# kiva12138/MIMRL

Measured on AMD Instinct MI355X. Metric: two-stage train iters/sec, higher is better.
Workload: dtype bf16

## Files before the change

include/mimrl.h:

```cpp
#ifndef MIMRL_H_
#define MIMRL_H_

#include <stdint.h>

#ifdef __cplusplus
extern "C" {
#endif

#define MIMRL_ABI_VERSION 6
#define MIMRL_MAX_BLOCKS 4
#define MIMRL_MAX_BATCH 2048
#define MIMRL_MAX_BATCH_CONCAT 1024
#define MIMRL_MAX_CLASSES 8

enum { MIMRL_OK = 0, MIMRL_ERR_ARG = -1, MIMRL_ERR_HIP = -2, MIMRL_ERR_STATE = -3, MIMRL_ERR_NODEVICE = -4 };
enum { MIMRL_GROUP_MAIN = 0, MIMRL_GROUP_CRITIC = 1 };
enum { MIMRL_CRITIC_SEPARATE = 0, MIMRL_CRITIC_CONCAT = 1 };
enum { MIMRL_BOUND_INFONCE = 0, MIMRL_BOUND_NWJ, MIMRL_BOUND_TUBA, MIMRL_BOUND_DV, MIMRL_BOUND_JS_FGAN,
       MIMRL_BOUND_JS, MIMRL_BOUND_SMILE, MIMRL_BOUND_MINE, MIMRL_BOUND_INTERPOLATE };
enum { MIMRL_ACT_NONE = 0, MIMRL_ACT_RELU = 1, MIMRL_ACT_GELU = 2, MIMRL_ACT_TANH = 3 };
enum { MIMRL_PREC_FP32 = 0, MIMRL_PREC_BF16_GEMM_FWD = 1, MIMRL_PREC_BF16_GEMM_BWD = 2, MIMRL_PREC_BF16_GRU_FWD = 4,
       MIMRL_PREC_BF16_GRU_BWD = 8, MIMRL_PREC_BF16 = 15 };

enum { MIMRL_BASELINE_CONSTANT = 0, MIMRL_BASELINE_GAUSSAIN = 1, MIMRL_BASELINE_UNNORMALIZED = 2 };
enum { MIMRL_ENCODER_GRU = 0, MIMRL_ENCODER_CONV = 1, MIMRL_ENCODER_LSTM = 2 };
enum { MIMRL_TASK_LOSS_MAE = 0, MIMRL_TASK_LOSS_MSE = 1, MIMRL_TASK_LOSS_RMSE = 2, MIMRL_TASK_LOSS_SIMSE = 3, MIMRL_TASK_LOSS_CCC = 4 };
enum { MIMRL_CLASS_LOSS_CE = 5, MIMRL_CLASS_LOSS_FOCAL = 6, MIMRL_CLASS_LOSS_BCE = 7 };

typedef struct mimrl_cfg {
  int32_t batch;
  int32_t seq_len;
  int32_t time_len;
  int32_t d_t, d_a, d_v;
  int32_t d_common;
  int32_t n_blocks;
  int32_t d_hiddens[MIMRL_MAX_BLOCKS][3];
  int32_t d_outs[MIMRL_MAX_BLOCKS][3];
  int32_t res_project[MIMRL_MAX_BLOCKS];
  int32_t bias, ln_first;
  int32_t activation;
  int32_t compose_t_sum, compose_k_sum;
  int32_t critic_type, bound_type;
  int32_t cmi_hardtanh;
  int32_t k_neighbor;
  int32_t bank_capacity;
  float dropout[4];
  float dropout_mlp[3];
  float coef1[11];
  float coef2[8];
  float weight_decay, grad_clip;
  float beta1, beta2, adam_eps;
  int32_t precision;
  int32_t use_graph;
  int32_t device_anchors;
  int32_t baseline_type;
  int32_t encoder;
  uint64_t seed;
  int32_t num_class;
} mimrl_cfg;

typedef struct mimrl_buffers {
  float *main_p, *main_g, *main_m, *main_v;
  float *crit_p, *crit_g, *crit_m, *crit_v;
  const float *text, *audio, *video, *labels;
  const float *bank_c, *bank_f, *bank_t, *bank_a, *bank_v;
  int32_t* anchors;
  float *lr_main, *lr_critic;
  float *pred;
  float *feats;
  float *scalars;
  const int32_t* knn_override;
  int32_t* counters;
} mimrl_buffers;

enum {
  MIMRL_S1_LOSS = 0,
  MIMRL_S1_MIS = 1,
  MIMRL_S1_LOSSES = 12,
  MIMRL_S2_LOSS = 32,
  MIMRL_S2_TASK = 33,
  MIMRL_S2_MIS = 34,
  MIMRL_S2_LOSSES = 42,
  MIMRL_NSCALARS = 64
};

const char* mimrl_last_error(void);
int mimrl_abi_version(void);
int mimrl_deterministic(void);
int mimrl_device_check(void);

int mimrl_layout_count(const mimrl_cfg* cfg);
int mimrl_layout_entry(const mimrl_cfg* cfg, int idx, char* name, int name_cap, int* group, int64_t* offset, int* ndim,
                       int* dim0, int* dim1);
int mimrl_layout_entry_dim2(const mimrl_cfg* cfg, int idx);
int64_t mimrl_bucket_floats(const mimrl_cfg* cfg, int group);

typedef struct mimrl_handle mimrl_handle;
int mimrl_create(const mimrl_cfg* cfg, void* hip_stream, mimrl_handle** out);
int mimrl_bind(mimrl_handle* h, const mimrl_buffers* bufs);
int mimrl_set_bank_rows(mimrl_handle* h, int rows);
int mimrl_set_inputs(mimrl_handle* h, int set, const float* text, const float* audio, const float* video, const float* labels);
int mimrl_stage1_pipe_prime(mimrl_handle* h);
int mimrl_stage1_pipe(mimrl_handle* h, int next_valid);
int mimrl_stage1_step(mimrl_handle* h);
int mimrl_stage2_step(mimrl_handle* h);
int mimrl_two_stage_step(mimrl_handle* h);
int mimrl_stage_grads(mimrl_handle* h, int stage);
int mimrl_stage_apply(mimrl_handle* h, int stage);
int mimrl_stage_grads_part(mimrl_handle* h, int stage, int part);
int mimrl_forward(mimrl_handle* h, int train_mode, int with_losses);
int mimrl_estimate(mimrl_handle* h, int stage);
int mimrl_set_stage2_prefetch(mimrl_handle* h, int on);
int mimrl_stage2_forward_tail(mimrl_handle* h);
int mimrl_set_grad_scale(mimrl_handle* h, float scale);
int mimrl_params_changed(mimrl_handle* h);
int64_t mimrl_workspace_bytes(const mimrl_handle* h);
enum { MIMRL_PH_GEMM_MISC = 0, MIMRL_PH_GRU_FWD, MIMRL_PH_GRU_BWD, MIMRL_PH_CUBE_FWD, MIMRL_PH_CUBE_BWD, MIMRL_PH_EST_FWD,
       MIMRL_PH_EST_BWD, MIMRL_PH_OPT, MIMRL_PH_MODEL_MISC, MIMRL_NPHASES };
int mimrl_profile_enable(mimrl_handle* h, int on);
int mimrl_set_kernel_stamps(mimrl_handle* h, unsigned long long* ring, int slots);
int mimrl_comm_unique_id(void* out128);
int mimrl_set_comm(mimrl_handle* h, const void* unique_id128, int world, int rank);
int64_t mimrl_main_late_offset(const mimrl_handle* h);
int mimrl_set_comm_critic_bf16(mimrl_handle* h, int on);
int mimrl_set_task_loss(mimrl_handle* h, int kind);
int mimrl_set_class_loss(mimrl_handle* h, int kind);
int mimrl_profile_read(mimrl_handle* h, float* ms_sum , int32_t* launches );
int mimrl_profile_read_gemm(mimrl_handle* h, double out[4]);
void mimrl_destroy(mimrl_handle* h);

int mimrl_op_gemm(void* stream, const float* A, const float* B, float* C, int M, int N, int K, int batch,
                  const int64_t strides[9] , const float* bias_n,
                  const float* bias_m, float alpha, float beta, int act, int precision);
int mimrl_op_gemm_ex(void* stream, const float* A, const float* B, float* C, int M, int N, int K, int batch, const int64_t strides[9],
                     const float* A2, const float* B2, int K2, const int64_t strides2[6], int a_gap_at, int a_gap_rows,
                     const float* bias_n, const float* gradact_u, float* colsum, int act, int precision);
int mimrl_op_gemm16(void* stream, const void* A, const void* B, void* C, int M, int N, int K, int batch, const int64_t strides[9],
                    const void* A2, const void* B2, int K2, const int64_t strides2[6], int batch_in, const int64_t strides_bo[5],
                    const float* bias_n, int flags);
int mimrl_op_gemm_wgrad_group(void* stream, int n, const float* const* A, const float* const* B, float* const* C, const int32_t* dims,
                              const int64_t* strides, int precision);
int64_t mimrl_op_gru_saved_floats(int B, int T);
int mimrl_op_gru_forward(void* stream, const float* gx_f, const float* gx_r, const float* whh_f, const float* whh_r,
                         const float* bhh_f, const float* bhh_r, const int32_t* lens, float* out, float* saved_f,
                         float* saved_r, int B, int T, int precision);
int mimrl_op_gru_backward(void* stream, const float* whh_f, const float* whh_r, const float* saved_f,
                          const float* saved_r, const int32_t* lens, const float* out, const float* dout, float* dg_f,
                          float* dg_r, float* hprev_f, float* hprev_r, int B, int T, int precision);
int mimrl_op_recur_btv(int B, int nmod);
int mimrl_op_lstm_forward(void* stream, const float* gx_f, const float* gx_r, const float* whh_f, const float* whh_r,
                          const float* bhh_f, const float* bhh_r, const int32_t* lens, float* out, float* saved_f,
                          float* saved_r, int B, int T, int kernel);
int mimrl_op_lstm_backward(void* stream, const float* whh_f, const float* whh_r, const float* saved_f,
                           const float* saved_r, const int32_t* lens, const float* out, const float* dout, float* dg_f,
                           float* dg_r, float* hprev_f, float* hprev_r, int B, int T, int kernel);
int mimrl_op_concat_dw(void* stream, const void* dz2, const void* a1, float* dw2, const void* dz1, const void* a0, float* dw1, int E, int64_t rows,
                       int64_t dw_stride, const float* ds, const void* a2h, float* dw3, const uint32_t* m2, const float* w3, const float* P,
                       const float* Q, int B);
int mimrl_op_gru_wgrad(void* stream, const void* const* dg, const void* const* x, const void* const* hp, float* const* dw_ih,
                       float* const* dw_hh, int64_t rows, int kp);
int mimrl_op_mi_bound(void* stream, const float* scores, float* dscores, float* mi, const float* gscale, int E, int B,
                      int bound);
int mimrl_op_mi_bound_ex(void* stream, const float* scores, float* dscores, float* mi, float* mi_loss, const float* gscale,
                         int E, int B, int bound, uint32_t lossform);
#define MIMRL_NCE_WS_FLOATS 2064
int mimrl_op_mi_infonce_rows(void* stream, const float* scores, float* dscores, float* mi, float* mi_loss, const float* gscale,
                             int E, int B, float* ws);
int mimrl_op_mi_bound_baseline(void* stream, float* scores, float* dscores, float* mi, const float* gscale, const float* lb,
                               float* dlb, int E, int B, int bound);
int mimrl_op_mi_sep_infonce(void* stream, const float* tout, float* dtout, float* mi, float* mi_loss, const float* gscale, int E,
                            int B, int tiled);
int mimrl_op_knn(void* stream, const float* Z, int dz, int N, const int32_t* anchors, int m, int k, int32_t* idx_out);
int mimrl_op_sample_anchors(void* stream, int32_t* anchors_out, int ncall, int m, int N, uint64_t seed, const int32_t* step,
                            uint32_t stream_id, int step_add);
int mimrl_knn_r1_host(const float* z, int N, const int32_t* anchors, int m, int k, int32_t* idx_out);
int mimrl_set_knn_override_mask(mimrl_handle* h, int stage, unsigned call_mask);
int mimrl_op_cmi_loss(void* stream, const float* logits, float* dlogits, float* bce, float* cmi, const float* g_bce,
                      const float* g_cmi, int E, int n, int hardtanh);
int mimrl_op_task_loss(void* stream, int kind, const float* pred, const float* y, float* dpred, float* loss, int B);
int mimrl_op_class_loss(void* stream, int kind, const float* logits, const float* y, float* dlogits, float* loss, int B, int C);
int mimrl_op_gather_rows(void* stream, int n_arrays, const void* const* src, void* const* dst, const int64_t* row_bytes, int64_t src_rows,
                         const int32_t* idx, int rows, int max_workgroups);
int mimrl_op_mlp_stack_forward(void* stream, int nb, int rows, int brows, int nl, const int32_t* dims, const float* const* W,
                               const float* const* b, int64_t pstride, const float* in, float* const* act, float* out);
int mimrl_op_mlp_stack_backward(void* stream, int nb, int rows, int brows, int nl, const int32_t* dims, const float* const* W,
                                int64_t pstride, const float* const* act, const float* dout, float* const* dz, float* din,
                                float* const* db);
int mimrl_probe_cube(mimrl_handle* h, const float* x, float* out, const float* dout, float* dx);
int mimrl_probe_encoders(mimrl_handle* h, float* cube_x, const float* dcube, const float* dmean);
int mimrl_probe_mi(mimrl_handle* h, int stage, float* mi, float* scores, float* dtin_out);
int mimrl_probe_cmi(mimrl_handle* h, int stage, const float* cmi_in, float* logits, float* vals, float* dcin_out);
int mimrl_probe_knn(mimrl_handle* h, int stage, int32_t* idx_out);
int mimrl_op_adam(void* stream, float* p, float* g, float* m, float* v, int64_t n, const float* lr, const int32_t* step,
                  float beta1, float beta2, float eps, float weight_decay, float clip);

#ifdef __cplusplus
}
#endif
#endif
```

mimrl_amd/_lib.py:

```python
from __future__ import annotations

import ctypes as C
import os
from typing import List, Tuple

_HERE = os.path.dirname(os.path.abspath(__file__))
DETERMINISTIC = os.environ.get("MIMRL_DETERMINISTIC", "0") not in ("", "0")
LIB_PATH = os.environ.get("MIMRL_LIB_PATH") or os.path.join(_HERE, "libmimrl_hip_det.so" if DETERMINISTIC else "libmimrl_hip.so")
MAX_BLOCKS = 4
MAX_BATCH = 2048
MAX_BATCH_CONCAT = 1024
NCE_WS_FLOATS = 2064
NSCALARS = 64
MAX_CLASSES = 8
PHASES = ["gemm_misc", "gru_fwd", "gru_bwd", "cube_fwd", "cube_bwd", "est_fwd", "est_bwd", "opt", "model_misc"]
S1_LOSS, S1_MIS, S1_LOSSES, S2_LOSS, S2_TASK, S2_MIS, S2_LOSSES = 0, 1, 12, 32, 33, 34, 42

BOUNDS = {"infonce": 0, "nwj": 1, "tuba": 2, "dv": 3, "js_fgan": 4, "js": 5, "smile": 6, "mine": 7, "interpolate": 8}
ACTS = {"none": 0, "relu": 1, "gelu": 2, "tanh": 3}
PREC = {"fp32": 0, "bf16": 15, "bf16_gemm_fwd": 1, "bf16_gemm_bwd": 2, "bf16_gemm": 3, "bf16_gru": 12, "bf16_nogemmbwd": 13}


class MimrlError(RuntimeError):
    pass


class Cfg(C.Structure):
    _fields_ = [
        ("batch", C.c_int32), ("seq_len", C.c_int32), ("time_len", C.c_int32),
        ("d_t", C.c_int32), ("d_a", C.c_int32), ("d_v", C.c_int32), ("d_common", C.c_int32),
        ("n_blocks", C.c_int32),
        ("d_hiddens", (C.c_int32 * 3) * MAX_BLOCKS), ("d_outs", (C.c_int32 * 3) * MAX_BLOCKS),
        ("res_project", C.c_int32 * MAX_BLOCKS),
        ("bias", C.c_int32), ("ln_first", C.c_int32), ("activation", C.c_int32),
        ("compose_t_sum", C.c_int32), ("compose_k_sum", C.c_int32),
        ("critic_type", C.c_int32), ("bound_type", C.c_int32), ("cmi_hardtanh", C.c_int32),
        ("k_neighbor", C.c_int32), ("bank_capacity", C.c_int32),
        ("dropout", C.c_float * 4), ("dropout_mlp", C.c_float * 3),
        ("coef1", C.c_float * 11), ("coef2", C.c_float * 8),
        ("weight_decay", C.c_float), ("grad_clip", C.c_float),
        ("beta1", C.c_float), ("beta2", C.c_float), ("adam_eps", C.c_float),
        ("precision", C.c_int32), ("use_graph", C.c_int32), ("device_anchors", C.c_int32), ("baseline_type", C.c_int32),
        ("encoder", C.c_int32),
        ("seed", C.c_uint64),
        ("num_class", C.c_int32),
    ]


_FP = C.c_void_p


class Buffers(C.Structure):
    _fields_ = [(n, _FP) for n in (
        "main_p", "main_g", "main_m", "main_v", "crit_p", "crit_g", "crit_m", "crit_v",
        "text", "audio", "video", "labels", "bank_c", "bank_f", "bank_t", "bank_a", "bank_v",
        "anchors", "lr_main", "lr_critic", "pred", "feats", "scalars", "knn_override", "counters")]


_lib = None


def load() -> C.CDLL:
    global _lib
    if _lib is not None:
        return _lib
    if not os.path.exists(LIB_PATH):
        raise MimrlError(f"{LIB_PATH} is missing: build it with `python -c 'import __graft_entry__ as g; g.build()'` "
                         f"or `make -C mimrl_amd/csrc` (hipcc --offload-arch=gfx950). There is no CPU fallback.")
    try:
        import torch
    except ImportError:
        pass
    lib = C.CDLL(LIB_PATH)
    if os.environ.get("MIMRL_LIB_PATH"):
        class _Partial:
            def __init__(self, lib):
                object.__setattr__(self, "_lib", lib)

            def __getattr__(self, name):
                try:
                    return getattr(self._lib, name)
                except AttributeError:
                    return type("_Missing", (), {})()
        real, lib = lib, _Partial(lib)
    lib.mimrl_last_error.restype = C.c_char_p
    lib.mimrl_bucket_floats.restype = C.c_int64
    lib.mimrl_workspace_bytes.restype = C.c_int64
    lib.mimrl_op_gru_saved_floats.restype = C.c_int64
    lib.mimrl_destroy.restype = None
    lib.mimrl_op_gemm.argtypes = [_FP, _FP, _FP, _FP, C.c_int, C.c_int, C.c_int, C.c_int, C.POINTER(C.c_int64), _FP, _FP,
                                  C.c_float, C.c_float, C.c_int, C.c_int]
    lib.mimrl_op_gemm_ex.argtypes = [_FP, _FP, _FP, _FP, C.c_int, C.c_int, C.c_int, C.c_int, C.POINTER(C.c_int64), _FP, _FP, C.c_int,
                                     C.POINTER(C.c_int64), C.c_int, C.c_int, _FP, _FP, _FP, C.c_int, C.c_int]
    lib.mimrl_comm_unique_id.argtypes = [_FP]
    lib.mimrl_set_comm.argtypes = [_FP, _FP, C.c_int, C.c_int]
    lib.mimrl_set_comm_critic_bf16.argtypes = [_FP, C.c_int]
    lib.mimrl_set_task_loss.argtypes = [_FP, C.c_int]
    lib.mimrl_op_task_loss.argtypes = [_FP, C.c_int, _FP, _FP, _FP, _FP, C.c_int]
    lib.mimrl_set_class_loss.argtypes = [_FP, C.c_int]
    lib.mimrl_op_class_loss.argtypes = [_FP, C.c_int, _FP, _FP, _FP, _FP, C.c_int, C.c_int]
    lib.mimrl_op_gather_rows.argtypes = [_FP, C.c_int, C.POINTER(C.c_void_p), C.POINTER(C.c_void_p), C.POINTER(C.c_int64), C.c_int64, _FP,
                                         C.c_int, C.c_int]
    lib.mimrl_main_late_offset.argtypes = [_FP]
    lib.mimrl_main_late_offset.restype = C.c_int64
    lib.mimrl_op_gemm16.argtypes = [_FP, _FP, _FP, _FP, C.c_int, C.c_int, C.c_int, C.c_int, C.POINTER(C.c_int64), _FP, _FP, C.c_int,
                                    C.POINTER(C.c_int64), C.c_int, C.POINTER(C.c_int64), _FP, C.c_int]
    lib.mimrl_op_gemm_wgrad_group.argtypes = [_FP, C.c_int, C.POINTER(C.c_void_p), C.POINTER(C.c_void_p), C.POINTER(C.c_void_p),
                                              C.POINTER(C.c_int32), C.POINTER(C.c_int64), C.c_int]
    lib.mimrl_op_adam.argtypes = [_FP, _FP, _FP, _FP, _FP, C.c_int64, _FP, _FP, C.c_float, C.c_float, C.c_float,
                                  C.c_float, C.c_float]
    lib.mimrl_op_gru_forward.argtypes = [_FP] * 11 + [C.c_int, C.c_int, C.c_int]
    lib.mimrl_op_gru_backward.argtypes = [_FP] * 12 + [C.c_int, C.c_int, C.c_int]
    lib.mimrl_op_lstm_forward.argtypes = [_FP] * 11 + [C.c_int, C.c_int, C.c_int]
    lib.mimrl_op_lstm_backward.argtypes = [_FP] * 12 + [C.c_int, C.c_int, C.c_int]
    lib.mimrl_op_recur_btv.argtypes = [C.c_int, C.c_int]
    lib.mimrl_op_concat_dw.argtypes = [C.c_void_p] * 7 + [C.c_int, C.c_int64, C.c_int64] + [C.c_void_p] * 7 + [C.c_int]
    lib.mimrl_op_gru_wgrad.argtypes = [C.c_void_p] + [C.POINTER(C.c_void_p)] * 5 + [C.c_int64, C.c_int]
    lib.mimrl_op_mi_bound.argtypes = [_FP] * 5 + [C.c_int, C.c_int, C.c_int]
    lib.mimrl_op_mi_bound_ex.argtypes = [_FP] * 6 + [C.c_int, C.c_int, C.c_int, C.c_uint32]
    lib.mimrl_op_mi_infonce_rows.argtypes = [_FP] * 6 + [C.c_int, C.c_int, _FP]
    lib.mimrl_op_mi_sep_infonce.argtypes = [_FP] * 6 + [C.c_int, C.c_int, C.c_int]
    lib.mimrl_op_mi_bound_baseline.argtypes = [_FP] * 7 + [C.c_int, C.c_int, C.c_int]
    lib.mimrl_op_knn.argtypes = [_FP, _FP, C.c_int, C.c_int, _FP, C.c_int, C.c_int, _FP]
    lib.mimrl_op_cmi_loss.argtypes = [_FP] * 7 + [C.c_int, C.c_int, C.c_int]
    lib.mimrl_op_sample_anchors.argtypes = [_FP, _FP, C.c_int, C.c_int, C.c_int, C.c_uint64, _FP, C.c_uint32, C.c_int]
    lib.mimrl_create.argtypes = [C.POINTER(Cfg), _FP, C.POINTER(_FP)]
    lib.mimrl_bind.argtypes = [_FP, C.POINTER(Buffers)]
    lib.mimrl_profile_read.argtypes = [_FP, C.POINTER(C.c_float), C.POINTER(C.c_int32)]
    lib.mimrl_profile_read_gemm.argtypes = [_FP, C.POINTER(C.c_double)]
    for fn in ("mimrl_set_bank_rows", "mimrl_stage_grads", "mimrl_stage_grads_part", "mimrl_stage_apply", "mimrl_estimate", "mimrl_profile_enable", "mimrl_set_stage2_prefetch"):
        getattr(lib, fn).argtypes = [_FP, C.c_int]
    lib.mimrl_set_grad_scale.argtypes = [_FP, C.c_float]
    lib.mimrl_stage_grads_part.argtypes = [_FP, C.c_int, C.c_int]
    lib.mimrl_set_inputs.argtypes = [_FP, C.c_int, _FP, _FP, _FP, _FP]
    lib.mimrl_knn_r1_host.argtypes = [_FP, C.c_int, _FP, C.c_int, C.c_int, _FP]
    lib.mimrl_set_knn_override_mask.argtypes = [_FP, C.c_int, C.c_uint]
    for fn in ("mimrl_stage1_step", "mimrl_stage2_step", "mimrl_two_stage_step", "mimrl_destroy", "mimrl_workspace_bytes", "mimrl_params_changed",
               "mimrl_stage2_forward_tail"):
        getattr(lib, fn).argtypes = [_FP]
    lib.mimrl_forward.argtypes = [_FP, C.c_int, C.c_int]
    lib.mimrl_set_kernel_stamps.argtypes = [_FP, _FP, C.c_int]
    lib.mimrl_probe_cube.argtypes = [_FP] * 5
    lib.mimrl_probe_mi.argtypes = [_FP, C.c_int, _FP, _FP, _FP]
    lib.mimrl_probe_cmi.argtypes = [_FP, C.c_int, _FP, _FP, _FP, _FP]
    lib.mimrl_probe_knn.argtypes = [_FP, C.c_int, _FP]
    lib.mimrl_probe_encoders.argtypes = [_FP] * 4
    lib.mimrl_layout_count.argtypes = [C.POINTER(Cfg)]
    lib.mimrl_layout_entry_dim2.argtypes = [C.POINTER(Cfg), C.c_int]
    lib.mimrl_bucket_floats.argtypes = [C.POINTER(Cfg), C.c_int]
    lib.mimrl_layout_entry.argtypes = [C.POINTER(Cfg), C.c_int, C.c_char_p, C.c_int, C.POINTER(C.c_int),
                                       C.POINTER(C.c_int64), C.POINTER(C.c_int), C.POINTER(C.c_int), C.POINTER(C.c_int)]
    if os.environ.get("MIMRL_LIB_PATH"):
        lib = real
    _lib = lib
    return lib


ENCODERS = {"gru": 0, "conv": 1, "lstm": 2}
BASELINES = {"constant": 0, "gaussain": 1, "unnormalized": 2}

EXPORTS = [
    "mimrl_last_error", "mimrl_abi_version", "mimrl_deterministic", "mimrl_device_check", "mimrl_layout_count", "mimrl_layout_entry", "mimrl_layout_entry_dim2",
    "mimrl_bucket_floats", "mimrl_create", "mimrl_bind", "mimrl_set_bank_rows", "mimrl_set_inputs", "mimrl_stage1_step", "mimrl_stage2_step", "mimrl_two_stage_step",
    "mimrl_stage_grads", "mimrl_stage_grads_part", "mimrl_stage_apply", "mimrl_forward", "mimrl_estimate", "mimrl_profile_enable", "mimrl_profile_read", "mimrl_profile_read_gemm",
    "mimrl_workspace_bytes", "mimrl_params_changed", "mimrl_set_stage2_prefetch", "mimrl_stage2_forward_tail", "mimrl_set_grad_scale", "mimrl_destroy", "mimrl_op_gemm", "mimrl_op_gemm_ex", "mimrl_op_gemm16", "mimrl_op_gemm_wgrad_group",
    "mimrl_op_gru_saved_floats", "mimrl_op_gru_forward", "mimrl_op_gru_backward", "mimrl_op_gru_wgrad", "mimrl_op_concat_dw", "mimrl_op_mi_bound", "mimrl_op_mi_bound_ex", "mimrl_op_mi_bound_baseline", "mimrl_op_mi_sep_infonce", "mimrl_op_knn",
    "mimrl_op_cmi_loss", "mimrl_op_sample_anchors", "mimrl_knn_r1_host", "mimrl_set_knn_override_mask", "mimrl_op_mlp_stack_forward", "mimrl_op_mlp_stack_backward", "mimrl_op_adam",
    "mimrl_probe_cube", "mimrl_probe_mi", "mimrl_probe_cmi", "mimrl_probe_knn", "mimrl_probe_encoders", "mimrl_set_kernel_stamps", "mimrl_comm_unique_id", "mimrl_set_comm", "mimrl_main_late_offset", "mimrl_set_comm_critic_bf16",
    "mimrl_stage1_pipe_prime", "mimrl_stage1_pipe", "mimrl_set_task_loss", "mimrl_op_task_loss", "mimrl_set_class_loss", "mimrl_op_class_loss",
    "mimrl_op_mi_infonce_rows", "mimrl_op_lstm_forward", "mimrl_op_lstm_backward", "mimrl_op_recur_btv", "mimrl_op_gather_rows",
]

TASK_LOSSES = {"MAE": 0, "MSE": 1, "RMSE": 2, "SIMSE": 3, "CCC": 4}
BATCH_COUPLED_LOSSES = ("RMSE", "SIMSE", "CCC")
CLASS_LOSSES = {"CE": 5, "Focal": 6, "BCE": 7}


def task_loss_code(opt, world: int = 1) -> int:
    loss = getattr(opt, "loss", "MAE")
    task = getattr(opt, "task", "regression")
    ncls = int(getattr(opt, "num_class", 1))
    if loss in CLASS_LOSSES:
        if task != "classification":
            raise NotImplementedError(f"--loss {loss} is a classification loss: it needs --task classification (and --num_class)")
        if loss == "BCE" and ncls not in (1, 2):
            raise NotImplementedError(f"--loss BCE needs --num_class 1 or 2, got {ncls} (Solver.py:327-337)")
        if loss != "BCE" and not 2 <= ncls <= MAX_CLASSES:
            raise NotImplementedError(f"--loss {loss} needs 2 <= --num_class <= {MAX_CLASSES}, got {ncls}")
        if int(world) > 1 and loss == "Focal":
            raise NotImplementedError(f"--loss {loss} couples the whole batch: with {int(world)} ranks each would see only its shard, not the "
                                      f"reference's global batch; run it on one rank, or use CE / BCE")
        return CLASS_LOSSES[loss]
    if loss not in TASK_LOSSES:
        raise NotImplementedError(f"--loss {loss}: unknown task loss (choose one of {', '.join(list(TASK_LOSSES) + list(CLASS_LOSSES))})")
    if task == "classification" or ncls > 1:
        raise NotImplementedError(f"--loss {loss} is a regression loss: --task classification / --num_class {ncls} need one of "
                                  f"{', '.join(CLASS_LOSSES)}")
    if int(world) > 1 and loss in BATCH_COUPLED_LOSSES:
        raise NotImplementedError(f"--loss {loss} couples the whole batch: with {int(world)} ranks each would see only its shard, not the "
                                  f"reference's global batch; run it on one rank, or use MAE / MSE")
    return TASK_LOSSES[loss]


def check(rc: int) -> int:
    if rc < 0:
        raise MimrlError(f"libmimrl_hip error {rc}: {load().mimrl_last_error().decode()}")
    return rc


def make_cfg(opt, d_t: int, d_a: int, d_v: int, seq_len: int = None, bank_capacity: int = 0, precision: str = "fp32",
             use_graph: bool = False, seed: int = 0, device_anchors: bool = False, batch: int = None) -> Cfg:
    c = Cfg()
    c.batch = int(batch if batch is not None else opt.batch_size)
    c.time_len = int(opt.time_len)
    c.seq_len = int(seq_len if seq_len is not None else opt.time_len)
    c.d_t, c.d_a, c.d_v, c.d_common = int(d_t), int(d_a), int(d_v), int(opt.d_common)
    enc = getattr(opt, "encoders", "gru")
    if enc not in ENCODERS:
        raise MimrlError(f"--encoders {enc}: choose gru, conv or lstm (Model.py:237)")
    c.encoder = ENCODERS[enc]
    nb = len(opt.d_hiddens)
    if nb > MAX_BLOCKS or len(opt.d_outs) != nb or len(opt.res_project) != nb:
        raise MimrlError("d_hiddens / d_outs / res_project must have the same length (<= 4)")
    c.n_blocks = nb
    for i in range(nb):
        for ax in range(3):
            c.d_hiddens[i][ax] = int(opt.d_hiddens[i][ax])
            c.d_outs[i][ax] = int(opt.d_outs[i][ax])
        c.res_project[i] = int(bool(opt.res_project[i]))
    c.bias, c.ln_first = int(bool(opt.bias)), int(bool(opt.ln_first))
    if opt.activate not in ACTS:
        raise MimrlError(f"--activate {opt.activate} not supported on the HIP path (gelu/relu/tanh)")
    c.activation = ACTS[opt.activate]
    for name, attr in (("features_compose_t", "compose_t_sum"), ("features_compose_k", "compose_k_sum")):
        v = getattr(opt, name, "mean")
        if v not in ("mean", "sum"):
            raise MimrlError(f"--{name} {v}: only mean/sum supported")
        setattr(c, attr, int(v == "sum"))
    if opt.critic_type not in ("separate", "concat"):
        raise NotImplementedError(opt.critic_type)
    c.critic_type = 0 if opt.critic_type == "separate" else 1
    bl = getattr(opt, "baseline_type", "constant")
    if bl not in BASELINES:
        raise NotImplementedError(f"--baseline_type {bl}")
    c.baseline_type = BASELINES[bl]
    if opt.bound_type not in BOUNDS:
        raise NotImplementedError(opt.bound_type)
    c.bound_type = BOUNDS[opt.bound_type]
    if opt.cmi_last_acticate not in ("sigmoid", "hardtanh"):
        raise NotImplementedError(opt.cmi_last_acticate)
    c.cmi_hardtanh = int(opt.cmi_last_acticate == "hardtanh")
    c.k_neighbor = int(opt.k_neighbor)
    c.bank_capacity = int(bank_capacity)
    for i in range(4):
        c.dropout[i] = float(opt.dropout[i])
    for i in range(3):
        c.dropout_mlp[i] = float(opt.dropout_mlp[i])
    if len(opt.loss_mi_coefficient1) != 11 or len(opt.loss_mi_coefficient2) != 8:
        raise MimrlError("loss_mi_coefficient1/2 need 11 / 8 entries")
    for i in range(11):
        c.coef1[i] = float(opt.loss_mi_coefficient1[i])
    for i in range(8):
        c.coef2[i] = float(opt.loss_mi_coefficient2[i])
    c.weight_decay, c.grad_clip = float(opt.weight_decay), float(opt.gradient_clip)
    c.beta1, c.beta2, c.adam_eps = 0.9, 0.999, 1e-8
    c.precision = PREC[precision]
    c.use_graph = int(bool(use_graph))
    c.device_anchors = int(bool(device_anchors))
    c.seed = int(seed) & 0xFFFFFFFFFFFFFFFF
    c.num_class = int(getattr(opt, "num_class", 1))
    return c


def layout_entries(cfg: Cfg) -> Tuple[List[Tuple[str, int, int, Tuple[int, ...]]], Tuple[int, int]]:
    lib = load()
    n = check(lib.mimrl_layout_count(C.byref(cfg)))
    out = []
    name = C.create_string_buffer(256)
    g, nd, d0, d1 = C.c_int(), C.c_int(), C.c_int(), C.c_int()
    off = C.c_int64()
    for i in range(n):
        check(lib.mimrl_layout_entry(C.byref(cfg), i, name, 256, C.byref(g), C.byref(off), C.byref(nd), C.byref(d0), C.byref(d1)))
        shape = (d0.value, d1.value) if nd.value == 2 else (d0.value,)
        if nd.value == 3:
            shape = (d0.value, d1.value, check(lib.mimrl_layout_entry_dim2(C.byref(cfg), i)))
        out.append((name.value.decode(), g.value, off.value, shape))
    sizes = (check(lib.mimrl_bucket_floats(C.byref(cfg), 0)), check(lib.mimrl_bucket_floats(C.byref(cfg), 1)))
    return out, sizes


def knn_r1_host(z, anchors, k: int):
    import numpy as np
    z = np.ascontiguousarray(np.asarray(z, dtype=np.float32).reshape(-1))
    a = np.ascontiguousarray(np.asarray(anchors, dtype=np.int32).reshape(-1))
    if int(k) >= (len(z) - len(a)) // 2:
        return None
    out = np.empty((len(a), int(k)), dtype=np.int32)
    check(load().mimrl_knn_r1_host(z.ctypes.data_as(C.c_void_p), len(z), a.ctypes.data_as(C.c_void_p), len(a), int(k),
                                   out.ctypes.data_as(C.c_void_p)))
    return out
```

mimrl_amd/csrc/cube_bwd_fused.h:

```cpp
#pragma once
#include "common.h"
#include "model_ops.h"

namespace mimrl {

struct LAxisBwdArgs {
  const float *dz, *y, *mean, *rstd, *gamma;
  const float* u;
  const float *w2, *w1, *wr;
  float *dy, *du, *dx;
  float *db2, *db1;
  int B, il, hl, ol, C, act;
};
bool laxis_bwd_supported(int il, int hl, int ol, int C);
int laxis_bwd_fused(hipStream_t s, const LAxisBwdArgs& a);

struct DAxisBwdArgs {
  const float *dz, *y, *mean, *rstd, *gamma;
  const float* u;
  const __bf16 *w2t, *w1t, *wrt;
  float *dy, *du, *dx;
  long R;
  int act;
  float *dgamma, *dbeta, *db2, *db1;
};
bool daxis_bwd_supported(int id, int hd, int od);
int daxis_bwd_fused(hipStream_t s, const DAxisBwdArgs& a);

struct WtTransposeArgs { const float* src[12]; __bf16* dst[12]; int n; };
int wt_transpose_bf16(hipStream_t s, const WtTransposeArgs& a);

int daxis_param_grads(hipStream_t s, const float* y, const float* mean, const float* rstd, const float* dz, const float* dy,
                      const float* du, float* dgamma, float* dbeta, float* db2, float* db1, long R);

#ifdef MIMRL_PHASE_PROBE
int cube_bwd_read_phases(long long* out);
#endif

}
```

mimrl_amd/csrc/cube_bwd_fused.hip:

```cpp
#include "cube_bwd_fused.h"
#include "kmix_device.h"

namespace mimrl {

namespace {

#ifdef MIMRL_PHASE_PROBE
__device__ long long g_cbwd_phase[64];
#define BPHASE(base, i) do { if (blockIdx.x == 0 && blockIdx.y == 0 && threadIdx.x == 0) g_cbwd_phase[(base) + (i)] = (long long)wall_clock64(); } while (0)
#else
#define BPHASE(base, i) do { } while (0)
#endif

constexpr int CT = 128;
constexpr int KP = 64 + 8;


template <bool LONG = false>
__global__ __launch_bounds__(256, LONG ? 2 : 1) void laxis_bwd_kernel(LAxisBwdArgs a) {
  __shared__ __attribute__((aligned(16))) __bf16 sdyu[2][CT][KP];
  auto& sdy = sdyu[0];
  auto& sdu = sdyu[1];
  __shared__ __attribute__((aligned(16))) __bf16 wts[3][64][KP];
  float (*red)[2][CT] = reinterpret_cast<float (*)[2][CT]>(&sdu[0][0]);
  __shared__ float acc_l[3][64];
  __shared__ LdsAcc acc_h[64];
  __shared__ float sgam[64];
  const int tid = threadIdx.x, lane = tid & 63, wave = tid >> 6, lr = lane & 31, lh = lane >> 5;
  const int b = blockIdx.y, c0 = blockIdx.x * CT;
  const int il = a.il, hl = a.hl, ol = a.ol, C = a.C;
  const int pb = ol > 32 ? 16 : 0;
  BPHASE(pb, 0);

  float uu[2][16];
  {
    const int ccu = c0 + wave * 32 + lr;
#pragma unroll
    for (int mt = 0; mt < 2; ++mt)
#pragma unroll
      for (int r = 0; r < 16; ++r) {
        const int h = min(mt * 32 + (r & 3) + 8 * (r >> 2) + 4 * lh, hl - 1);
        uu[mt][r] = a.u[((long)b * hl + h) * C + ccu];
      }
  }
  {
    uint4* z = reinterpret_cast<uint4*>(&wts[0][0][0]);
    for (int i = tid; i < 3 * 64 * KP * 2 / 16; i += 256) z[i] = make_uint4(0u, 0u, 0u, 0u);
    if (tid < 64) { acc_l[0][tid] = 0.f; acc_l[1][tid] = 0.f; acc_l[2][tid] = 0.f; acc_h[tid].zero(); sgam[tid] = a.gamma[tid < ol ? tid : ol - 1]; }
  }
  __syncthreads();
  BPHASE(pb, 1);
  {
    const int n2 = ol * hl, n1 = hl * il, nr = ol * il;
    float wv[3][16];
#pragma unroll
    for (int j = 0; j < 16; ++j) {
      const int idx = tid + 256 * j;
      wv[0][j] = a.w2[idx < n2 ? idx : n2 - 1];
      if constexpr (!LONG) {
        wv[1][j] = a.w1[idx < n1 ? idx : n1 - 1];
        wv[2][j] = a.wr[idx < nr ? idx : nr - 1];
      }
    }
#pragma unroll
    for (int j = 0; j < 16; ++j) {
      const int idx = tid + 256 * j;
      if (idx < n2) { const int o = idx / hl, h = idx - o * hl; wts[0][h][o] = to_bf16(wv[0][j]); }
      if constexpr (!LONG) {
        if (idx < n1) { const int h = idx / il, i = idx - h * il; wts[1][i][h] = to_bf16(wv[1][j]); }
        if (idx < nr) { const int o = idx / il, i = idx - o * il; wts[2][i][o] = to_bf16(wv[2][j]); }
      }
    }
  }

  BPHASE(pb, 2);
  const int col = tid & (CT - 1), half = tid >> 7;
  const long cidx = (long)b * C + c0 + col;
  const float mu = a.mean[cidx], rs = a.rstd[cidx];
  const float* __restrict__ dzb = a.dz + (long)b * ol * C + c0 + col;
  const float* __restrict__ yb = a.y + (long)b * ol * C + c0 + col;
  float* __restrict__ dyb = a.dy + (long)b * ol * C + c0 + col;
  float gq[32], xq[32];
#pragma unroll
  for (int j = 0; j < 32; ++j) {
    const int l = min(half + 2 * j, ol - 1);
    gq[j] = dzb[(long)l * C]; xq[j] = yb[(long)l * C];
  }
  float s1 = 0.f, s2 = 0.f;
#pragma unroll
  for (int j = 0; j < 32; ++j) {
    const int l = half + 2 * j;
    xq[j] = (xq[j] - mu) * rs;
    gq[j] = l < ol ? gq[j] * sgam[min(l, 63)] : 0.f;
    s1 += gq[j]; s2 += gq[j] * xq[j];
  }
  BPHASE(pb, 3);
  red[0][half][col] = s1;
  red[1][half][col] = s2;
  __syncthreads();
  s1 = (red[0][0][col] + red[0][1][col]) / ol;
  s2 = (red[1][0][col] + red[1][1][col]) / ol;
#pragma unroll
  for (int j = 0; j < 32; ++j) {
    const int l = half + 2 * j;
    if (l < ol) {
      const float v = rs * (gq[j] - s1 - xq[j] * s2);
      dyb[(long)l * C] = v;
      sdy[col][l] = to_bf16(v);
    }
  }
  for (int l = ol + ((half ^ ol) & 1); l < 64; l += 2) sdy[col][l] = to_bf16(0.f);
  __syncthreads();

  if (a.db2 && tid >= 192 && tid - 192 < ol) {
    float t = 0.f;
    for (int c = 0; c < CT; ++c) t += (float)sdy[(c + tid) & (CT - 1)][tid - 192];
    acc_l[2][tid - 192] = t;
  }
  BPHASE(pb, 4);
  const int nt = wave;
  const int cc = c0 + nt * 32 + lr;
  {
    f32x16 acc0, acc1;
#pragma unroll
    for (int r = 0; r < 16; ++r) { acc0[r] = 0.f; acc1[r] = 0.f; }
#pragma unroll
    for (int ks = 0; ks < 4; ++ks) {
      const bf16x8 bf = *reinterpret_cast<const bf16x8*>(&sdy[nt * 32 + lr][ks * 16 + 8 * lh]);
      const bf16x8 a0 = *reinterpret_cast<const bf16x8*>(&wts[0][lr][ks * 16 + 8 * lh]);
      acc0 = __builtin_amdgcn_mfma_f32_32x32x16_bf16(a0, bf, acc0, 0, 0, 0);
      const bf16x8 a1 = *reinterpret_cast<const bf16x8*>(&wts[0][32 + lr][ks * 16 + 8 * lh]);
      acc1 = __builtin_amdgcn_mfma_f32_32x32x16_bf16(a1, bf, acc1, 0, 0, 0);
    }
    act_dispatch(a.act, [&](auto AT) __attribute__((always_inline)) {
#pragma unroll
    for (int mt = 0; mt < 2; ++mt)
#pragma unroll
      for (int r = 0; r < 16; ++r) {
        const int h = mt * 32 + (r & 3) + 8 * (r >> 2) + 4 * lh;
        float v = 0.f;
        if (h < hl) {
          const long ui = ((long)b * hl + h) * C + cc;
          v = (mt == 0 ? acc0[r] : acc1[r]) * act_grad_c<decltype(AT)::value>(a.act, uu[mt][r]);
          a.du[ui] = v;
        }
        sdu[nt * 32 + lr][h] = to_bf16(v);
        if (a.db1) {
          const float t = half_sum_hi(v);
          if (lr == 16 && h < hl) acc_h[h].add(t);
        }
      }
    });
  }
  __syncthreads();
  BPHASE(pb, 5);
  if constexpr (LONG) {
    float w1v[16], wrv[16];
    auto wreq = [&](int i0) __attribute__((always_inline)) {
      const int i = min(i0 + (tid & 63), il - 1);
#pragma unroll
      for (int j = 0; j < 16; ++j) {
        const int r = 16 * (tid >> 6) + j;
        w1v[j] = a.w1[(long)min(r, hl - 1) * il + i];
        wrv[j] = a.wr[(long)min(r, ol - 1) * il + i];
      }
    };
    wreq(0);
    for (int i0 = 0; i0 < il; i0 += 64) {
      __syncthreads();
      {
        const int ii = tid & 63, r0 = 16 * (tid >> 6);
        const bool iok = i0 + ii < il;
        bf16x8 p1[2], p2[2];
#pragma unroll
        for (int j = 0; j < 16; ++j) {
          p1[j >> 3][j & 7] = to_bf16(iok && r0 + j < hl ? w1v[j] : 0.f);
          p2[j >> 3][j & 7] = to_bf16(iok && r0 + j < ol ? wrv[j] : 0.f);
        }
        *reinterpret_cast<bf16x8*>(&wts[1][ii][r0]) = p1[0]; *reinterpret_cast<bf16x8*>(&wts[1][ii][r0 + 8]) = p1[1];
        *reinterpret_cast<bf16x8*>(&wts[2][ii][r0]) = p2[0]; *reinterpret_cast<bf16x8*>(&wts[2][ii][r0 + 8]) = p2[1];
      }
      __syncthreads();
      wreq(i0 + 64 < il ? i0 + 64 : i0);
      f32x16 acc0, acc1;
#pragma unroll
      for (int r = 0; r < 16; ++r) { acc0[r] = 0.f; acc1[r] = 0.f; }
#pragma unroll
      for (int ks = 0; ks < 8; ++ks) {
        const bool first = ks < 4;
        const int kk = (first ? ks : ks - 4) * 16 + 8 * lh;
        const bf16x8 bf = *reinterpret_cast<const bf16x8*>(first ? &sdu[nt * 32 + lr][kk] : &sdy[nt * 32 + lr][kk]);
        const bf16x8 a0 = *reinterpret_cast<const bf16x8*>(&wts[first ? 1 : 2][lr][kk]);
        acc0 = __builtin_amdgcn_mfma_f32_32x32x16_bf16(a0, bf, acc0, 0, 0, 0);
        const bf16x8 a1 = *reinterpret_cast<const bf16x8*>(&wts[first ? 1 : 2][32 + lr][kk]);
        acc1 = __builtin_amdgcn_mfma_f32_32x32x16_bf16(a1, bf, acc1, 0, 0, 0);
      }
      {
#pragma unroll
        for (int mt = 0; mt < 2; ++mt)
#pragma unroll
          for (int r = 0; r < 16; ++r) {
            const int i = i0 + mt * 32 + (r & 3) + 8 * (r >> 2) + 4 * lh;
            if (i < il) a.dx[((long)b * il + i) * C + cc] = mt == 0 ? acc0[r] : acc1[r];
          }
      }
    }
  } else {
    f32x16 acc0, acc1;
#pragma unroll
    for (int r = 0; r < 16; ++r) { acc0[r] = 0.f; acc1[r] = 0.f; }
#pragma unroll
    for (int ks = 0; ks < 8; ++ks) {
      const bool first = ks < 4;
      const int kk = (first ? ks : ks - 4) * 16 + 8 * lh;
      const bf16x8 bf = *reinterpret_cast<const bf16x8*>(first ? &sdu[nt * 32 + lr][kk] : &sdy[nt * 32 + lr][kk]);
      const bf16x8 a0 = *reinterpret_cast<const bf16x8*>(&wts[first ? 1 : 2][lr][kk]);
      acc0 = __builtin_amdgcn_mfma_f32_32x32x16_bf16(a0, bf, acc0, 0, 0, 0);
      const bf16x8 a1 = *reinterpret_cast<const bf16x8*>(&wts[first ? 1 : 2][32 + lr][kk]);
      acc1 = __builtin_amdgcn_mfma_f32_32x32x16_bf16(a1, bf, acc1, 0, 0, 0);
    }
    {
#pragma unroll
      for (int mt = 0; mt < 2; ++mt)
#pragma unroll
        for (int r = 0; r < 16; ++r) {
          const int i = mt * 32 + (r & 3) + 8 * (r >> 2) + 4 * lh;
          if (i < il) a.dx[((long)b * il + i) * C + cc] = mt == 0 ? acc0[r] : acc1[r];
        }
    }
  }
  __syncthreads();
  BPHASE(pb, 6);
  if (a.db2 && tid < ol) acc_add(&a.db2[tid], acc_l[2][tid]);
  if (a.db1 && tid >= 64 && tid - 64 < hl) acc_add(&a.db1[tid - 64], acc_h[tid - 64].get());
  BPHASE(pb, 7);
}

}

#ifdef MIMRL_PHASE_PROBE
int cube_bwd_read_phases(long long* out) { return hipMemcpyFromSymbol(out, HIP_SYMBOL(g_cbwd_phase), sizeof(long long) * 64) == hipSuccess ? 0 : 1; }
#endif

bool laxis_bwd_supported(int il, int hl, int ol, int C) {
  return il >= 1 && hl >= 1 && ol >= 1 && hl <= 64 && ol <= 64 && C % CT == 0;
}

int laxis_bwd_fused(hipStream_t s, const LAxisBwdArgs& a) {
  if (!laxis_bwd_supported(a.il, a.hl, a.ol, a.C)) return set_error(MIMRL_ERR_ARG, "laxis_bwd_fused: unsupported shape");
  if (!a.wr) return set_error(MIMRL_ERR_ARG, "laxis_bwd_fused: needs the residual projection");
  if (a.il > 64) hipLaunchKernelGGL(laxis_bwd_kernel<true>, dim3(a.C / CT, a.B), dim3(256), 0, s, a);
  else hipLaunchKernelGGL(laxis_bwd_kernel<false>, dim3(a.C / CT, a.B), dim3(256), 0, s, a);
  LAUNCH_CHECK();
  return MIMRL_OK;
}

namespace {

constexpr int DR = 32;
constexpr int DP = 128 + 8;

__global__ __launch_bounds__(256) void daxis_bwd_kernel(DAxisBwdArgs a) {
  __shared__ __attribute__((aligned(16))) __bf16 sdy[DR][DP];
  __shared__ __attribute__((aligned(16))) __bf16 sdu[DR][DP];
  __shared__ LdsAcc spg[3][128];
  const int tid = threadIdx.x, lane = tid & 63, wave = tid >> 6, lr = lane & 31, lh = lane >> 5;
  const long r0 = (long)blockIdx.x * DR;
  const bool pg = a.dgamma != nullptr;
  const int pb = gridDim.x <= 200 ? 32 : 48;
  BPHASE(pb, 0);
  if (pg) for (int i = tid; i < 3 * 128; i += 256) (&spg[0][0])[i].zero();
  const int row1 = tid >> 3, part1 = tid & 7;
  const long r1 = r0 + row1;
  const bool ok1 = r1 < a.R;
  const long rc1 = ok1 ? r1 : a.R - 1;
  const float mu1 = a.mean[rc1], rs1 = a.rstd[rc1];
  float4 gz4[4], yv4[4];
#pragma unroll
  for (int q = 0; q < 4; ++q) {
    gz4[q] = *reinterpret_cast<const float4*>(a.dz + rc1 * 128 + part1 * 16 + q * 4);
    yv4[q] = *reinterpret_cast<const float4*>(a.y + rc1 * 128 + part1 * 16 + q * 4);
  }
  const int n = wave * 32 + lr;
  bf16x8 bw2[8], bw1[8], bwr[8];
#pragma unroll
  for (int ks = 0; ks < 8; ++ks) {
    bw2[ks] = *reinterpret_cast<const bf16x8*>(a.w2t + n * 128 + ks * 16 + 8 * lh);
    bw1[ks] = *reinterpret_cast<const bf16x8*>(a.w1t + n * 128 + ks * 16 + 8 * lh);
    bwr[ks] = *reinterpret_cast<const bf16x8*>(a.wrt + n * 128 + ks * 16 + 8 * lh);
  }
  float uu[16];
#pragma unroll
  for (int r = 0; r < 16; ++r) {
    const long row = min(r0 + (r & 3) + 8 * (r >> 2) + 4 * lh, a.R - 1);
    uu[r] = a.u[row * 128 + n];
  }
  BPHASE(pb, 1);
  {
    const int row = row1, part = part1;
    const long r = r1;
    const bool ok = ok1;
    float g[16], xh[16], dyk[16];
    float s1 = 0.f, s2 = 0.f;
    const float mu = mu1, rs = rs1;
#pragma unroll
    for (int q = 0; q < 4; ++q) {
      const float4 gz = gz4[q];
      const float4 yv = yv4[q];
      const float gg[4] = {gz.x, gz.y, gz.z, gz.w}, yy[4] = {yv.x, yv.y, yv.z, yv.w};
#pragma unroll
      for (int j = 0; j < 4; ++j) {
        g[q * 4 + j] = gg[j];
        xh[q * 4 + j] = (yy[j] - mu) * rs;
        const float dxh = gg[j] * a.gamma[part * 16 + q * 4 + j];
        s1 += dxh; s2 += dxh * xh[q * 4 + j];
      }
    }
    s1 = group_sum<8>(s1); s2 = group_sum<8>(s2);
    s1 *= (1.f / 128.f); s2 *= (1.f / 128.f);
#pragma unroll
    for (int q = 0; q < 4; ++q) {
      float v[4];
#pragma unroll
      for (int j = 0; j < 4; ++j) {
        const int c = part * 16 + q * 4 + j;
        v[j] = rs * (g[q * 4 + j] * a.gamma[c] - s1 - xh[q * 4 + j] * s2);
      }
      if (ok) *reinterpret_cast<float4*>(a.dy + r * 128 + part * 16 + q * 4) = make_float4(v[0], v[1], v[2], v[3]);
      bf16x4 p; p[0] = to_bf16(v[0]); p[1] = to_bf16(v[1]); p[2] = to_bf16(v[2]); p[3] = to_bf16(v[3]);
      *reinterpret_cast<bf16x4*>(&sdy[row][part * 16 + q * 4]) = p;
      if (pg) {
#pragma unroll
        for (int j = 0; j < 4; ++j) { const float gz = ok ? g[q * 4 + j] : 0.f; xh[q * 4 + j] *= gz; g[q * 4 + j] = gz; v[j] = ok ? v[j] : 0.f; }
        dyk[q * 4 + 0] = v[0]; dyk[q * 4 + 1] = v[1]; dyk[q * 4 + 2] = v[2]; dyk[q * 4 + 3] = v[3];
      }
    }
    if (pg) {
      __syncthreads();
#pragma unroll
      for (int j = 0; j < 16; ++j) {
        float sa = xh[j], sb = g[j], sc = dyk[j];
#pragma unroll
        for (int o = 8; o < 64; o <<= 1) { sa += __shfl_xor(sa, o, 64); sb += __shfl_xor(sb, o, 64); sc += __shfl_xor(sc, o, 64); }
        if (lane < 8) { spg[0][part * 16 + j].add(sa); spg[1][part * 16 + j].add(sb); spg[2][part * 16 + j].add(sc); }
      }
    }
  }
  __syncthreads();
  BPHASE(pb, 2);
  {
    f32x16 acc;
#pragma unroll
    for (int r = 0; r < 16; ++r) acc[r] = 0.f;
#pragma unroll
    for (int ks = 0; ks < 8; ++ks) {
      const bf16x8 af = *reinterpret_cast<const bf16x8*>(&sdy[lr][ks * 16 + 8 * lh]);
      acc = __builtin_amdgcn_mfma_f32_32x32x16_bf16(af, bw2[ks], acc, 0, 0, 0);
    }
    float csum = 0.f;
    act_dispatch(a.act, [&](auto AT) __attribute__((always_inline)) {
#pragma unroll
    for (int r = 0; r < 16; ++r) {
      const int m = (r & 3) + 8 * (r >> 2) + 4 * lh;
      const long row = r0 + m;
      float v = 0.f;
      if (row < a.R) {
        v = acc[r] * act_grad_c<decltype(AT)::value>(a.act, uu[r]);
        a.du[row * 128 + n] = v;
      }
      sdu[m][n] = to_bf16(v);
      csum += v;
    }
    });
    if (pg) {
      csum += __shfl_xor(csum, 32, 64);
      if (lh == 0) acc_add(&a.db1[n], csum);
    }
  }
  __syncthreads();
  BPHASE(pb, 3);
  if (pg && tid < 128) {
    acc_add(&a.dgamma[tid], spg[0][tid].get());
    acc_add(&a.dbeta[tid], spg[1][tid].get());
    acc_add(&a.db2[tid], spg[2][tid].get());
  }
  {
    f32x16 acc;
#pragma unroll
    for (int r = 0; r < 16; ++r) acc[r] = 0.f;
#pragma unroll
    for (int ks = 0; ks < 8; ++ks) {
      const bf16x8 a1 = *reinterpret_cast<const bf16x8*>(&sdu[lr][ks * 16 + 8 * lh]);
      acc = __builtin_amdgcn_mfma_f32_32x32x16_bf16(a1, bw1[ks], acc, 0, 0, 0);
      const bf16x8 a2 = *reinterpret_cast<const bf16x8*>(&sdy[lr][ks * 16 + 8 * lh]);
      acc = __builtin_amdgcn_mfma_f32_32x32x16_bf16(a2, bwr[ks], acc, 0, 0, 0);
    }
#pragma unroll
    for (int r = 0; r < 16; ++r) {
      const long row = r0 + (r & 3) + 8 * (r >> 2) + 4 * lh;
      if (row < a.R) a.dx[row * 128 + n] = acc[r];
    }
  }
  BPHASE(pb, 4);
}

__global__ void wt_transpose_kernel(WtTransposeArgs a) {
  __shared__ float t[32][33];
  const float* __restrict__ src = a.src[blockIdx.z];
  __bf16* __restrict__ dst = a.dst[blockIdx.z];
  const int k0 = blockIdx.y * 32, n0 = blockIdx.x * 32, tx = threadIdx.x & 31, ty = threadIdx.x >> 5;
  for (int j = ty; j < 32; j += 8) t[j][tx] = src[(k0 + j) * 128 + n0 + tx];
  __syncthreads();
  for (int j = ty; j < 32; j += 8) dst[(n0 + j) * 128 + k0 + tx] = to_bf16(t[tx][j]);
}

__global__ __launch_bounds__(256) void daxis_param_grads_kernel(const float* __restrict__ y, const float* __restrict__ mean,
                                                                const float* __restrict__ rstd, const float* __restrict__ dz,
                                                                const float* __restrict__ dy, const float* __restrict__ du,
                                                                float* __restrict__ dgamma, float* __restrict__ dbeta,
                                                                float* __restrict__ db2, float* __restrict__ db1, long R) {
  __shared__ float4 red[4][8][32];
  const int cq = threadIdx.x & 31, rl = threadIdx.x >> 5;
  const long r0 = (long)blockIdx.x * 64;
  float4 a0 = make_float4(0.f, 0.f, 0.f, 0.f), a1 = a0, a2 = a0, a3 = a0;
#pragma unroll
  for (int i = 0; i < 8; ++i) {
    const long r = r0 + rl + 8 * i;
    const long rc = r < R ? r : R - 1;
    const float m = r < R ? 1.f : 0.f;
    const float mu = mean[rc], rs = rstd[rc] * m;
    const float4 g = *reinterpret_cast<const float4*>(dz + rc * 128 + cq * 4);
    const float4 yv = *reinterpret_cast<const float4*>(y + rc * 128 + cq * 4);
    const float4 v = *reinterpret_cast<const float4*>(dy + rc * 128 + cq * 4);
    const float4 u = *reinterpret_cast<const float4*>(du + rc * 128 + cq * 4);
    a0.x += g.x * (yv.x - mu) * rs; a0.y += g.y * (yv.y - mu) * rs; a0.z += g.z * (yv.z - mu) * rs; a0.w += g.w * (yv.w - mu) * rs;
    a1.x += g.x * m; a1.y += g.y * m; a1.z += g.z * m; a1.w += g.w * m;
    a2.x += v.x * m; a2.y += v.y * m; a2.z += v.z * m; a2.w += v.w * m;
    a3.x += u.x * m; a3.y += u.y * m; a3.z += u.z * m; a3.w += u.w * m;
  }
  red[0][rl][cq] = a0; red[1][rl][cq] = a1; red[2][rl][cq] = a2; red[3][rl][cq] = a3;
  __syncthreads();
#pragma unroll
  for (int h = 0; h < 2; ++h) {
    const int idx = threadIdx.x + 256 * h, q = idx >> 7, c = idx & 127;
    const float* base = reinterpret_cast<const float*>(&red[q][0][0]);
    float sum = 0.f;
#pragma unroll
    for (int j = 0; j < 8; ++j) sum += base[j * 128 + c];
    float* dst = q == 0 ? dgamma : (q == 1 ? dbeta : (q == 2 ? db2 : db1));
    if (dst) acc_add(&dst[c], sum);
  }
}

}

int daxis_param_grads(hipStream_t s, const float* y, const float* mean, const float* rstd, const float* dz, const float* dy,
                      const float* du, float* dgamma, float* dbeta, float* db2, float* db1, long R) {
  if (R <= 0) return MIMRL_OK;
  hipLaunchKernelGGL(daxis_param_grads_kernel, dim3((unsigned)((R + 63) / 64)), dim3(256), 0, s, y, mean, rstd, dz, dy, du, dgamma, dbeta,
                     db2, db1, R);
  LAUNCH_CHECK();
  return MIMRL_OK;
}

bool daxis_bwd_supported(int id, int hd, int od) { return id == 128 && hd == 128 && od == 128; }

int daxis_bwd_fused(hipStream_t s, const DAxisBwdArgs& a) {
  if (!a.w2t || !a.w1t || !a.wrt) return set_error(MIMRL_ERR_ARG, "daxis_bwd_fused: needs the transposed weight images");
  if ((a.dgamma || a.dbeta || a.db2 || a.db1) && !(a.dgamma && a.dbeta && a.db2 && a.db1))
    return set_error(MIMRL_ERR_ARG, "daxis_bwd_fused: the four parameter-gradient outputs come together");
  hipLaunchKernelGGL(daxis_bwd_kernel, dim3((unsigned)((a.R + DR - 1) / DR)), dim3(256), 0, s, a);
  LAUNCH_CHECK();
  return MIMRL_OK;
}

int wt_transpose_bf16(hipStream_t s, const WtTransposeArgs& a) {
  if (a.n < 1 || a.n > 12) return set_error(MIMRL_ERR_ARG, "wt_transpose_bf16: 1..12 matrices");
  hipLaunchKernelGGL(wt_transpose_kernel, dim3(4, 4, a.n), dim3(256), 0, s, a);
  LAUNCH_CHECK();
  return MIMRL_OK;
}

}
```

mimrl_amd/csrc/engine.h:

```cpp
#pragma once
#include <cstdio>
#include <cstdlib>
#include <cstring>
#include <algorithm>
#include <vector>
#include <dlfcn.h>

#include "cube_fused.h"
#include "mlp_fused.h"
#include "concat_fused.h"
#include "cube_bwd_fused.h"
#include "cube_long.h"
#include "estimator_ops.h"
#include "gemm.h"
#include "gru.h"
#include "gru_wgrad.h"
#include "concat_dw.h"
#include "lstm.h"
#include "layout.h"
#include "comm.h"
#include "model_ops.h"
#include "scoped.h"

namespace mimrl {

namespace eng {


constexpr int H = 128, G = 384, HID = 256, EMB = 128;
constexpr int NE_MI = 5, NE_CMI = 6;
constexpr int ACT_SLACK = 4 * MLPF_MAX_WIDTH;

enum { FT_F = 0, FT_T = 1, FT_A = 2, FT_V = 3, FT_C = 4 };
const int kMiWire[NE_MI][2] = {{FT_F, FT_T}, {FT_F, FT_A}, {FT_F, FT_V}, {FT_T, FT_A}, {FT_T, FT_V}};
const int kCmiWire[NE_CMI][3] = {{FT_A, FT_C, FT_T}, {FT_T, FT_A, FT_C}, {FT_V, FT_C, FT_T},
                                 {FT_T, FT_V, FT_C}, {FT_T, FT_C, FT_A}, {FT_T, FT_C, FT_V}};
static const char* const kVmi[NE_MI] = {"f_t", "f_a", "f_v", "t_a", "t_v"};
static const char* const kVcmi[NE_CMI] = {"ac_t", "ta_c", "vc_t", "tv_c", "tc_a", "tc_v"};

void launch_begin_stage(hipStream_t s, int* rng_step, int* adam_step, float* scalars, int scal_off, int scal_n);
void launch_bucket_to_bf16(hipStream_t s, const float* src, void* dst, long n);
void launch_bucket_from_bf16(hipStream_t s, const void* src, float* dst, long n);
void launch_task_loss(hipStream_t s, int kind, const float* pred, const float* y, float* dpred, float* task, int B, int C = 1);
void launch_finalize_stage1(hipStream_t s, float* scal, const float* mi, const float* cmi, const float* bce, const float* coef1);
void launch_finalize_stage2(hipStream_t s, float* scal, const float* mi, const float* cmi, const float* coef2, int have_mi);
void launch_stage_boundary(hipStream_t s, float* scal, const float* mi, const float* cmi, const float* bce, const float* coef1, int* rng_step,
                           int* adam_step, const float* pred, const float* y, float* dpred, int B, int kind, int C = 1);

struct Roctx {
  int (*push)(const char*) = nullptr;
  int (*pop)() = nullptr;
  Roctx() {
    void* h = dlopen("librocprofiler-sdk-roctx.so", RTLD_LAZY | RTLD_LOCAL);
    if (!h) h = dlopen("librocprofiler-sdk-roctx.so.1", RTLD_LAZY | RTLD_LOCAL);
    if (!h) h = dlopen("libroctx64.so", RTLD_LAZY | RTLD_LOCAL);
    if (!h) h = dlopen("libroctx64.so.4", RTLD_LAZY | RTLD_LOCAL);
    if (h) {
      push = reinterpret_cast<int (*)(const char*)>(dlsym(h, "roctxRangePushA"));
      pop = reinterpret_cast<int (*)()>(dlsym(h, "roctxRangePop"));
      if (!push || !pop) push = nullptr;
    }
  }
};
inline Roctx& roctx() { static Roctx r; return r; }
struct Range {
  bool on;
  explicit Range(const char* name) : on(roctx().push != nullptr) { if (on) roctx().push(name); }
  ~Range() { if (on) roctx().pop(); }
};

struct Lin { long w = -1, b = -1; int out = 0, in = 0; };
struct GruDirW { long w_ih = 0, w_hh = 0, b_ih = 0, b_hh = 0; int din = 0; };
struct AxisW { Lin fc1, fc2; long res = -1, ln_g = -1, ln_b = -1; int in = 0, hid = 0, out = 0; };
struct BlockW { AxisW ax[3]; };
struct MixBuf { float *xn = nullptr, *xn_mean = nullptr, *xn_rstd = nullptr, *u = nullptr, *h = nullptr, *y = nullptr,
                      *z = nullptr, *mean = nullptr, *rstd = nullptr; };
struct BlockBuf { MixBuf l, k, d; };

}

using namespace eng;

}

using namespace mimrl;

struct mimrl_handle {
  mimrl_cfg cfg;
  hipStream_t stream = nullptr;
  hipStream_t user_stream = nullptr;
  hipStream_t cap_stream = nullptr;
  Layout layout;
  mimrl_buffers bufs;
  bool bound = false;
  DetRanges det_ranges;
  float* nce_ws = nullptr;
  bool grads_clean[3] = {true, true, true};
  int bank_rows = 0;
  bool bf16 = false;
  int prec = 0;
  bool bf16_fwd() const { return (prec & MIMRL_PREC_BF16_GEMM_FWD) != 0; }
  bool bf16_bwd() const { return (prec & MIMRL_PREC_BF16_GEMM_BWD) != 0; }

  GruDirW gru[2][2][2];
  long ln_g[2], ln_b[2], w_t;
  BlockW blk[MIMRL_MAX_BLOCKS];
  long cls_w, cls_b;
  __bf16 *crit_img = nullptr, *crit_imgT = nullptr;
  __bf16 *crit_frag = nullptr, *crit_fragT = nullptr;
  FragTable ftab;
  bool frag_side_pending = false;
  bool frag_tr_deferred = false;
  FragTable ftab_tr;
  bool adam_frag_on = true;
  bool boundary_in_adam = false;
  bool img_valid = false;
  unsigned knn_ovr_mask[2] = {0u, 0u};
  bool knn_pre = true;
  bool mi_fused_bwd_done = false;
  bool imgT_ready = false;
  TransposeTable ttab;
  int ensure_images() {
    if (img_valid || !crit_img) return MIMRL_OK;
    MX(bf16_image(user_stream, bufs.crit_p, crit_img, layout.floats[MIMRL_GROUP_CRITIC]));
    if (crit_frag && ftab.n > 0) MX(bf16_frag_images(user_stream, bufs.crit_p, crit_frag, ftab));
    img_valid = true;
    return MIMRL_OK;
  }
  long bl0 = 0, bl_stride = 0, bl_l[4][2];
  float *lbv = nullptr, *dlbv = nullptr, *bact[3] = {nullptr, nullptr, nullptr}, *bdz[3] = {nullptr, nullptr, nullptr}, *bdin = nullptr;
  bool has_baseline() const {
    return cfg.baseline_type != MIMRL_BASELINE_CONSTANT && (cfg.bound_type == MIMRL_BOUND_TUBA || cfg.bound_type == MIMRL_BOUND_INTERPOLATE);
  }
  int baseline_forward();
  int baseline_backward(int stage);
  long tower0 = 0, tower_stride = 0;
  long tower_l[4][2];
  long cmi0 = 0, cmi_stride = 0, cmi_l[4][2];

  char* ws = nullptr;
  size_t ws_bytes = 0, ws_used = 0;
  int* d_ints = nullptr;
  int* d_ints_own = nullptr;
  float* d_consts = nullptr;
  int *lens[2] = {nullptr, nullptr};
  bool kmix_pg_on_side3 = false;
  bool begin_in_pack = false;
  hipEvent_t ev_lens = nullptr;
  float *tx_raw = nullptr, *gx[2][2], *h0[2], *h1[2], *sv[2][2][2], *ln_mean[2], *ln_rstd[2];
  float* tailp_part = nullptr;
  bool pre_done = false;
  int dual_tail_pre();
  float* cube0 = nullptr;
  float *xpack = nullptr, *wpack = nullptr, *bpack = nullptr, *dwih_pack = nullptr, *dwhh_pack = nullptr;
  _Float16* h0h[2] = {nullptr, nullptr}; _Float16* w1h = nullptr; __bf16* w1b = nullptr;
  __bf16* w1bt = nullptr;
  bool h16_on = true;
  float* w2p[MIMRL_MAX_BLOCKS] = {};
  bool w2p_valid[MIMRL_MAX_BLOCKS] = {};
  bool xin_on = true;
  bool part0_done = false;
  bool l0_xin = false;
  bool xpack16 = false;
  bool laxis_bwd_long_on = true;
  bool laxis_long_on = true;
  bool rec16_on = true, dwih_h16_on = true;
  bool hp16_live = false;
  bool dh0_bf16_live = false, ds_bf16_live = false;
  bool h16_live = false;
  bool w1_img_valid = false;
  int KP() const { return ((cfg.d_a > cfg.d_v ? cfg.d_a : cfg.d_v) + 15) & ~15; }
  bool dg_bf16 = false;
  bool concat_compact = false;
  bool a0_regen_live = false;
  bool fused_concat = true;
  bool l0_packed = false;
  bool l0_bwd_pack = false;
  BlockBuf bb[MIMRL_MAX_BLOCKS];
  __bf16* wtT[MIMRL_MAX_BLOCKS][3] = {};
  struct FwdSet {
    int* lens[2] = {nullptr, nullptr};
    float *tx_raw = nullptr, *gx[2][2] = {{nullptr, nullptr}, {nullptr, nullptr}}, *h0[2] = {nullptr, nullptr}, *h1[2] = {nullptr, nullptr};
    float *ln_mean[2] = {nullptr, nullptr}, *ln_rstd[2] = {nullptr, nullptr}, *cube0 = nullptr, *feats = nullptr, *pred = nullptr;
    _Float16* h0h[2] = {nullptr, nullptr};
    BlockBuf bb[MIMRL_MAX_BLOCKS];
  } alt;
  void swap_fwd_set() {
    for (int m = 0; m < 2; ++m) {
      std::swap(lens[m], alt.lens[m]); std::swap(h0[m], alt.h0[m]); std::swap(h1[m], alt.h1[m]); std::swap(h0h[m], alt.h0h[m]);
      std::swap(ln_mean[m], alt.ln_mean[m]); std::swap(ln_rstd[m], alt.ln_rstd[m]);
      for (int d = 0; d < 2; ++d) std::swap(gx[m][d], alt.gx[m][d]);
    }
    std::swap(tx_raw, alt.tx_raw); std::swap(cube0, alt.cube0);
    std::swap(bufs.feats, alt.feats); std::swap(bufs.pred, alt.pred);
    for (int i = 0; i < MIMRL_MAX_BLOCKS; ++i) std::swap(bb[i], alt.bb[i]);
  }
  struct FwdSetSwap {
    mimrl_handle* h; bool on = false;
    explicit FwdSetSwap(mimrl_handle* h_, bool now = true) : h(h_) { if (now) enter(); }
    ~FwdSetSwap() { if (on) h->swap_fwd_set(); }
    FwdSetSwap(const FwdSetSwap&) = delete;
    FwdSetSwap& operator=(const FwdSetSwap&) = delete;
    void enter() { h->swap_fwd_set(); on = true; }
  };
  bool prefetch = false;
  bool defer_tail = false;
  bool tail2_needed = false;
  bool fwd2_pending = false;
  float grad_scale = 1.f;
  void* comm = nullptr; int comm_world = 1, comm_rank = 0;
  bool comm_crit_bf16 = false; void* comm_crit16 = nullptr;
  int task_loss = MIMRL_TASK_LOSS_MAE;
  int ncls() const { return cfg.num_class >= 2 ? cfg.num_class : 1; }
  hipStream_t comm_s = nullptr;
  bool comm_split = true;
  KernelStamp kstamp;

  int run_fwd2_tail();
  hipStream_t pre_stream = nullptr;
  int carve_fwd(size_t* gmax_out);
  float *ff = nullptr, *dpred = nullptr;
  float *tin = nullptr, *ta[3], *tout = nullptr, *scores = nullptr, *dscores = nullptr;
  float *cP = nullptr, *cQ = nullptr, *ca[3];
  int split_part = 0;
  bool fold_unpack = false, unpack_pending = false;
  bool fold_unpack_on = true;
  bool gx_f16 = false;
  int *knn_idx = nullptr, *knn_idx2 = nullptr;
  int knn_flip = 0;
  int knn_slot(int stage) const { return (stage - 1) ^ knn_flip; }
  char* knn_scr[2] = {nullptr, nullptr};
  size_t knn_scr_bytes = 0;
  float *cmi_in = nullptr, *cc[3], *logits = nullptr, *dlogits = nullptr;
  float *mi_raw = nullptr, *cmi_raw = nullptr, *bce_raw = nullptr;
  float *dfeat = nullptr, *dtout = nullptr, *dta[3], *dtin = nullptr, *dca[3], *dP = nullptr, *dQ = nullptr;
  float *dcc[3], *dcin = nullptr;
  static constexpr int NGBUF = 24;
  float* gbuf[NGBUF];
  size_t gbuf_floats = 0;
  float *dtx = nullptr, *ds[2], *dg[2][2][2], *hprev[2][2][2], *dh0[2];

  static constexpr int NSIDE = 6;
  hipStream_t side[NSIDE] = {nullptr, nullptr, nullptr, nullptr, nullptr, nullptr};
  std::vector<hipEvent_t> ev_pool;
  size_t ev_next = 0;
  bool multi_stream = true;
  bool fused_cube_bwd = true;
  bool fused_mlp = true;
  bool fused_cube = true;
  bool fused_pre_on = true;
  bool cube_bookends = true;
  bool keep_cube0 = false;
  int fwd_f16 = 1;
  int next_event(hipEvent_t* e) {
    if (ev_next == ev_pool.size()) {
      hipEvent_t n;
      HIPX(hipEventCreateWithFlags(&n, hipEventDisableTiming));
      ev_pool.push_back(n);
    }
    *e = ev_pool[ev_next++];
    return MIMRL_OK;
  }
  int G_group(hipStream_t st, const GemmDesc* ds, int n) {
    if (!prof_on) return gemm_group(st, ds, n, bf16);
    for (int i = 0; i < n; ++i) MX(G_on(st, ds[i]));
    return MIMRL_OK;
  }
  unsigned side_mask = ~0u;
  bool side_on(int i) const { return multi_stream && ((side_mask >> i) & 1u); }
  hipStream_t S(int i) const { return side_on(i) ? side[i] : stream; }
  int fork(int lo, int hi) {
    if (!multi_stream) return MIMRL_OK;
    hipEvent_t e = nullptr;
    for (int i = lo; i <= hi; ++i) {
      if (!side_on(i)) continue;
      if (!e) { MX(next_event(&e)); HIPX(hipEventRecord(e, stream)); }
      HIPX(hipStreamWaitEvent(side[i], e, 0));
    }
    return MIMRL_OK;
  }
  int join(int lo, int hi) {
    if (!multi_stream) return MIMRL_OK;
    for (int i = lo; i <= hi; ++i) {
      if (!side_on(i)) continue;
      hipEvent_t e;
      MX(next_event(&e));
      HIPX(hipEventRecord(e, side[i]));
      HIPX(hipStreamWaitEvent(stream, e, 0));
    }
    return MIMRL_OK;
  }
  int chain(int i, int j) {
    if (!multi_stream || S(i) == S(j)) return MIMRL_OK;
    hipEvent_t e;
    MX(next_event(&e));
    HIPX(hipEventRecord(e, S(j)));
    HIPX(hipStreamWaitEvent(S(i), e, 0));
    return MIMRL_OK;
  }
  int reduce_bucket(int stage) {
    if (!comm) return MIMRL_OK;
    Range rg(stage == 1 ? "mimrl.stage1.allreduce(crit_g) [RCCL]" : "mimrl.stage2.allreduce(main_g) [RCCL]");
    if (stage == 1 && comm_crit_bf16) {
      const long n = layout.floats[MIMRL_GROUP_CRITIC];
      launch_bucket_to_bf16(stream, bufs.crit_g, comm_crit16, n);
      LAUNCH_CHECK();
      MX(comm_allreduce_sum_bf16(comm, comm_crit16, (size_t)n, stream));
      launch_bucket_from_bf16(stream, comm_crit16, bufs.crit_g, n);
      LAUNCH_CHECK();
      return MIMRL_OK;
    }
    return comm_allreduce_sum(comm, stage == 1 ? bufs.crit_g : bufs.main_g, (size_t)layout.floats[stage == 1 ? MIMRL_GROUP_CRITIC : MIMRL_GROUP_MAIN], stream);
  }
  int enqueue_grads2_reduced(bool skip_zero);
  struct GemmProf { hipEvent_t a, b; double flops, bytes; };
  std::vector<GemmProf> prof_gemm;
  int G_on(hipStream_t st, const GemmDesc& d) {
    if (!prof_on) return gemm(st, d, bf16);
    GemmProf g;
    if (!prof_pool.empty()) { g.a = prof_pool.back().first; g.b = prof_pool.back().second; prof_pool.pop_back(); }
    else { HIPX(hipEventCreate(&g.a)); HIPX(hipEventCreate(&g.b)); }
    auto distinct = [&](long s_b, long s_bo) -> double {
      if (d.batch_in > 0) return (double)(s_bo != 0 ? d.batch / d.batch_in : 1) * (s_b != 0 ? d.batch_in : 1);
      return s_b != 0 ? d.batch : 1;
    };
    g.flops = 2.0 * d.M * d.N * ((double)d.K + (d.A2 ? d.K2 : 0)) * d.batch;
    const double ea = d.a_bf16 ? 2.0 : 4.0, eb = d.b_bf16 ? 2.0 : 4.0;
    g.bytes = ea * d.M * d.K * distinct(d.sa_b, d.sa_bo) + eb * d.K * d.N * distinct(d.sb_b, d.sb_bo) +
              4.0 * d.M * d.N * distinct(d.sc_b, d.sc_bo) * ((d.beta != 0.f || d.atomic) ? 2 : 1);
    if (d.A2) g.bytes += ea * d.M * d.K2 * (d.sa2_b ? d.batch : 1) + eb * d.K2 * d.N * (d.sb2_b ? d.batch : 1);
    HIPX(hipEventRecord(g.a, st));
    const int r = gemm(st, d, bf16);
    HIPX(hipEventRecord(g.b, st));
    prof_gemm.push_back(g);
    return r;
  }

  bool prof_on = false;
  std::vector<std::pair<hipEvent_t, hipEvent_t>> prof_ev[MIMRL_NPHASES];
  std::vector<std::pair<hipEvent_t, hipEvent_t>> prof_pool;
  struct Scope {
    mimrl_handle* h; int ph; hipEvent_t a = nullptr, b = nullptr;
    Scope(mimrl_handle* h_, int ph_) : h(h_), ph(ph_) {
      if (!h->prof_on) return;
      if (!h->prof_pool.empty()) { a = h->prof_pool.back().first; b = h->prof_pool.back().second; h->prof_pool.pop_back(); }
      else { (void)hipEventCreate(&a); (void)hipEventCreate(&b); }
      (void)hipEventRecord(a, h->stream);
    }
    ~Scope() {
      if (!a) return;
      (void)hipEventRecord(b, h->stream);
      h->prof_ev[ph].push_back({a, b});
    }
  };

  struct CachedGraph { hipGraphExec_t exec = nullptr; int rows = -1; };
  struct GraphSet {
    CachedGraph all[3 * 4 + 1 + 2 * 4];
    CachedGraph& graph(int stage, int k) { return all[stage * 4 + k]; }
    CachedGraph& tail() { return all[12]; }
    CachedGraph& pipe(int ahead, int parity) { return all[13 + ahead * 4 + parity]; }
    const void* in[4] = {nullptr, nullptr, nullptr, nullptr};
  } gsets[2];
  int cur_set = 0;
  GraphSet& GS() { return gsets[cur_set]; }
  std::vector<hipGraphExec_t> retired;
  void retire(hipGraphExec_t& ex) { if (ex) { retired.push_back(ex); ex = nullptr; } }
  void drop_graphs(int set = -1) {
    for (int q = 0; q < 2; ++q)
      if (set < 0 || q == set)
        for (CachedGraph& c : gsets[q].all) retire(c.exec);
  }
  template <typename Body>
  int replay_or_capture(CachedGraph& slot, Body&& body, bool postprocess = false);
  float* P(long off) const { return bufs.main_p + off; }
  float* Gm(long off) const { return bufs.main_g + off; }
  float* CP(long off) const { return bufs.crit_p + off; }
  float* CG(long off) const { return bufs.crit_g + off; }
  long conv_w[2] = {0, 0}, conv_b[2] = {0, 0};
  int encoders_forward(bool save, int knn_stage);
  int conv_forward(int knn_stage);
  int conv_backward();
  int lstm_encoders_forward(bool save, int knn_stage);
  int lstm_encoders_backward();
  int rng_add = 0;
  RngKey key() const { return RngKey{(uint32_t)cfg.seed, (uint32_t)(cfg.seed >> 32), d_ints, rng_add}; }
  const float* coef1() const { return d_consts; }
  const float* coef2() const { return d_consts + 11; }
  const float* gs_mi(int stage) const { return d_consts + 19 + (stage - 1) * 5; }
  const float* g_bce(int stage) const { return d_consts + 29 + (stage - 1) * 6; }
  const float* g_cmi(int stage) const { return d_consts + 41 + (stage - 1) * 6; }
  int nprod() const { return (cfg.batch / cfg.k_neighbor) * cfg.k_neighbor; }
  int m_anchor() const { return cfg.batch / cfg.k_neighbor; }

  int resolve();
  int alloc_workspace();
  template <typename T>
  int take(T** p, size_t count) {
    const size_t bytes = (count * sizeof(T) + 255) / 256 * 256;
    if (ws) {
      if (ws_used + bytes > ws_bytes) return set_error(MIMRL_ERR_STATE, "workspace overflow");
      *p = reinterpret_cast<T*>(ws + ws_used);
    }
    ws_used += bytes;
    return MIMRL_OK;
  }
  int carve();

  int G_(const GemmDesc& d) { return G_on(stream, d); }
  struct Deferred { int kind; int side; GemmDesc g; const float* src; long n0, n1, n2, n3; float* dst;
                    const float *p1 = nullptr, *p2 = nullptr, *p3 = nullptr; float* dst2 = nullptr; KMixW kw = KMixW();
                    const float *p4 = nullptr, *p5 = nullptr; float *dst3 = nullptr, *dst4 = nullptr; };
  std::vector<Deferred> deferred;
  int flush_deferred(int only_side = 0);
  int wg_helper = -1;
  int dbg_delay(hipStream_t st, int tag);
  int model_forward(bool train, bool save, int knn_stage = 0, int part = 0);
  int cube_forward(bool train, bool save, const CubePre* pre = nullptr, const CubeHead* head = nullptr);
  bool cube_block_fused(int i, bool train) const;
  int cube_backward(int cur_in, int* cur_out);
  int wt_images(hipStream_t st, bool bwd_bf16, bool launch, bool* d_fused);
  int model_backward();
  int encoders_backward(float* dcube);
  int gru_layer_backward(int l);
  int knn_launch(int stage, hipStream_t st);
  bool pipe_primed = false; int fwd_parity = 0, pipe_set = 0;
  int pipe_forward_body(bool other_inputs);
  int run_stage1_pipe_prime();
  int run_stage1_pipe(bool next_valid);
  int mi_forward(int stage, bool want_grad);
  int cmi_forward(int stage, bool want_grad);
  int mi_backward(int stage);
  int cmi_backward(int stage);
  int route_feature_grads();
  GatherSum head_gather;
  bool head_gather_on = false;
  hipEvent_t ev_dmean = nullptr;
  int estimators_all(int stage, bool want_grad, bool backward);
  int mlp_stack_forward(int nb, int rows, int brows, long p0, long pstride, int nl, const long (*l_off)[2], const int* dims,
                        const float* in, float* const* act, float* out);
  int mlp_stack_backward(int nb, int rows, int brows, long p0, long pstride, int nl, const long (*l_off)[2],
                         const int* dims, const float* in, float* const* act, float* dout, float* const* dtmp, float* din,
                         bool wgrad);
  int enqueue_grads(int stage, bool skip_zero = false);
  int enqueue_apply(int stage);
  int run(int stage, int kind);
  int run_step();
  bool keep_events = false;
  bool fuse_boundary = false;
  bool imgT_valid = false;
  bool skip_imgT_refresh = false;
  bool wtT_prebuilt = false;
  bool wtT_built = false;
};
```

mimrl_amd/csrc/engine_abi.hip:

```cpp
#include "engine.h"

extern "C" {

const char* mimrl_last_error(void) { return mimrl::last_error_slot().c_str(); }
#ifdef MIMRL_PHASE_PROBE
int mimrl_dbg_cube_phases(long long* out) { return mimrl::cube_fwd_read_phases(out); }
int mimrl_dbg_cube_bwd_phases(long long* out) { return mimrl::cube_bwd_read_phases(out); }
int mimrl_dbg_kmix_phases(long long* out) { return mimrl::kmix_bwd_read_phases(out); }
int mimrl_dbg_nce_phases(long long* out) { return mimrl::nce_read_phases(out); }
int mimrl_dbg_model_ops_phases(long long* out) { return mimrl::model_ops_read_phases(out); }
int mimrl_dbg_gru_bwd_phases(long long* out) { return mimrl::gru_bwd_read_phases(out); }
int mimrl_dbg_concat_bwd_phases(long long* out) { return mimrl::concat_bwd_read_phases(out); }
#endif
int mimrl_abi_version(void) { return MIMRL_ABI_VERSION; }

int mimrl_device_check(void) {
  int n = 0;
  if (hipGetDeviceCount(&n) != hipSuccess || n <= 0) return set_error(MIMRL_ERR_NODEVICE, "no HIP device visible");
  int dev = 0;
  if (hipGetDevice(&dev) != hipSuccess) return set_error(MIMRL_ERR_NODEVICE, "hipGetDevice failed");
  hipDeviceProp_t p;
  if (hipGetDeviceProperties(&p, dev) != hipSuccess) return set_error(MIMRL_ERR_NODEVICE, "hipGetDeviceProperties failed");
  if (std::strncmp(p.gcnArchName, "gfx950", 6) != 0)
    return set_error(MIMRL_ERR_NODEVICE, "device %d is %s; this library is built for gfx950 (MI355X) only", dev, p.gcnArchName);
// ... 173 lines not shown
  if (h->bank_rows <= 0) return set_error(MIMRL_ERR_STATE, "mimrl_estimate needs non-empty banks");
  MX(h->ensure_images());
  h->ev_next = 0;
  MX(h->fork(4, 4));
  MX(h->knn_launch(stage, h->S(4)));
  MX(h->estimators_all(stage, false, false));
  if (stage == 1) {
    launch_finalize_stage1(h->stream, h->bufs.scalars, h->mi_raw, h->cmi_raw,
                       h->bce_raw, h->coef1());
  } else {
    launch_task_loss(h->stream, h->task_loss, h->bufs.pred, h->bufs.labels, (float*)nullptr,
                       h->bufs.scalars + MIMRL_S2_TASK, h->cfg.batch, h->ncls());
    launch_finalize_stage2(h->stream, h->bufs.scalars, h->mi_raw, h->cmi_raw,
                       h->coef2(), 1);
  }
  LAUNCH_CHECK();
  return MIMRL_OK;
}

int mimrl_probe_cube(mimrl_handle* h, const float* x, float* out, const float* dout, float* dx) {
  if (!h || !x || !out) return set_error(MIMRL_ERR_ARG, "null argument");
  if (!h->bound) return set_error(MIMRL_ERR_STATE, "mimrl_bind must be called first");
  if (dout && !dx) return set_error(MIMRL_ERR_ARG, "dout without dx");
  const mimrl_cfg& c = h->cfg;
  const int nb = c.n_blocks;
  const size_t nin = (size_t)c.batch * c.time_len * 3 * c.d_common;
  const size_t nout = (size_t)c.batch * c.d_outs[nb - 1][0] * c.d_outs[nb - 1][1] * c.d_outs[nb - 1][2];
  h->ev_next = 0;
  HIPX(hipMemcpyAsync(h->cube0, x, sizeof(float) * nin, hipMemcpyDeviceToDevice, h->stream));
  h->bf16 = h->bf16_fwd();
  MX(h->cube_forward(false, dout != nullptr));
  HIPX(hipMemcpyAsync(out, h->bb[nb - 1].d.z, sizeof(float) * nout, hipMemcpyDeviceToDevice, h->stream));
  if (!dout) return MIMRL_OK;
  if (nout > h->gbuf_floats) return set_error(MIMRL_ERR_STATE, "probe: gradient buffer too small");
  HIPX(hipMemsetAsync(h->bufs.main_g, 0, sizeof(float) * h->layout.floats[MIMRL_GROUP_MAIN], h->stream));
  HIPX(hipMemcpyAsync(h->gbuf[0], dout, sizeof(float) * nout, hipMemcpyDeviceToDevice, h->stream));
  int ci = 0, r;
  {
    Hold bwd(h->bf16, h->bf16_bwd());
    Hold in_place(h->wtT_prebuilt, false);
    h->deferred.clear();
    r = h->cube_backward(0, &ci);
    if (r == 0) r = h->flush_deferred();
  }
  h->kmix_pg_on_side3 = false;
  MX(r);
  MX(h->join(0, 5));
  HIPX(hipMemcpyAsync(dx, h->gbuf[ci], sizeof(float) * nin, hipMemcpyDeviceToDevice, h->stream));
  h->grads_clean[2] = false;
  return MIMRL_OK;
}

int mimrl_probe_encoders(mimrl_handle* h, float* cube_x, const float* dcube, const float* dmean) {
  if (!h || !cube_x) return set_error(MIMRL_ERR_ARG, "null argument");
  if (!h->bound) return set_error(MIMRL_ERR_STATE, "mimrl_bind must be called first");
  const mimrl_cfg& c = h->cfg;
  const size_t nin = (size_t)c.batch * c.time_len * 3 * c.d_common, nf = (size_t)c.batch * c.d_common;
  MX(h->ensure_images());
  h->ev_next = 0;
  h->bf16 = h->bf16_fwd();
  {
    Hold keep(h->keep_cube0, true);
    MX(h->model_forward(true, dcube != nullptr, 0, 0));
  }
  HIPX(hipMemcpyAsync(cube_x, h->cube0, sizeof(float) * nin, hipMemcpyDeviceToDevice, h->stream));
  if (!dcube) return MIMRL_OK;
  if (nin > h->gbuf_floats) return set_error(MIMRL_ERR_STATE, "probe: gradient buffer too small");
  HIPX(hipMemsetAsync(h->bufs.main_g, 0, sizeof(float) * h->layout.floats[MIMRL_GROUP_MAIN], h->stream));
  HIPX(hipMemcpyAsync(h->gbuf[0], dcube, sizeof(float) * nin, hipMemcpyDeviceToDevice, h->stream));
  if (dmean) HIPX(hipMemcpyAsync(h->dfeat + nf, dmean, sizeof(float) * 3 * nf, hipMemcpyDeviceToDevice, h->stream));
  else HIPX(hipMemsetAsync(h->dfeat, 0, sizeof(float) * 4 * nf, h->stream));
  h->deferred.clear();
  h->head_gather_on = false; h->ev_dmean = nullptr; h->kmix_pg_on_side3 = false;
  h->grads_clean[2] = false;
  Hold bwd(h->bf16, h->bf16_bwd());
  return h->encoders_backward(h->gbuf[0]);
}

int mimrl_probe_mi(mimrl_handle* h, int stage, float* mi, float* scores, float* dtin_out) {
  if (!h || !mi) return set_error(MIMRL_ERR_ARG, "null argument");
  if (!h->bound) return set_error(MIMRL_ERR_STATE, "mimrl_bind must be called first");
  if (stage != 1 && stage != 2) return set_error(MIMRL_ERR_ARG, "stage must be 1 or 2");
  const int B = h->cfg.batch;
  const bool bf_bwd = h->bf16_bwd();
  h->ev_next = 0;
  MX(h->ensure_images());
  h->imgT_ready = false;
  if (bf_bwd && h->fused_mlp && h->crit_imgT && h->ttab.n > 0) {
    MX(bf16_transposed_images(h->stream, h->bufs.crit_p, h->crit_imgT, h->ttab));
    h->imgT_ready = true;
  }
  if (stage == 1) HIPX(hipMemsetAsync(h->bufs.crit_g, 0, sizeof(float) * h->layout.floats[MIMRL_GROUP_CRITIC], h->stream));
  h->bf16 = h->bf16_fwd();
  MX(h->mi_forward(stage, true));
  {
    Hold bwd(h->bf16, bf_bwd);
    h->wg_helper = -1;
    MX(h->mi_backward(stage));
  }
  MX(h->join(0, 5));
  HIPX(hipMemcpyAsync(mi, h->mi_raw, sizeof(float) * 2 * NE_MI, hipMemcpyDeviceToDevice, h->stream));
  if (scores) {
    if (h->cfg.critic_type != MIMRL_CRITIC_CONCAT) return set_error(MIMRL_ERR_ARG, "probe: the separable fused path does not materialise scores");
    HIPX(hipMemcpyAsync(scores, h->scores, sizeof(float) * NE_MI * B * B, hipMemcpyDeviceToDevice, h->stream));
  }
  if (dtin_out) {
    if (stage != 2) return set_error(MIMRL_ERR_ARG, "probe: tower-input gradients exist in stage 2 only");
    HIPX(hipMemcpyAsync(dtin_out, h->dtin, sizeof(float) * 2 * NE_MI * B * EMB, hipMemcpyDeviceToDevice, h->stream));
  }
  if (stage == 1) h->grads_clean[1] = false;
  return MIMRL_OK;
}

int mimrl_probe_cmi(mimrl_handle* h, int stage, const float* cmi_in_, float* logits_out, float* vals, float* dcin_out) {
  if (!h || !cmi_in_ || !logits_out || !vals) return set_error(MIMRL_ERR_ARG, "null argument");
  if (!h->bound) return set_error(MIMRL_ERR_STATE, "mimrl_bind must be called first");
  if (stage != 1 && stage != 2) return set_error(MIMRL_ERR_ARG, "stage must be 1 or 2");
  const int n = h->nprod();
  const bool bf_bwd = h->bf16_bwd();
  h->ev_next = 0;
  MX(h->ensure_images());
  h->imgT_ready = false;
  if (bf_bwd && h->fused_mlp && h->crit_imgT && h->ttab.n > 0) {
    MX(bf16_transposed_images(h->stream, h->bufs.crit_p, h->crit_imgT, h->ttab));
    h->imgT_ready = true;
  }
  if (stage == 1) HIPX(hipMemsetAsync(h->bufs.crit_g, 0, sizeof(float) * h->layout.floats[MIMRL_GROUP_CRITIC], h->stream));
  HIPX(hipMemcpyAsync(h->cmi_in, cmi_in_, sizeof(float) * NE_CMI * 2 * n * 384, hipMemcpyDeviceToDevice, h->stream));
  h->bf16 = h->bf16_fwd();
  const int cdims[5] = {3 * EMB, HID, HID, HID, 2};
  MX(h->mlp_stack_forward(NE_CMI, 2 * n, 2 * n, h->cmi0, h->cmi_stride, 4, h->cmi_l, cdims, h->cmi_in, h->cc, h->logits));
  MX(cmi_loss_fwd_bwd(h->stream, h->logits, h->dlogits, h->bce_raw, h->cmi_raw, h->g_bce(stage), h->g_cmi(stage), NE_CMI, n, h->cfg.cmi_hardtanh));
  {
    Hold bwd(h->bf16, bf_bwd);
    h->wg_helper = -1;
    MX(h->cmi_backward(stage));
  }
  MX(h->join(0, 5));
  HIPX(hipMemcpyAsync(logits_out, h->logits, sizeof(float) * NE_CMI * 2 * n * 2, hipMemcpyDeviceToDevice, h->stream));
  HIPX(hipMemcpyAsync(vals, h->bce_raw, sizeof(float) * NE_CMI, hipMemcpyDeviceToDevice, h->stream));
  HIPX(hipMemcpyAsync(vals + NE_CMI, h->cmi_raw, sizeof(float) * NE_CMI, hipMemcpyDeviceToDevice, h->stream));
  if (dcin_out) {
    if (stage != 2) return set_error(MIMRL_ERR_ARG, "probe: classifier-input gradients exist in stage 2 only");
    HIPX(hipMemcpyAsync(dcin_out, h->dcin, sizeof(float) * NE_CMI * 2 * n * 384, hipMemcpyDeviceToDevice, h->stream));
  }
  if (stage == 1) h->grads_clean[1] = false;
  return MIMRL_OK;
}

int mimrl_set_kernel_stamps(mimrl_handle* h, unsigned long long* ring, int slots) {
  if (!h) return set_error(MIMRL_ERR_ARG, "null handle");
  if (ring && (slots < 1 || (slots & (slots - 1)))) return set_error(MIMRL_ERR_ARG, "stamp ring: slots must be a power of two");
  h->kstamp.ring = ring; h->kstamp.step = h->d_ints; h->kstamp.slots = ring ? slots : 0;
  h->drop_graphs();
  return MIMRL_OK;
}

int mimrl_profile_enable(mimrl_handle* h, int on) {
  if (!h) return set_error(MIMRL_ERR_ARG, "null handle");
  h->prof_on = on != 0;
  return MIMRL_OK;
}

int mimrl_profile_read(mimrl_handle* h, float* ms_sum, int32_t* launches) {
  if (!h || !ms_sum || !launches) return set_error(MIMRL_ERR_ARG, "null argument");
  HIPX(hipStreamSynchronize(h->stream));
  for (int p = 0; p < MIMRL_NPHASES; ++p) {
    double acc = 0.0;
    for (auto& ev : h->prof_ev[p]) {
      float ms = 0.f;
      HIPX(hipEventElapsedTime(&ms, ev.first, ev.second));
      acc += ms;
      h->prof_pool.push_back(ev);
    }
    ms_sum[p] = (float)acc;
    launches[p] = (int32_t)h->prof_ev[p].size();
    h->prof_ev[p].clear();
  }
  return MIMRL_OK;
}

int mimrl_profile_read_gemm(mimrl_handle* h, double out[4]) {
  if (!h || !out) return set_error(MIMRL_ERR_ARG, "null argument");
  HIPX(hipStreamSynchronize(h->stream));
  HIPX(hipDeviceSynchronize());
  out[0] = out[1] = out[2] = 0.0; out[3] = (double)h->prof_gemm.size();
  for (auto& g : h->prof_gemm) {
    float ms = 0.f;
    HIPX(hipEventElapsedTime(&ms, g.a, g.b));
    out[0] += g.flops; out[1] += g.bytes; out[2] += ms;
    h->prof_pool.push_back({g.a, g.b});
  }
  h->prof_gemm.clear();
  return MIMRL_OK;
}

int mimrl_params_changed(mimrl_handle* h) {
  if (!h) return set_error(MIMRL_ERR_ARG, "null handle");
  h->img_valid = false;
  h->imgT_valid = false;
  return MIMRL_OK;
}

int mimrl_set_knn_override_mask(mimrl_handle* h, int stage, unsigned call_mask) {
  if (!h || (stage != 1 && stage != 2)) return set_error(MIMRL_ERR_ARG, "bad handle / stage");
  if (call_mask && !h->bufs.knn_override) return set_error(MIMRL_ERR_STATE, "mimrl_buffers.knn_override is not bound");
  if (h->knn_ovr_mask[stage - 1] == (call_mask & 63u)) return MIMRL_OK;
  HIPX(hipStreamSynchronize(h->user_stream));
  h->drop_graphs();
  h->knn_ovr_mask[stage - 1] = call_mask & 63u;
  return MIMRL_OK;
}

int mimrl_stage2_forward_tail(mimrl_handle* h) { return h ? h->run_fwd2_tail() : set_error(MIMRL_ERR_ARG, "null handle"); }

int mimrl_set_grad_scale(mimrl_handle* h, float scale) {
  if (!h) return set_error(MIMRL_ERR_ARG, "null handle");
  if (scale == h->grad_scale) return MIMRL_OK;
  HIPX(hipStreamSynchronize(h->user_stream));
  h->drop_graphs();
  h->grad_scale = scale;
  return MIMRL_OK;
}

int mimrl_comm_unique_id(void* out128) { return mimrl::comm_unique_id(out128); }

int mimrl_set_comm(mimrl_handle* h, const void* unique_id128, int world, int rank) {
  if (!h) return set_error(MIMRL_ERR_ARG, "null handle");
  HIPX(hipStreamSynchronize(h->user_stream));
  h->drop_graphs();
  if (h->comm) { MX(mimrl::comm_destroy(h->comm)); h->comm = nullptr; }
  h->comm_world = 1; h->comm_rank = 0;
  if (!unique_id128) return MIMRL_OK;
  MX(mimrl::comm_init(&h->comm, unique_id128, world, rank));
  h->comm_world = world; h->comm_rank = rank;
  if (!h->comm_s) HIPX(hipStreamCreateWithFlags(&h->comm_s, hipStreamNonBlocking));
  const char* sp = knob("MIMRL_DDP_SPLIT");
  h->comm_split = !(sp && sp[0] == '0');
  if (h->bound) {
    HIPX(hipMemsetAsync(h->bufs.scalars, 0, sizeof(float), h->user_stream));
    MX(mimrl::comm_allreduce_sum(h->comm, h->bufs.scalars, 1, h->user_stream));
    MX(mimrl::comm_allreduce_sum(h->comm, h->bufs.scalars, 1, h->comm_s));
    HIPX(hipStreamSynchronize(h->user_stream)); HIPX(hipStreamSynchronize(h->comm_s));
  }
  return MIMRL_OK;
}

int mimrl_set_comm_critic_bf16(mimrl_handle* h, int on) {
  if (!h) return set_error(MIMRL_ERR_ARG, "null handle");
  if ((on != 0) == h->comm_crit_bf16) return MIMRL_OK;
  HIPX(hipStreamSynchronize(h->user_stream));
  h->drop_graphs();
  if (on && !h->comm_crit16) HIPX(hipMalloc(&h->comm_crit16, sizeof(uint16_t) * (size_t)h->layout.floats[MIMRL_GROUP_CRITIC]));
  h->comm_crit_bf16 = on != 0;
  if (on && h->comm && h->bound) {
    HIPX(hipMemsetAsync(h->comm_crit16, 0, 16, h->user_stream));
    MX(mimrl::comm_allreduce_sum_bf16(h->comm, h->comm_crit16, 8, h->user_stream));
    HIPX(hipStreamSynchronize(h->user_stream));
  }
  return MIMRL_OK;
}

int mimrl_set_task_loss(mimrl_handle* h, int kind) {
  if (!h) return set_error(MIMRL_ERR_ARG, "null handle");
  if (kind < MIMRL_TASK_LOSS_MAE || kind > MIMRL_TASK_LOSS_CCC) return set_error(MIMRL_ERR_ARG, "task loss kind %d unknown", kind);
  if (h->ncls() >= 2) return set_error(MIMRL_ERR_ARG, "a regression task loss needs the one-output head (num_class %d)", h->cfg.num_class);
  if (kind == h->task_loss) return MIMRL_OK;
  HIPX(hipStreamSynchronize(h->user_stream));
  h->drop_graphs();
  h->task_loss = kind;
  return MIMRL_OK;
}

int mimrl_set_class_loss(mimrl_handle* h, int kind) {
  if (!h) return set_error(MIMRL_ERR_ARG, "null handle");
  if (kind < MIMRL_CLASS_LOSS_CE || kind > MIMRL_CLASS_LOSS_BCE) return set_error(MIMRL_ERR_ARG, "classification loss kind %d unknown", kind);
  if (kind != MIMRL_CLASS_LOSS_BCE && h->ncls() < 2) return set_error(MIMRL_ERR_ARG, "CE / Focal need num_class >= 2 (got %d)", h->cfg.num_class);
  if (kind == MIMRL_CLASS_LOSS_BCE && h->ncls() > 2) return set_error(MIMRL_ERR_ARG, "BCE needs num_class 1 or 2 (got %d; Solver.py:327-337)", h->cfg.num_class);
  if (kind == h->task_loss) return MIMRL_OK;
  HIPX(hipStreamSynchronize(h->user_stream));
  h->drop_graphs();
  h->task_loss = kind;
  return MIMRL_OK;
}

int64_t mimrl_main_late_offset(const mimrl_handle* h) { return h ? (int64_t)h->layout.late_offset : 0; }

int mimrl_set_stage2_prefetch(mimrl_handle* h, int on) {
  if (!h) return set_error(MIMRL_ERR_ARG, "null handle");
#ifdef MIMRL_DET
  on = 0;
#endif
  if ((on != 0) == h->prefetch && (on == 2) == h->defer_tail) return MIMRL_OK;
  if (on && !h->pre_stream) HIPX(hipStreamCreateWithFlags(&h->pre_stream, hipStreamNonBlocking));
  HIPX(hipStreamSynchronize(h->user_stream));
  h->drop_graphs();
  h->prefetch = on != 0;
  h->defer_tail = on == 2;
  h->fwd2_pending = false;
  h->tail2_needed = false;
  return MIMRL_OK;
}

int64_t mimrl_workspace_bytes(const mimrl_handle* h) { return h ? (int64_t)h->ws_bytes : 0; }

void mimrl_destroy(mimrl_handle* h) {
  if (!h) return;
  h->drop_graphs();
  for (auto g : h->retired) (void)hipGraphExecDestroy(g);
  h->retired.clear();
  for (int p = 0; p < MIMRL_NPHASES; ++p)
    for (auto& ev : h->prof_ev[p]) h->prof_pool.push_back(ev);
  for (auto& g : h->prof_gemm) h->prof_pool.push_back({g.a, g.b});
  for (auto& ev : h->prof_pool) { (void)hipEventDestroy(ev.first); (void)hipEventDestroy(ev.second); }
  for (int i = 0; i < mimrl_handle::NSIDE; ++i)
    if (h->side[i]) (void)hipStreamDestroy(h->side[i]);
  for (auto e : h->ev_pool) (void)hipEventDestroy(e);
  if (h->cap_stream) (void)hipStreamDestroy(h->cap_stream);
  if (h->pre_stream) (void)hipStreamDestroy(h->pre_stream);
  if (h->comm) (void)mimrl::comm_destroy(h->comm);
  if (h->comm_s) (void)hipStreamDestroy(h->comm_s);
  if (h->comm_crit16) (void)hipFree(h->comm_crit16);
  if (h->ws) (void)hipFree(h->ws);
  delete h;
}

int mimrl_op_gemm(void* stream, const float* A, const float* B, float* C, int M, int N, int K, int batch,
                  const int64_t st[9], const float* bias_n, const float* bias_m, float alpha, float beta, int act,
                  int precision) {
  if (!st) return set_error(MIMRL_ERR_ARG, "null strides");
  GemmDesc d;
  d.A = A; d.B = B; d.C = C; d.M = M; d.N = N; d.K = K; d.batch = batch;
  d.sa_m = st[0]; d.sa_k = st[1]; d.sa_b = st[2]; d.sb_k = st[3]; d.sb_n = st[4]; d.sb_b = st[5];
  d.sc_m = st[6]; d.sc_n = st[7]; d.sc_b = st[8];
  d.bias_n = bias_n; d.bias_m = bias_m; d.alpha = alpha; d.beta = beta; d.act = act & 0xff;
  d.atomic = (act >> 8) & 1;
  return gemm(reinterpret_cast<hipStream_t>(stream), d, (precision & 1) != 0);
}

int mimrl_op_gemm_ex(void* stream, const float* A, const float* B, float* C, int M, int N, int K, int batch, const int64_t st[9],
                     const float* A2, const float* B2, int K2, const int64_t st2[6], int a_gap_at, int a_gap_rows, const float* bias_n,
                     const float* gradact_u, float* colsum, int act, int precision) {
  if (!st || (A2 && !st2)) return set_error(MIMRL_ERR_ARG, "null strides");
  GemmDesc d;
  d.A = A; d.B = B; d.C = C; d.M = M; d.N = N; d.K = K; d.batch = batch;
  d.sa_m = st[0]; d.sa_k = st[1]; d.sa_b = st[2]; d.sb_k = st[3]; d.sb_n = st[4]; d.sb_b = st[5];
  d.sc_m = st[6]; d.sc_n = st[7]; d.sc_b = st[8];
  if (A2) {
    d.A2 = A2; d.B2 = B2; d.K2 = K2;
    d.sa2_m = st2[0]; d.sa2_k = st2[1]; d.sa2_b = st2[2]; d.sb2_k = st2[3]; d.sb2_n = st2[4]; d.sb2_b = st2[5];
  }
  d.a_gap_at = a_gap_at; d.a_gap_rows = a_gap_rows;
  d.bias_n = bias_n; d.gradact_u = gradact_u; d.colsum = colsum; d.act = act & 0xff; d.atomic = (act >> 8) & 1;
  return gemm(reinterpret_cast<hipStream_t>(stream), d, (precision & 1) != 0);
}

int mimrl_op_gemm16(void* stream, const void* A, const void* B, void* C, int M, int N, int K, int batch, const int64_t st[9],
                    const void* A2, const void* B2, int K2, const int64_t st2[6], int batch_in, const int64_t st_bo[5],
                    const float* bias_n, int flags) {
  if (!st || (A2 && !st2) || (batch_in > 0 && !st_bo)) return set_error(MIMRL_ERR_ARG, "null strides");
  if (batch_in < 0 || (batch_in > 0 && batch % batch_in != 0)) return set_error(MIMRL_ERR_ARG, "batch_in must divide batch");
  GemmDesc d;
  d.A = static_cast<const float*>(A); d.B = static_cast<const float*>(B); d.C = static_cast<float*>(C);
  d.M = M; d.N = N; d.K = K; d.batch = batch;
  d.sa_m = st[0]; d.sa_k = st[1]; d.sa_b = st[2]; d.sb_k = st[3]; d.sb_n = st[4]; d.sb_b = st[5];
  d.sc_m = st[6]; d.sc_n = st[7]; d.sc_b = st[8];
  if (A2) {
    d.A2 = static_cast<const float*>(A2); d.B2 = static_cast<const float*>(B2); d.K2 = K2;
    d.sa2_m = st2[0]; d.sa2_k = st2[1]; d.sa2_b = st2[2]; d.sb2_k = st2[3]; d.sb2_n = st2[4]; d.sb2_b = st2[5];
  }
  if (batch_in > 0) { d.batch_in = batch_in; d.sa_bo = st_bo[0]; d.sb_bo = st_bo[1]; d.sc_bo = st_bo[2]; d.bias_n_bo = st_bo[3]; }
  if (st_bo) d.bias_n_b = st_bo[4];
  d.bias_n = bias_n;
  d.a_bf16 = flags & 1; d.b_bf16 = (flags >> 1) & 1; d.f16 = (flags >> 2) & 1; d.c_f16 = (flags >> 3) & 1; d.atomic = (flags >> 4) & 1;
  if (flags >> 8) { d.a_gap_at = (flags >> 8) & 0xfff; d.a_gap_rows = (flags >> 20) & 0xfff; }
  return gemm(reinterpret_cast<hipStream_t>(stream), d, true);
}

int mimrl_op_gemm_wgrad_group(void* stream, int n, const float* const* A, const float* const* B, float* const* C, const int32_t* dims,
                              const int64_t* st, int precision) {
  if (n <= 0 || n > 12 || !A || !B || !C || !dims || !st) return set_error(MIMRL_ERR_ARG, "gemm_wgrad_group: 1..12 problems");
  GemmDesc d[12];
  for (int i = 0; i < n; ++i) {
    d[i].A = A[i]; d[i].B = B[i]; d[i].C = C[i];
    d[i].M = dims[4 * i]; d[i].N = dims[4 * i + 1]; d[i].K = dims[4 * i + 2]; d[i].batch = dims[4 * i + 3];
    const int64_t* q = st + 9 * i;
    d[i].sa_m = q[0]; d[i].sa_k = q[1]; d[i].sa_b = q[2]; d[i].sb_k = q[3]; d[i].sb_n = q[4]; d[i].sb_b = q[5];
    d[i].sc_m = q[6]; d[i].sc_n = q[7]; d[i].sc_b = q[8];
    d[i].atomic = 1;
  }
  return gemm_group_splitk(reinterpret_cast<hipStream_t>(stream), d, n, (precision & 1) != 0);
}

int64_t mimrl_op_gru_saved_floats(int B, int T) { return gru_saved_floats(B, T); }

int mimrl_op_gru_forward(void* stream, const float* gx_f, const float* gx_r, const float* whh_f, const float* whh_r,
                         const float* bhh_f, const float* bhh_r, const int32_t* lens, float* out, float* saved_f,
                         float* saved_r, int B, int T, int precision) {
  GruFwdArgs a;
  std::memset(&a, 0, sizeof a);
  a.B = B; a.T = T; a.out_ld = 2 * H; a.nmod = 1; a.btv = gru_pick_btv(B, 1);
  a.lens[0] = lens; a.lens[1] = lens;
  a.seq[0][0] = GruSeq{gx_f, whh_f, bhh_f, out, saved_f};
  a.seq[0][1] = GruSeq{gx_r, whh_r, bhh_r, out, saved_r};
  return gru_forward(reinterpret_cast<hipStream_t>(stream), a, (precision & 1) != 0);
}

int mimrl_op_gru_backward(void* stream, const float* whh_f, const float* whh_r, const float* saved_f,
                          const float* saved_r, const int32_t* lens, const float* out, const float* dout, float* dg_f,
                          float* dg_r, float* hprev_f, float* hprev_r, int B, int T, int precision) {
  GruBwdArgs a;
  std::memset(&a, 0, sizeof a);
  a.B = B; a.T = T; a.out_ld = 2 * H; a.dout_ld = 2 * H; a.dout_off = H; a.nmod = 1; a.btv = gru_pick_btv(B, 1);
  a.lens[0] = lens; a.lens[1] = lens;
  a.seq[0][0] = GruSeqBwd{whh_f, saved_f, out, dout, dg_f, hprev_f, nullptr, nullptr};
  a.seq[0][1] = GruSeqBwd{whh_r, saved_r, out, dout, dg_r, hprev_r, nullptr, nullptr};
  return gru_backward(reinterpret_cast<hipStream_t>(stream), a, (precision & 1) != 0);
}

int mimrl_op_recur_btv(int B, int nmod) {
  if (B < 1 || nmod < 1 || nmod > 2) return set_error(MIMRL_ERR_ARG, "mimrl_op_recur_btv: B >= 1, nmod 1 or 2");
  const int g = gru_pick_btv(B, nmod), l = lstm_btv(B, nmod);
  if (g != l) return set_error(MIMRL_ERR_STATE, "mimrl_op_recur_btv: the GRU (%d) and LSTM (%d) picks differ: give this entry point an encoder argument", g, l);
  return g;
}

int mimrl_op_lstm_forward(void* stream, const float* gx_f, const float* gx_r, const float* whh_f, const float* whh_r,
                          const float* bhh_f, const float* bhh_r, const int32_t* lens, float* out, float* saved_f,
                          float* saved_r, int B, int T, int kernel) {
  if (!gx_f || !gx_r || !whh_f || !whh_r || !bhh_f || !bhh_r || !lens || !out) return set_error(MIMRL_ERR_ARG, "mimrl_op_lstm_forward: null argument");
  if ((saved_f != nullptr) != (saved_r != nullptr)) return set_error(MIMRL_ERR_ARG, "mimrl_op_lstm_forward: both saved records or neither");
  LstmFwdArgs a;
  std::memset(&a, 0, sizeof a);
  a.B = B; a.T = T; a.out_ld = 2 * H; a.nmod = 1;
  a.lens[0] = lens; a.lens[1] = lens;
  a.seq[0][0] = LstmSeq{gx_f, whh_f, bhh_f, out, saved_f};
  a.seq[0][1] = LstmSeq{gx_r, whh_r, bhh_r, out, saved_r};
  return lstm_forward_kernels(reinterpret_cast<hipStream_t>(stream), a, kernel);
}

int mimrl_op_lstm_backward(void* stream, const float* whh_f, const float* whh_r, const float* saved_f,
                           const float* saved_r, const int32_t* lens, const float* out, const float* dout, float* dg_f,
                           float* dg_r, float* hprev_f, float* hprev_r, int B, int T, int kernel) {
  if (!whh_f || !whh_r || !saved_f || !saved_r || !lens || !out || !dout || !dg_f || !dg_r || !hprev_f || !hprev_r)
    return set_error(MIMRL_ERR_ARG, "mimrl_op_lstm_backward: null argument");
  LstmBwdArgs a;
  std::memset(&a, 0, sizeof a);
  a.B = B; a.T = T; a.out_ld = 2 * H; a.dout_ld = 2 * H; a.nmod = 1;
  a.lens[0] = lens; a.lens[1] = lens;
  a.seq[0][0] = LstmSeqBwd{whh_f, saved_f, out, dout, dg_f, hprev_f};
  a.seq[0][1] = LstmSeqBwd{whh_r, saved_r, out, dout + H, dg_r, hprev_r};
  return lstm_backward_kernels(reinterpret_cast<hipStream_t>(stream), a, kernel);
}

int mimrl_op_concat_dw(void* stream, const void* dz2, const void* a1, float* dw2, const void* dz1, const void* a0, float* dw1, int E, int64_t rows,
                       int64_t dw_stride, const float* ds, const void* a2h, float* dw3, const uint32_t* m2, const float* w3, const float* P,
                       const float* Q, int B) {
  if ((!dz2 && !m2) || !a1 || !dw2) return set_error(MIMRL_ERR_ARG, "mimrl_op_concat_dw: null argument");
  if ((dz1 != nullptr) != (a0 != nullptr || P != nullptr) || (dz1 != nullptr) != (dw1 != nullptr)) return set_error(MIMRL_ERR_ARG, "mimrl_op_concat_dw: the second layer comes as a set");
  if (!concat_dw_ok(E, rows, 256)) return set_error(MIMRL_ERR_ARG, "mimrl_op_concat_dw: E >= 1, rows >= 1");
  ConcatDwArgs a;
  a.dz[0] = static_cast<const __bf16*>(dz2); a.act[0] = static_cast<const __bf16*>(a1); a.dw[0] = dw2;
  a.dz[1] = static_cast<const __bf16*>(dz1); a.act[1] = static_cast<const __bf16*>(a0); a.dw[1] = dw1;
  a.nlayer = dz1 ? 2 : 1; a.E = E; a.rows = rows; a.dw_stride = dw_stride;
  a.ds = ds; a.a2 = static_cast<const _Float16*>(a2h); a.dw3 = dw3; a.m2 = m2; a.w3 = w3; a.P = P; a.Q = Q; a.B = B;
  return concat_dw(reinterpret_cast<hipStream_t>(stream), a);
}

int mimrl_op_gru_wgrad(void* stream, const void* const* dg, const void* const* x, const void* const* hp, float* const* dw_ih,
                       float* const* dw_hh, int64_t rows, int kp) {
  if (!dg || !x || !hp || !dw_ih || !dw_hh) return set_error(MIMRL_ERR_ARG, "mimrl_op_gru_wgrad: null argument");
  GruWgradArgs a;
  for (int s = 0; s < 4; ++s) {
    if (!dg[s] || !x[s] || !hp[s] || !dw_ih[s] || !dw_hh[s]) return set_error(MIMRL_ERR_ARG, "mimrl_op_gru_wgrad: null array for sequence %d", s);
    a.seq[s] = GruWgradSeq{static_cast<const __bf16*>(dg[s]), static_cast<const __bf16*>(x[s]), static_cast<const __bf16*>(hp[s]), dw_ih[s], dw_hh[s]};
  }
  a.rows = rows; a.kp = kp;
  return gru_wgrad(reinterpret_cast<hipStream_t>(stream), a);
}

int mimrl_op_mi_bound(void* stream, const float* scores, float* dscores, float* mi, const float* gscale, int E, int B,
                      int bound) {
  return mi_bound_fwd_bwd(reinterpret_cast<hipStream_t>(stream), scores, dscores, mi, nullptr, gscale, E, B, bound, 0u);
}
int mimrl_op_mi_bound_baseline(void* stream, float* scores, float* dscores, float* mi, const float* gscale, const float* lb,
                               float* dlb, int E, int B, int bound) {
  return mi_bound_fwd_bwd(reinterpret_cast<hipStream_t>(stream), scores, dscores, mi, nullptr, gscale, E, B, bound, 0u, lb, dlb, B);
}
int mimrl_op_mi_bound_ex(void* stream, const float* scores, float* dscores, float* mi, float* mi_loss, const float* gscale,
                         int E, int B, int bound, uint32_t lossform) {
  return mi_bound_fwd_bwd(reinterpret_cast<hipStream_t>(stream), scores, dscores, mi, mi_loss, gscale, E, B, bound, lossform);
}

int mimrl_op_mi_infonce_rows(void* stream, const float* scores, float* dscores, float* mi, float* mi_loss, const float* gscale,
                             int E, int B, float* ws) {
  static_assert(MIMRL_NCE_WS_FLOATS >= NCE_WS_WIDE_FLOATS && NCE_WS_WIDE_FLOATS >= NCE_WS_FLOATS, "MIMRL_NCE_WS_FLOATS too small");
  if (!scores || !mi || !ws || E < 1 || E > 16) return set_error(MIMRL_ERR_ARG, "mi_infonce_rows: null array or E = %d outside [1, 16]", E);
  return mi_bound_fwd_bwd(reinterpret_cast<hipStream_t>(stream), scores, dscores, mi, mi_loss, gscale, E, B, BOUND_INFONCE, 0u, nullptr,
                          nullptr, 0, ws);
}
int mimrl_op_mi_sep_infonce(void* stream, const float* tout, float* dtout, float* mi, float* mi_loss, const float* gscale, int E,
                            int B, int tiled) {
  hipStream_t st = reinterpret_cast<hipStream_t>(stream);
  if (!tiled) return mi_sep_fused(st, tout, dtout, mi, mi_loss, gscale, E, B, BOUND_INFONCE, 0x1fu, dtout ? 1 : 0);
  return mi_sep_nce_tiled(st, tout, dtout, mi, mi_loss, gscale, E, B, dtout ? 1 : 0);
}

int mimrl_op_knn(void* stream, const float* Z, int dz, int N, const int32_t* anchors, int m, int k, int32_t* idx_out) {
  KnnArgs a;
  std::memset(&a, 0, sizeof a);
  a.call[0] = KnnCall{Z, dz, anchors, idx_out};
  a.N = N; a.m = m; a.k = k; a.ncall = 1;
  return knn_sample(reinterpret_cast<hipStream_t>(stream), a);
}

int mimrl_probe_knn(mimrl_handle* h, int stage, int32_t* idx_out) {
  if (!h || !idx_out) return set_error(MIMRL_ERR_ARG, "mimrl_probe_knn: null argument");
  if (stage != 1 && stage != 2) return set_error(MIMRL_ERR_ARG, "stage must be 1 or 2");
  HIPX(hipMemcpyAsync(idx_out, stage == 2 ? h->knn_idx2 : h->knn_idx, sizeof(int32_t) * NE_CMI * h->nprod(), hipMemcpyDeviceToDevice, h->user_stream));
  return MIMRL_OK;
}

int mimrl_op_sample_anchors(void* stream, int32_t* anchors_out, int ncall, int m, int N, uint64_t seed, const int32_t* step,
                            uint32_t stream_id, int step_add) {
  if (!anchors_out || !step || ncall < 1 || ncall > KNN_MAX_CALLS) return set_error(MIMRL_ERR_ARG, "mimrl_op_sample_anchors: bad argument");
  AnchorDraws d;
  d.n = ncall;
  for (int c = 0; c < ncall; ++c) { d.out[c] = anchors_out + (size_t)c * m; d.call[c] = c; d.stream_id[c] = stream_id; d.step_add[c] = step_add; }
  return sample_anchors(reinterpret_cast<hipStream_t>(stream), d, m, N, (uint32_t)seed, (uint32_t)(seed >> 32), step);
}

int mimrl_op_cmi_loss(void* stream, const float* logits, float* dlogits, float* bce, float* cmi, const float* g_bce,
                      const float* g_cmi, int E, int n, int hardtanh) {
  return cmi_loss_fwd_bwd(reinterpret_cast<hipStream_t>(stream), logits, dlogits, bce, cmi, g_bce, g_cmi, E, n, hardtanh);
}

int mimrl_op_task_loss(void* stream, int kind, const float* pred, const float* y, float* dpred, float* loss, int B) {
  if (!pred || !y || !loss) return set_error(MIMRL_ERR_ARG, "task_loss: null argument");
  if (kind < MIMRL_TASK_LOSS_MAE || kind > MIMRL_TASK_LOSS_CCC) return set_error(MIMRL_ERR_ARG, "task loss kind %d unknown", kind);
  if (B < 1 || B > 1024) return set_error(MIMRL_ERR_ARG, "task_loss: batch %d outside [1, 1024]", B);
  launch_task_loss(reinterpret_cast<hipStream_t>(stream), kind, pred, y, dpred, loss, B);
  LAUNCH_CHECK();
  return MIMRL_OK;
}

int mimrl_op_class_loss(void* stream, int kind, const float* logits, const float* y, float* dlogits, float* loss, int B, int C) {
  if (!logits || !y || !loss) return set_error(MIMRL_ERR_ARG, "class_loss: null argument");
  if (kind < MIMRL_CLASS_LOSS_CE || kind > MIMRL_CLASS_LOSS_BCE) return set_error(MIMRL_ERR_ARG, "classification loss kind %d unknown", kind);
  if (B < 1 || B > 1024) return set_error(MIMRL_ERR_ARG, "class_loss: batch %d outside [1, 1024]", B);
  if (C < 1 || C > MIMRL_MAX_CLASSES) return set_error(MIMRL_ERR_ARG, "class_loss: %d classes outside [1, %d]", C, MIMRL_MAX_CLASSES);
  if (kind != MIMRL_CLASS_LOSS_BCE && C < 2) return set_error(MIMRL_ERR_ARG, "class_loss: CE / Focal need at least 2 classes");
  if (kind == MIMRL_CLASS_LOSS_BCE && C > 2) return set_error(MIMRL_ERR_ARG, "class_loss: BCE takes 1 or 2 classes (got %d)", C);
  launch_task_loss(reinterpret_cast<hipStream_t>(stream), kind, logits, y, dlogits, loss, B, C);
  LAUNCH_CHECK();
  return MIMRL_OK;
}

static int fill_mlp_args(MlpFusedArgs* fa, int nb, int rows, int brows, int nl, const int32_t* dims, const float* const* W,
                         int64_t pstride) {
  if (!dims || !W || nl < 1 || nl > MLPF_MAX_LAYERS) return set_error(MIMRL_ERR_ARG, "mlp_stack: bad arguments");
  std::memset(fa, 0, sizeof *fa);
  fa->nb = nb; fa->rows = rows; fa->brows = brows; fa->nl = nl; fa->pstride = pstride;
  for (int l = 0; l <= nl; ++l) fa->dims[l] = dims[l];
  for (int l = 0; l < nl; ++l) fa->W[l] = W[l];
  return MIMRL_OK;
}

int mimrl_op_mlp_stack_forward(void* stream, int nb, int rows, int brows, int nl, const int32_t* dims, const float* const* W,
                               const float* const* b, int64_t pstride, const float* in, float* const* act, float* out) {
  MlpFusedArgs fa;
  MX(fill_mlp_args(&fa, nb, rows, brows, nl, dims, W, pstride));
  if (!b || !in || !out || (nl > 1 && !act)) return set_error(MIMRL_ERR_ARG, "mlp_stack_forward: null argument");
  for (int l = 0; l < nl; ++l) { fa.b[l] = b[l]; if (l < nl - 1) fa.act[l] = act[l]; }
  fa.in = in; fa.out = out;
  return mlp_stack_fwd_fused(reinterpret_cast<hipStream_t>(stream), fa);
}

int mimrl_op_mlp_stack_backward(void* stream, int nb, int rows, int brows, int nl, const int32_t* dims, const float* const* W,
                                int64_t pstride, const float* const* act, const float* dout, float* const* dz, float* din,
                                float* const* db) {
  MlpFusedArgs fa;
  MX(fill_mlp_args(&fa, nb, rows, brows, nl, dims, W, pstride));
  if (!dout || (nl > 1 && (!act || !dz))) return set_error(MIMRL_ERR_ARG, "mlp_stack_backward: null argument");
  for (int l = 0; l < nl - 1; ++l) { fa.act[l] = const_cast<float*>(act[l]); fa.dz[l + 1] = dz[l + 1]; fa.db[l] = db ? db[l] : nullptr; }
  fa.dout = dout; fa.din = din;
  return mlp_stack_bwd_fused(reinterpret_cast<hipStream_t>(stream), fa);
}

int mimrl_op_adam(void* stream, float* p, float* g, float* m, float* v, int64_t n, const float* lr, const int32_t* step,
                  float beta1, float beta2, float eps, float weight_decay, float clip) {
  AdamArgs a;
  a.p = p; a.g = g; a.m = m; a.v = v; a.n = n; a.lr = lr; a.step = step;
  a.beta1 = beta1; a.beta2 = beta2; a.eps = eps; a.weight_decay = weight_decay; a.clip = clip;
  return adam_step(reinterpret_cast<hipStream_t>(stream), a);
}

}
```

mimrl_amd/csrc/engine_backward.hip:

```cpp
#include "engine.h"

int mimrl_handle::cube_backward(int cur_in, int* cur_out) {
  const int B = cfg.batch;
  int dims[MIMRL_MAX_BLOCKS + 1][3];
  dims[0][0] = cfg.time_len; dims[0][1] = 3; dims[0][2] = cfg.d_common;
  for (int i = 0; i < cfg.n_blocks; ++i)
    for (int ax = 0; ax < 3; ++ax) dims[i + 1][ax] = cfg.d_outs[i][ax];
  const int per_block = 7 + (cfg.dropout_mlp[0] > 0.f) + (cfg.dropout_mlp[2] > 0.f);
  const bool defer = multi_stream && !cfg.ln_first && per_block * cfg.n_blocks + 1 <= NGBUF;
  const int npool = defer ? NGBUF : 4;
  int used[NGBUF] = {0};
  used[cur_in] = 1;
  int cur = cur_in;
  auto grab = [&]() { for (int q = 0; q < npool; ++q) if (!used[q]) { used[q] = 1; return q; } return -1; };
  auto release = [&](int q) { if (!defer) used[q] = 0; };
  auto W_gemm = [&](int sd, const GemmDesc& g) -> int {
    if (defer) { deferred.push_back(Deferred{0, sd, g, nullptr, 0, 0, 0, 0, nullptr}); return MIMRL_OK; }
    return G_on(S(sd), g);
  };
  auto W_colsum = [&](int sd, const float* src, long rows, int cols, int ld, float* dst) -> int {
    if (defer) { deferred.push_back(Deferred{1, sd, GemmDesc(), src, rows, cols, ld, 0, dst}); return MIMRL_OK; }
    return colsum(S(sd), src, rows, cols, ld, dst);
  };
  auto W_rowsum = [&](int sd, const float* src, int nb, int rows, int cols, float* dst) -> int {
    if (defer) { deferred.push_back(Deferred{2, sd, GemmDesc(), src, nb, rows, cols, 0, dst}); return MIMRL_OK; }
    return rowsum_batched(S(sd), src, nb, rows, cols, dst);
  };
  auto W_lnpar = [&](int sd, const float* y, const float* mean, const float* rstd, const float* dz, float* dgam, float* dbet,
                     int nb, int n, int cols) -> int {
    if (defer) {
      Deferred d{3, sd, GemmDesc(), y, nb, n, cols, 0, dgam};
      d.p1 = mean; d.p2 = rstd; d.p3 = dz; d.dst2 = dbet;
      deferred.push_back(d);
      return MIMRL_OK;
    }
    return colln_param_grads(S(sd), y, mean, rstd, dz, dgam, dbet, nb, n, cols);
  };
  auto W_dpg = [&](int sd, const float* y, const float* mean, const float* rstd, const float* dz, const float* dy, const float* du,
                   float* dgam, float* dbet, float* db2, float* db1, long rows) -> int {
    if (defer) {
      Deferred d{6, sd, GemmDesc(), y, rows, 0, 0, 0, dgam};
      d.p1 = mean; d.p2 = rstd; d.p3 = dz; d.p4 = dy; d.p5 = du; d.dst2 = dbet; d.dst3 = db2; d.dst4 = db1;
      deferred.push_back(d);
      return MIMRL_OK;
    }
    return daxis_param_grads(S(sd), y, mean, rstd, dz, dy, du, dgam, dbet, db2, db1, rows);
  };
  auto W_fork = [&](int lo, int hi) -> int { return defer ? MIMRL_OK : fork(lo, hi); };
  bool d_fused[MIMRL_MAX_BLOCKS] = {};
  MX(wt_images(stream, bf16, !(wtT_prebuilt && wtT_built), d_fused));
  auto W_join = [&](int lo, int hi) -> int { return defer ? MIMRL_OK : join(lo, hi); };
#define GRAB(var)                                                                                   \
  const int var = grab();                                                                           \
  if (var < 0) return set_error(MIMRL_ERR_STATE, "cube_backward: out of gradient buffers (line %d)", __LINE__)

  for (int i = cfg.n_blocks - 1; i >= 0; --i) {
    const BlockW& w = blk[i];
    BlockBuf& b = bb[i];
    const int il = dims[i][0], ik = dims[i][1], id = dims[i][2];
    const int hl = w.ax[0].hid, ol = w.ax[0].out, hk = w.ax[1].hid, ok = w.ax[1].out, hd = w.ax[2].hid, od = w.ax[2].out;
    const float* xblk = i == 0 ? cube0 : bb[i - 1].d.z;
    const float pl = cfg.dropout_mlp[0], pk = cfg.dropout_mlp[1], pd = cfg.dropout_mlp[2];
    if (d_fused[i]) {
      const AxisW& a = w.ax[2];
      const long R2 = (long)B * ol * ok;
      GRAB(i_dy); GRAB(i_du); GRAB(i_dx);
      DAxisBwdArgs fa;
      fa.dz = gbuf[cur]; fa.y = b.d.y; fa.mean = b.d.mean; fa.rstd = b.d.rstd; fa.gamma = P(a.ln_g); fa.u = b.d.u;
      fa.w2t = wtT[i][0]; fa.w1t = wtT[i][1]; fa.wrt = wtT[i][2];
      fa.dy = gbuf[i_dy]; fa.du = gbuf[i_du]; fa.dx = gbuf[i_dx];
      fa.R = R2; fa.act = cfg.activation;
      fa.dgamma = fa.dbeta = fa.db2 = fa.db1 = nullptr;
      MX(daxis_bwd_fused(stream, fa));
      MX(W_fork(1, 3));
      MX(W_dpg(2, b.d.y, b.d.mean, b.d.rstd, gbuf[cur], gbuf[i_dy], gbuf[i_du], Gm(a.ln_g), Gm(a.ln_b),
               a.fc2.b >= 0 ? Gm(a.fc2.b) : nullptr, a.fc1.b >= 0 ? Gm(a.fc1.b) : nullptr, R2));
      { GemmDesc g = gemm_tn(gbuf[i_dy], od, b.d.h, hd, Gm(a.fc2.w), hd, od, hd, (int)R2); g.atomic = 1; MX(W_gemm(1, g)); }
      { GemmDesc g = gemm_tn(gbuf[i_dy], od, b.k.z, id, Gm(a.res), id, od, id, (int)R2); g.atomic = 1; MX(W_gemm(2, g)); }
      { GemmDesc g = gemm_tn(gbuf[i_du], hd, b.k.z, id, Gm(a.fc1.w), id, hd, id, (int)R2); g.atomic = 1; MX(W_gemm(3, g)); }
      MX(W_join(1, 3));
      release(cur); release(i_dy); release(i_du);
      cur = i_dx;
    } else {
      const AxisW& a = w.ax[2];
      const long R2 = (long)B * ol * ok;
      const float* xin = b.k.z;
      const float* xmlp = cfg.ln_first ? b.d.xn : b.k.z;
      int i_dy = cur;
      if (!cfg.ln_first) {
        GRAB(q);
        MX(rowln_bwd(stream, b.d.y, P(a.ln_g), b.d.mean, b.d.rstd, gbuf[cur], gbuf[q], Gm(a.ln_g), Gm(a.ln_b), R2, od));
        release(cur);
        i_dy = q;
      }
      const float* dy = gbuf[i_dy];
      int i_dym = i_dy;
      if (pd > 0.f) {
        GRAB(q);
        HIPX(hipMemcpyAsync(gbuf[q], dy, sizeof(float) * R2 * od, hipMemcpyDeviceToDevice, stream));
        MX(dropout_inplace(stream, gbuf[q], R2 * od, pd, key(), 12 + 3 * i));
        i_dym = q;
      }
      const float* dym = gbuf[i_dym];
      MX(W_fork(1, 2));
      { GemmDesc g = gemm_tn(dym, od, b.d.h, hd, Gm(a.fc2.w), hd, od, hd, (int)R2); g.atomic = 1; MX(W_gemm(1, g)); }
      if (a.fc2.b >= 0) MX(W_colsum(1, dym, R2, od, od, Gm(a.fc2.b)));
      if (a.res >= 0) { GemmDesc g = gemm_tn(dy, od, xin, id, Gm(a.res), id, od, id, (int)R2); g.atomic = 1; MX(W_gemm(2, g)); }
      GRAB(i_du);
      { GemmDesc g = gemm_nn(dym, od, P(a.fc2.w), hd, gbuf[i_du], hd, (int)R2, hd, od); g.act = cfg.activation; g.gradact_u = b.d.u;
        if (a.fc1.b >= 0) g.colsum = Gm(a.fc1.b);
        MX(G_(g)); }
      MX(W_fork(3, 3));
      { GemmDesc g = gemm_tn(gbuf[i_du], hd, xmlp, id, Gm(a.fc1.w), id, hd, id, (int)R2); g.atomic = 1; MX(W_gemm(3, g)); }
      GRAB(i_dx0);
      int i_dx = i_dx0;
      const bool fuse_dx = a.res >= 0 && !cfg.ln_first;
      { GemmDesc g = gemm_nn(gbuf[i_du], hd, P(a.fc1.w), id, gbuf[i_dx], id, (int)R2, id, hd);
        if (fuse_dx) { g.A2 = dy; g.sa2_m = od; g.sa2_k = 1; g.B2 = P(a.res); g.sb2_k = id; g.sb2_n = 1; g.K2 = od; }
        MX(G_(g)); }
      if (cfg.ln_first) {
        MX(join(3, 3));
        MX(rowln_bwd(stream, b.k.z, P(a.ln_g), b.d.xn_mean, b.d.xn_rstd, gbuf[i_dx], gbuf[i_du], Gm(a.ln_g), Gm(a.ln_b), R2, id));
        release(i_dx);
        i_dx = i_du;
      } else {
        release(i_du);
      }
      if (!fuse_dx) {
        if (a.res >= 0) { GemmDesc g = gemm_nn(dy, od, P(a.res), id, gbuf[i_dx], id, (int)R2, id, od); g.beta = 1.f; MX(G_(g)); }
        else MX(add_inplace(stream, gbuf[i_dx], dy, R2 * id));
      }
      MX(W_join(1, 3));
      if (i_dym != i_dy) release(i_dym);
      release(i_dy);
      cur = i_dx;
    }
    {
      const AxisW& a = w.ax[1];
      KMixW kw;
      std::memset(&kw, 0, sizeof kw);
      kw.w1 = P(a.fc1.w); kw.b1 = a.fc1.b >= 0 ? P(a.fc1.b) : nullptr;
      kw.w2 = P(a.fc2.w); kw.b2 = a.fc2.b >= 0 ? P(a.fc2.b) : nullptr;
      kw.wr = a.res >= 0 ? P(a.res) : nullptr; kw.g = P(a.ln_g); kw.be = P(a.ln_b);
      kw.dw1 = Gm(a.fc1.w); kw.db1 = a.fc1.b >= 0 ? Gm(a.fc1.b) : nullptr;
      kw.dw2 = Gm(a.fc2.w); kw.db2 = a.fc2.b >= 0 ? Gm(a.fc2.b) : nullptr;
      kw.dwr = a.res >= 0 ? Gm(a.res) : nullptr; kw.dg = Gm(a.ln_g); kw.dbe = Gm(a.ln_b);
      kw.ik = ik; kw.hk = hk; kw.ok = ok; kw.act = cfg.activation; kw.ln_first = cfg.ln_first;
      kw.drop_p = pk; kw.key = key(); kw.stream_id = 11 + 3 * i;
      GRAB(q);
      static const int kmix_inchain = dbg_env("MIMRL_KMIX_PG_INCHAIN") ? atoi(dbg_env("MIMRL_KMIX_PG_INCHAIN")) : 1;
      if (defer && kmix_inchain) {
        MX(kmix_bwd(stream, b.l.z, gbuf[cur], gbuf[q], kw, (long)B * ol, id));
      } else if (defer) {
        MX(kmix_bwd_part(stream, b.l.z, gbuf[cur], gbuf[q], kw, (long)B * ol, id, 1));
        static const int kdbg = dbg_env("MIMRL_DBG_KMIX") ? atoi(dbg_env("MIMRL_DBG_KMIX")) : 0;
        static const bool kmix_park = dbg_env("MIMRL_KMIX_PG_PARKED") != nullptr;
        if (kmix_park) {
          Deferred d{5, 2, GemmDesc(), b.l.z, (long)B * ol, id, 0, 0, nullptr};
          d.p3 = gbuf[cur]; d.kw = kw; d.kw.dbg = kdbg;
          deferred.push_back(d);
        } else {
          KMixW kp = kw; kp.dbg = kdbg;
          MX(fork(3, 3));
          MX(kmix_bwd_part(S(3), b.l.z, gbuf[cur], nullptr, kp, (long)B * ol, id, 2));
          kmix_pg_on_side3 = true;
        }
      } else {
        MX(kmix_bwd(stream, b.l.z, gbuf[cur], gbuf[q], kw, (long)B * ol, id));
      }
      release(cur);
      cur = q;
    }
    if (bf16 && fused_cube_bwd && !cfg.ln_first && pl <= 0.f && w.ax[0].res >= 0 && laxis_bwd_supported(il, hl, ol, ik * id) &&
        (il <= 64 || laxis_bwd_long_on)) {
      const AxisW& a = w.ax[0];
      const long C = (long)ik * id;
      GRAB(i_dy); GRAB(i_du); GRAB(i_dx);
      LAxisBwdArgs fa;
      fa.dz = gbuf[cur]; fa.y = b.l.y; fa.mean = b.l.mean; fa.rstd = b.l.rstd; fa.gamma = P(a.ln_g); fa.u = b.l.u;
      fa.w2 = P(a.fc2.w); fa.w1 = P(a.fc1.w); fa.wr = P(a.res);
      fa.dy = gbuf[i_dy]; fa.du = gbuf[i_du]; fa.dx = gbuf[i_dx];
      fa.db2 = a.fc2.b >= 0 ? Gm(a.fc2.b) : nullptr; fa.db1 = a.fc1.b >= 0 ? Gm(a.fc1.b) : nullptr;
      fa.B = B; fa.il = il; fa.hl = hl; fa.ol = ol; fa.C = (int)C; fa.act = cfg.activation;
      MX(laxis_bwd_fused(stream, fa));
      MX(W_fork(1, 3));
      MX(W_lnpar(1, b.l.y, b.l.mean, b.l.rstd, gbuf[cur], Gm(a.ln_g), Gm(a.ln_b), B, ol, (int)C));
      release(cur);
      { GemmDesc g; g.A = gbuf[i_dy]; g.sa_m = C; g.sa_k = 1; g.sa_b = (long)ol * C;
        g.B = b.l.h; g.sb_k = 1; g.sb_n = C; g.sb_b = (long)hl * C;
        g.C = Gm(a.fc2.w); g.sc_m = hl; g.sc_n = 1; g.sc_b = 0; g.M = ol; g.N = hl; g.K = (int)C; g.batch = B; g.atomic = 1;
        MX(W_gemm(1, g)); }
      { GemmDesc g; g.A = gbuf[i_dy]; g.sa_m = C; g.sa_k = 1; g.sa_b = (long)ol * C;
        g.B = xblk; g.sb_k = 1; g.sb_n = C; g.sb_b = (long)il * C;
        g.C = Gm(a.res); g.sc_m = il; g.sc_n = 1; g.sc_b = 0; g.M = ol; g.N = il; g.K = (int)C; g.batch = B; g.atomic = 1;
        MX(W_gemm(2, g)); }
      { GemmDesc g; g.A = gbuf[i_du]; g.sa_m = C; g.sa_k = 1; g.sa_b = (long)hl * C;
        g.B = xblk; g.sb_k = 1; g.sb_n = C; g.sb_b = (long)il * C;
        g.C = Gm(a.fc1.w); g.sc_m = il; g.sc_n = 1; g.sc_b = 0; g.M = hl; g.N = il; g.K = (int)C; g.batch = B; g.atomic = 1;
        MX(W_gemm(3, g)); }
      MX(W_join(1, 3));
      release(i_dy); release(i_du);
      cur = i_dx;
    } else {
      const AxisW& a = w.ax[0];
      const long C = (long)ik * id;
      const float* xmlp = cfg.ln_first ? b.l.xn : xblk;
      int i_dy = cur;
      if (!cfg.ln_first) {
        GRAB(q);
        MX(colln_bwd(stream, b.l.y, P(a.ln_g), b.l.mean, b.l.rstd, gbuf[cur], gbuf[q], Gm(a.ln_g), Gm(a.ln_b), B, ol, (int)C));
        release(cur);
        i_dy = q;
      }
      const float* dy = gbuf[i_dy];
      int i_dym = i_dy;
      if (pl > 0.f) {
        GRAB(q);
        HIPX(hipMemcpyAsync(gbuf[q], dy, sizeof(float) * B * ol * C, hipMemcpyDeviceToDevice, stream));
        MX(dropout_inplace(stream, gbuf[q], (long)B * ol * C, pl, key(), 10 + 3 * i));
        i_dym = q;
      }
      const float* dym = gbuf[i_dym];
      MX(W_fork(1, 2));
      { GemmDesc g; g.A = dym; g.sa_m = C; g.sa_k = 1; g.sa_b = (long)ol * C;
        g.B = b.l.h; g.sb_k = 1; g.sb_n = C; g.sb_b = (long)hl * C;
        g.C = Gm(a.fc2.w); g.sc_m = hl; g.sc_n = 1; g.sc_b = 0; g.M = ol; g.N = hl; g.K = (int)C; g.batch = B; g.atomic = 1;
        MX(W_gemm(1, g)); }
      if (a.fc2.b >= 0) MX(W_rowsum(1, dym, B, ol, (int)C, Gm(a.fc2.b)));
      if (a.res >= 0) {
        GemmDesc g; g.A = dy; g.sa_m = C; g.sa_k = 1; g.sa_b = (long)ol * C;
        g.B = xblk; g.sb_k = 1; g.sb_n = C; g.sb_b = (long)il * C;
        g.C = Gm(a.res); g.sc_m = il; g.sc_n = 1; g.sc_b = 0; g.M = ol; g.N = il; g.K = (int)C; g.batch = B; g.atomic = 1;
        MX(W_gemm(2, g));
      }
      GRAB(i_du);
      { GemmDesc g; g.A = P(a.fc2.w); g.sa_m = 1; g.sa_k = hl; g.sa_b = 0;
        if (bf16 && w2p[i] && w2p_valid[i] && hl % 4 != 0) { g.A = w2p[i]; g.sa_k = (hl + 3) & ~3; g.a_pad4 = 1; }
        g.B = dym; g.sb_k = C; g.sb_n = 1; g.sb_b = (long)ol * C;
        g.C = gbuf[i_du]; g.sc_m = C; g.sc_n = 1; g.sc_b = (long)hl * C; g.M = hl; g.N = (int)C; g.K = ol; g.batch = B;
        g.act = cfg.activation; g.gradact_u = b.l.u;
        MX(G_(g)); }
      MX(W_fork(3, 3));
      { GemmDesc g; g.A = gbuf[i_du]; g.sa_m = C; g.sa_k = 1; g.sa_b = (long)hl * C;
        g.B = xmlp; g.sb_k = 1; g.sb_n = C; g.sb_b = (long)il * C;
        g.C = Gm(a.fc1.w); g.sc_m = il; g.sc_n = 1; g.sc_b = 0; g.M = hl; g.N = il; g.K = (int)C; g.batch = B; g.atomic = 1;
        MX(W_gemm(3, g)); }
      if (a.fc1.b >= 0) MX(W_rowsum(3, gbuf[i_du], B, hl, (int)C, Gm(a.fc1.b)));
      GRAB(i_dx0);
      int i_dx = i_dx0;
      { GemmDesc g; g.A = P(a.fc1.w); g.sa_m = 1; g.sa_k = il; g.sa_b = 0;
        g.B = gbuf[i_du]; g.sb_k = C; g.sb_n = 1; g.sb_b = (long)hl * C;
        g.C = gbuf[i_dx]; g.sc_m = C; g.sc_n = 1; g.sc_b = (long)il * C; g.M = il; g.N = (int)C; g.K = hl; g.batch = B;
        if (a.res >= 0 && !cfg.ln_first) {
          g.A2 = P(a.res); g.sa2_m = 1; g.sa2_k = il; g.sa2_b = 0;
          g.B2 = dy; g.sb2_k = C; g.sb2_n = 1; g.sb2_b = (long)ol * C; g.K2 = ol;
        }
        MX(G_(g)); }
      if (cfg.ln_first) {
        MX(join(3, 3));
        MX(colln_bwd(stream, xblk, P(a.ln_g), b.l.xn_mean, b.l.xn_rstd, gbuf[i_dx], gbuf[i_du], Gm(a.ln_g), Gm(a.ln_b), B, il, (int)C));
        release(i_dx);
        i_dx = i_du;
      } else {
        release(i_du);
      }
      if (a.res >= 0 && !cfg.ln_first) {
      } else if (a.res >= 0) {
        GemmDesc g; g.A = P(a.res); g.sa_m = 1; g.sa_k = il; g.sa_b = 0;
        g.B = dy; g.sb_k = C; g.sb_n = 1; g.sb_b = (long)ol * C;
        g.C = gbuf[i_dx]; g.sc_m = C; g.sc_n = 1; g.sc_b = (long)il * C; g.M = il; g.N = (int)C; g.K = ol; g.batch = B; g.beta = 1.f;
        MX(G_(g));
      } else {
        MX(add_inplace(stream, gbuf[i_dx], dy, (long)B * il * C));
      }
      MX(W_join(1, 3));
      if (i_dym != i_dy) release(i_dym);
      release(i_dy);
      cur = i_dx;
    }
    static const int early = dbg_env("MIMRL_EARLY_FLUSH") ? atoi(dbg_env("MIMRL_EARLY_FLUSH")) : 2;
    if (defer && (early == 2 || (early == 1 && i == cfg.n_blocks - 1))) MX(flush_deferred(1));
  }
#undef GRAB
  *cur_out = cur;
  return MIMRL_OK;
}

__global__ void dbg_spin_kernel(long ticks) {
  const long t0 = wall_clock64();
  while (wall_clock64() - t0 < ticks) __builtin_amdgcn_s_sleep(16);
}
int mimrl_handle::dbg_delay(hipStream_t st, int tag) {
  static const char* spec = knob("MIMRL_DBG_DELAY_TAG");
  static const int want = spec ? atoi(spec) : -1;
  static const int us = spec && strchr(spec, ':') ? atoi(strchr(spec, ':') + 1) : 50;
  if (tag != want) return MIMRL_OK;
  hipLaunchKernelGGL(dbg_spin_kernel, dim3(1), dim3(64), 0, st, (long)us * 100);
  LAUNCH_CHECK();
  return MIMRL_OK;
}

int mimrl_handle::flush_deferred(int only_side) {
  if (deferred.empty()) return MIMRL_OK;
  if (only_side > 0) MX(fork(only_side, only_side)); else MX(fork(1, 3));
  for (int q = 1; q <= 3; ++q) MX(dbg_delay(S(q), 9));
  constexpr int wg_sides = 3;
  static const int dbg_skip_kinds = dbg_env("MIMRL_DBG_SKIP_DEFERRED") ? atoi(dbg_env("MIMRL_DBG_SKIP_DEFERRED")) : 0;
  const bool groupk = !prof_on && bf16 && !((dbg_skip_kinds >> 0) & 1) && cfg.seq_len <= 128;
  if (groupk) {
    std::vector<GemmDesc> cls[2];
    for (const Deferred& d : deferred) if (d.kind == 0) cls[d.g.sa_k == 1 ? 0 : 1].push_back(d.g);
    for (int c = 0; c < 2; ++c) {
      hipStream_t st = only_side > 0 ? S(only_side) : S(1 + c % wg_sides);
      for (size_t i = 0; i < cls[c].size(); i += 12) MX(gemm_group_splitk(st, cls[c].data() + i, (int)std::min<size_t>(12, cls[c].size() - i), bf16));
    }
  }
  int rr = 2;
  for (const Deferred& d : deferred) {
    if ((dbg_skip_kinds >> d.kind) & 1) continue;
    if (groupk && d.kind == 0) continue;
    static const bool dbg_defer_main = dbg_env("MIMRL_DBG_DEFER_MAIN") != nullptr;
    hipStream_t st = dbg_defer_main ? stream : only_side > 0 ? S(only_side) : S(1 + (groupk ? rr++ : d.side - 1) % wg_sides);
    if (d.kind == 0) MX(G_on(st, d.g));
    else if (d.kind == 1) MX(colsum(st, d.src, d.n0, (int)d.n1, (int)d.n2, d.dst));
    else if (d.kind == 2) MX(rowsum_batched(st, d.src, (int)d.n0, (int)d.n1, (int)d.n2, d.dst));
    else if (d.kind == 3) MX(colln_param_grads(st, d.src, d.p1, d.p2, d.p3, d.dst, d.dst2, (int)d.n0, (int)d.n1, (int)d.n2));
    else if (d.kind == 6) MX(daxis_param_grads(st, d.src, d.p1, d.p2, d.p3, d.p4, d.p5, d.dst, d.dst2, d.dst3, d.dst4, d.n0));
    else MX(kmix_bwd_part(st, d.src, d.p3, nullptr, d.kw, d.n0, (int)d.n1, 2));
  }
  deferred.clear();
  return MIMRL_OK;
}

int mimrl_handle::model_backward() {
  Range rg("mimrl.model_backward");
  DetDefer det_defer(stream, &det_ranges);
  const int B = cfg.batch, T = cfg.seq_len, L = cfg.time_len, D = cfg.d_common;
  const long BT_ = (long)B * T;
  const int nb = cfg.n_blocks;
  const int ol = cfg.d_outs[nb - 1][0], ok = cfg.d_outs[nb - 1][1], od = cfg.d_outs[nb - 1][2];
  MX(head_bwd(stream, dfeat, dpred, P(cls_w), bufs.feats, gbuf[0], Gm(cls_w), Gm(cls_b), B, ol, ok, od,
              cfg.compose_t_sum, cfg.compose_k_sum, head_gather_on ? &head_gather : nullptr, ncls()));
  int ci = 0;
  deferred.clear();
  { Scope sc(this, MIMRL_PH_CUBE_BWD); MX(cube_backward(0, &ci)); }
  MX(dbg_delay(stream, 7));
  return encoders_backward(gbuf[ci]);
}

int mimrl_handle::encoders_backward(float* dcube) {
  const int B = cfg.batch, T = cfg.seq_len, L = cfg.time_len, D = cfg.d_common;
  const long BT_ = (long)B * T;
  const float* dmean = dfeat + (size_t)B * D;
  if (head_gather_on && ev_dmean) { HIPX(hipStreamWaitEvent(stream, ev_dmean, 0)); ev_dmean = nullptr; }
  {
    LnSide2 sd[2];
    for (int m = 0; m < 2; ++m)
      sd[m] = LnSide2{h1[m], P(ln_g[m]), P(ln_b[m]), ln_mean[m], ln_rstd[m], ds[m], Gm(ln_g[m]), Gm(ln_b[m]), 1 + m,
                      cfg.dropout[1 + m], (uint32_t)(1 + m)};
    ds_bf16_live = rec16_on && cfg.encoder == MIMRL_ENCODER_GRU && dg_bf16 && (prec & MIMRL_PREC_BF16_GRU_BWD) != 0 && gru_bwd_io16_ok(0);
    MX(ln_relu_drop_bwd2(stream, sd[0], sd[1], dcube, B, T, L, 3, D, key(), dmean + (size_t)B * D, dmean + 2 * (size_t)B * D, ds_bf16_live ? 1 : 0));
  }
  MX(fork(0, 0));
  MX(text_post_bwd(S(0), dcube, dtx, B, T, L, 3, D, 0, cfg.dropout[0], key(), 0, dmean));
  { GemmDesc g = gemm_tn(dtx, D, bufs.text, cfg.d_t, Gm(w_t), cfg.d_t, D, cfg.d_t, (int)BT_); g.atomic = 1; MX(G_on(S(0), g)); }
  static const int dbg_join_at = dbg_env("MIMRL_DBG_JOIN_AT") ? atoi(dbg_env("MIMRL_DBG_JOIN_AT")) : 0;
  MX(flush_deferred());
  if (dbg_join_at == 1) MX(join(1, 3));
  if (cfg.encoder != MIMRL_ENCODER_GRU) kmix_pg_on_side3 = false;
  if (cfg.encoder == MIMRL_ENCODER_CONV) {
    MX(conv_backward());
    MX(join(0, 5));
    return MIMRL_OK;
  }
  if (cfg.encoder == MIMRL_ENCODER_LSTM) {
    MX(lstm_encoders_backward());
    MX(join(0, 5));
    return MIMRL_OK;
  }
  if (kmix_pg_on_side3) { MX(join(3, 3)); kmix_pg_on_side3 = false; }
  MX(gru_layer_backward(1));
  if (split_part == 1) return join(0, 5);
  MX(gru_layer_backward(0));
  return join(0, 5);
}

int mimrl_handle::gru_layer_backward(int l) {
  const int B = cfg.batch, T = cfg.seq_len;
  const long BT_ = (long)B * T;
  static const int dbg_join_at = dbg_env("MIMRL_DBG_JOIN_AT") ? atoi(dbg_env("MIMRL_DBG_JOIN_AT")) : 0;
  const float* xin[2] = {bufs.audio, bufs.video};
  {
    GruBwdArgs a;
    a.B = B; a.T = T; a.out_ld = 2 * H; a.nmod = 2;
    a.dout_ld = l == 1 ? H : 2 * H; a.dout_off = l == 1 ? 0 : H;
    a.btv = gru_pick_btv(B, 2);
    a.stamp = kstamp; a.stamp.id = l == 1 ? 2 : 3;
    const bool lbf = dg_bf16 && (l == 1 || l0_packed || l0_bwd_pack);
    a.dg_bf16 = lbf ? 1 : 0;
    a.slab_upl = l == 0 && l0_xin ? 2 : 0;
    const bool io16 = lbf && (prec & MIMRL_PREC_BF16_GRU_BWD) != 0 && gru_bwd_io16_ok(a.slab_upl);
    a.dout_bf16 = io16 && (l == 1 ? ds_bf16_live : dh0_bf16_live) ? 1 : 0;
    if ((l == 1 ? ds_bf16_live : dh0_bf16_live) && !a.dout_bf16) return set_error(MIMRL_ERR_STATE, "gru_layer_backward: dout was stored as bf16 but this BPTT launch cannot read it");
    const bool hp16 = l == 0 && io16 && hp16_live && h0h[0] && h0h[1];
    if (l == 0 && hp16_live && !hp16) return set_error(MIMRL_ERR_STATE, "gru_layer_backward: the forward pass counted on the fp16 h_prev path");
    for (int m = 0; m < 2; ++m) {
      a.lens[m] = lens[m];
      for (int d = 0; d < 2; ++d) {
        const GruDirW& g = gru[m][l][d];
        a.seq[m][d] = GruSeqBwd{P(g.w_hh), sv[l][m][d], l == 1 ? h1[m] : h0[m], l == 1 ? ds[m] : dh0[m], dg[l][m][d],
                                hprev[l][m][d], Gm(g.b_ih), Gm(g.b_hh)};
        if (hp16) a.seq[m][d].out16 = h0h[m];
      }
    }
    { Scope sc(this, MIMRL_PH_GRU_BWD); MX(gru_backward(stream, a, (prec & MIMRL_PREC_BF16_GRU_BWD) != 0)); }
    if ((l == 1 && dbg_join_at == 2) || (l == 0 && dbg_join_at == 4)) MX(join(1, 3));
    MX(dbg_delay(stream, 8));
    constexpr int l0_side = 1;
    MX(fork(1, l == 0 ? 5 : 3));
    if (l == 1) {
      dh0_bf16_live = false;
      {
        GemmDesc q = gemm_nn(dg[l][0][0], 4 * H, P(gru[0][l][0].w_ih), 2 * H, dh0[0], 2 * H, (int)BT_, 2 * H, G);
        q.A2 = dg[l][0][1]; q.sa2_m = 4 * H; q.sa2_k = 1;
        q.B2 = P(gru[0][l][1].w_ih); q.sb2_k = 2 * H; q.sb2_n = 1; q.K2 = G;
        q.batch = 2;
        q.sa_b = dg[l][1][0] - dg[l][0][0]; q.sa2_b = dg[l][1][1] - dg[l][0][1];
        q.sb_b = gru[1][l][0].w_ih - gru[0][l][0].w_ih; q.sb2_b = gru[1][l][1].w_ih - gru[0][l][1].w_ih;
        q.sc_b = dh0[1] - dh0[0];
        if (lbf) { q.a_bf16 = 1; q.sa_b *= 2; q.sa2_b *= 2; }
        if (lbf && w1_img_valid && h16_on && w1b) {
          q.B = reinterpret_cast<const float*>(w1b); q.B2 = reinterpret_cast<const float*>(w1b + (long)G * 2 * H);
          q.b_bf16 = 1; q.sb_b = 2L * G * 2 * H; q.sb2_b = 2L * G * 2 * H;
          if (w1bt) {
            GemmDesc t = q;
            t.B = reinterpret_cast<const float*>(w1bt); t.B2 = reinterpret_cast<const float*>(w1bt + G);
            t.sb_k = 1; t.sb_n = 2 * G; t.sb2_k = 1; t.sb2_n = 2 * G; t.sb_b = 2L * H * 2 * G; t.sb2_b = 2L * H * 2 * G;
            if (gemm_tall_ok(t)) {
              q = t;
              if (rec16_on && (prec & MIMRL_PREC_BF16_GRU_BWD) != 0 && (l0_packed || l0_bwd_pack) && gru_bwd_io16_ok(l0_xin ? 2 : 0)) { q.c_bf16 = 1; q.sc_b *= 2; dh0_bf16_live = true; }
            }
          }
        }
        MX(G_(q));
      }
    }
    if (l == 1 && dbg_join_at == 3) MX(join(1, 3));
    if (l == 0 && (l0_packed || l0_bwd_pack)) {
      const long s_dg = dg[0][0][1] - dg[0][0][0], o_dg = dg[0][1][0] - dg[0][0][0];
      const long s_hp = hprev[0][0][1] - hprev[0][0][0], o_hp = hprev[0][1][0] - hprev[0][0][0];
      static const bool wgrad_on = knob("MIMRL_NO_GRU_WGRAD") == nullptr;
      const bool one_pass = wgrad_on && lbf && xpack16 && BT_ >= 32768 && gru_wgrad_ok(BT_, KP());
      if (one_pass) {
        GruWgradArgs w;
        const __bf16* xb = reinterpret_cast<const __bf16*>(xpack + BT_ * KP());
        for (int m = 0; m < 2; ++m)
          for (int d = 0; d < 2; ++d)
            w.seq[m * 2 + d] = GruWgradSeq{reinterpret_cast<const __bf16*>(dg[0][m][d]), xb + (long)m * BT_ * KP(),
                                           reinterpret_cast<const __bf16*>(hprev[0][m][d]), dwih_pack + (long)(m * 2 + d) * G * KP(),
                                           dwhh_pack + (long)(m * 2 + d) * G * H};
        w.rows = BT_; w.kp = KP();
        MX(gru_wgrad(stream, w));
      } else {
      { GemmDesc q = gemm_tn(dg[0][0][0], 4 * H, xpack, KP(), dwih_pack, KP(), G, KP(), (int)BT_);
        q.batch = 4; q.batch_in = 2; q.sa_b = s_dg; q.sa_bo = o_dg; q.sb_b = 0; q.sb_bo = BT_ * KP(); q.sc_b = (long)G * KP(); q.sc_bo = 2L * G * KP();
        if (lbf) { q.a_bf16 = 1; q.sa_b *= 2; q.sa_bo *= 2; }
        if (lbf && xpack16) { q.B = reinterpret_cast<const float*>(reinterpret_cast<const __bf16*>(xpack + BT_ * KP())); q.b_bf16 = 1; }
        q.atomic = 1; MX(G_on(stream, q)); }
      { GemmDesc q = gemm_tn(dg[0][0][0], 4 * H, hprev[0][0][0], H, dwhh_pack, H, G, H, (int)BT_);
        q.a_gap_at = 2 * H; q.a_gap_rows = H;
        q.batch = 4; q.batch_in = 2; q.sa_b = s_dg; q.sa_bo = o_dg; q.sb_b = s_hp; q.sb_bo = o_hp; q.sc_b = (long)G * H; q.sc_bo = 2L * G * H;
        if (lbf) { q.a_bf16 = q.b_bf16 = 1; q.sa_b *= 2; q.sa_bo *= 2; q.sb_b *= 2; q.sb_bo *= 2; }
        q.atomic = 1; MX(G_on(S(l0_side), q)); }
      MX(join(l0_side, l0_side));
      }
      L0Unpack up;
      for (int m = 0; m < 2; ++m) {
        up.d[m] = gru[m][0][0].din;
        for (int d = 0; d < 2; ++d) { up.g_ih[m][d] = Gm(gru[m][0][d].w_ih); up.g_hh[m][d] = Gm(gru[m][0][d].w_hh); }
      }
      up.dwih_pack = dwih_pack; up.dwhh_pack = dwhh_pack; up.KP = KP();
// ... 57 lines not shown
```

mimrl_amd/engine.py:

```python
from __future__ import annotations

import ctypes as C
import os
from typing import Dict, Optional

import numpy as np
import torch

from . import _lib
from ._lib import Buffers, MimrlError, check
from .data import Rows


_ROW_MEAN_LOSSES = (_lib.TASK_LOSSES["MAE"], _lib.TASK_LOSSES["MSE"], _lib.CLASS_LOSSES["CE"], _lib.CLASS_LOSSES["BCE"])


def _ptr(t: Optional[torch.Tensor]):
    return None if t is None else C.c_void_p(t.data_ptr())


class HipEngine:

    def __init__(self, opt, d_t: int, d_a: int, d_v: int, seq_len: Optional[int] = None, bank_capacity: int = 0,
                 precision: str = "fp32", use_graph: bool = False, seed: int = 0, device: Optional[torch.device] = None,
                 device_anchors: bool = False, share: Optional["HipEngine"] = None, batch: Optional[int] = None):
        if not torch.cuda.is_available():
            raise MimrlError("HipEngine needs a ROCm GPU (torch.cuda.is_available() is False); there is no CPU fallback")
        self.lib = _lib.load()
        self.device = torch.device(device if device is not None else f"cuda:{torch.cuda.current_device()}")
        torch.cuda.set_device(self.device)
        self.opt = opt
        if share is not None:
            bank_capacity = share.cfg.bank_capacity
        self.cfg = _lib.make_cfg(opt, d_t, d_a, d_v, seq_len, bank_capacity, precision, use_graph, seed, device_anchors, batch=batch)
        self.precision = precision
        check(self.lib.mimrl_device_check())
        self.entries, (n_main, n_crit) = _lib.layout_entries(self.cfg)
        f32 = dict(dtype=torch.float32, device=self.device)
        B, T = self.cfg.batch, self.cfg.seq_len
        self.m_anchor = B // self.cfg.k_neighbor
        z = lambda *s: torch.zeros(*s, **f32)
        self.shared = share is not None
        self.main = share.main if share else {k: z(max(n_main, 1)) for k in "pgmv"}
        self.crit = share.crit if share else {k: z(max(n_crit, 1)) for k in "pgmv"}
        if share and (share.main["p"].numel() != max(n_main, 1) or share.crit["p"].numel() != max(n_crit, 1)):
            raise MimrlError("engines that share buckets must have the same parameter layout")
        self.text, self.audio, self.video = z(B, T, d_t), z(B, T, d_a), z(B, T, d_v)
        self.labels = z(B)
        cap = max(int(bank_capacity), 1)
        self.bank = share.bank if share else {"C": z(cap, 1), "F": z(cap, 128), "T": z(cap, 128), "A": z(cap, 128), "V": z(cap, 128)}
        self.anchors = torch.zeros(2, 6, max(self.m_anchor, 1), dtype=torch.int32, device=self.device)
        self.knn_override = torch.zeros(2, 6, max(self.m_anchor * self.cfg.k_neighbor, 1), dtype=torch.int32, device=self.device)
        self._ovr_mask = [0, 0]
        self.bank_c_host = share.bank_c_host if share else None
        self.lr_main = share.lr_main if share else torch.full((1,), float(opt.learning_rate), **f32)
        self.lr_critic = share.lr_critic if share else torch.full((1,), float(opt.learning_rate) * float(opt.mi_lr_rate), **f32)
        self.counters = share.counters if share else torch.zeros(4, dtype=torch.int32, device=self.device)
        self.num_class = max(int(self.cfg.num_class), 1)
        self.pred = z(B) if self.num_class == 1 else z(B, self.num_class)
        self.feats = z(4, B, 128)
        self.scalars = z(_lib.NSCALARS)
        self.bank_rows = 0
        self.params: Dict[str, torch.Tensor] = {}
        self.grads: Dict[str, torch.Tensor] = {}
        for name, group, off, shape in self.entries:
            bucket = self.crit if group == 1 else self.main
            n = int(np.prod(shape))
            self.params[name] = bucket["p"][off:off + n].view(*shape)
            self.grads[name] = bucket["g"][off:off + n].view(*shape)
        self.stream = torch.cuda.current_stream(self.device)
        self._pver = share._pver if share is not None else {"v": 0}
        self._seen = self._pver["v"]
        h = C.c_void_p()
        check(self.lib.mimrl_create(C.byref(self.cfg), C.c_void_p(self.stream.cuda_stream), C.byref(h)))
        self.handle = h
        self._bind()
        self.task_loss = _lib.TASK_LOSSES["MAE"] if self.num_class == 1 else _lib.CLASS_LOSSES["CE"]
        kind = share.task_loss if share is not None else _lib.task_loss_code(opt)
        if kind != self.task_loss:
            self.set_task_loss(kind)

    def _bind(self):
        b = Buffers()
        b.main_p, b.main_g, b.main_m, b.main_v = (_ptr(self.main[k]) for k in "pgmv")
        b.crit_p, b.crit_g, b.crit_m, b.crit_v = (_ptr(self.crit[k]) for k in "pgmv")
        b.text, b.audio, b.video, b.labels = _ptr(self.text), _ptr(self.audio), _ptr(self.video), _ptr(self.labels)
        b.bank_c, b.bank_f, b.bank_t, b.bank_a, b.bank_v = (_ptr(self.bank[k]) for k in "CFTAV")
        b.anchors = _ptr(self.anchors)
        b.lr_main, b.lr_critic = _ptr(self.lr_main), _ptr(self.lr_critic)
        b.pred, b.feats, b.scalars = _ptr(self.pred), _ptr(self.feats), _ptr(self.scalars)
        b.counters = _ptr(self.counters)
        b.knn_override = _ptr(self.knn_override)
        self._buffers = b
        check(self.lib.mimrl_bind(self.handle, C.byref(b)))

    def close(self):
        if getattr(self, "handle", None):
            torch.cuda.synchronize(self.device)
            self.lib.mimrl_destroy(self.handle)
            self.handle = None

    def __del__(self):
        try:
            self.close()
        except Exception:
            pass

    def load_params(self, state: Dict[str, "np.ndarray | torch.Tensor"], strict: bool = True):
        for name, view in self.params.items():
            if name not in state:
                if strict:
                    raise KeyError(name)
                continue
            src = state[name]
            src = torch.from_numpy(np.ascontiguousarray(src)) if isinstance(src, np.ndarray) else src
            view.copy_(src.to(torch.float32).reshape(view.shape))
        self.params_changed()

    def params_changed(self):
        check(self.lib.mimrl_params_changed(self.handle))
        self._pver["v"] += 1
        self._seen = self._pver["v"]

    def _coherent(self):
        if self._seen != self._pver["v"]:
            check(self.lib.mimrl_params_changed(self.handle))
            self._seen = self._pver["v"]

    def _stepped(self):
        self._pver["v"] += 1
        self._seen = self._pver["v"]

    def state_dict(self) -> Dict[str, torch.Tensor]:
        return {k: v.detach().clone() for k, v in self.params.items()}

    def set_batch(self, text, audio, video, labels):
        if any(isinstance(s, Rows) for s in (text, audio, video, labels)):
            self._put_rows((self.text, self.audio, self.video, self.labels), (text, audio, video, labels), self.stream)
            return
        for dst, src in ((self.text, text), (self.audio, audio), (self.video, video)):
            src = torch.as_tensor(src)
            dst.copy_(src.reshape(dst.shape), non_blocking=True)
        self.labels.copy_(torch.as_tensor(labels).reshape(-1), non_blocking=True)

    GATHER_MAX_WORKGROUPS = 0
    GATHER_ROWS = True

    def _put_rows(self, dsts, srcs, stream):
        B = dsts[3].shape[0]
        rows = all(isinstance(s, Rows) for s in srcs)
        if rows:
            idx = srcs[0].idx
            rows = all(s.idx is idx for s in srcs) and idx.dtype == torch.int32 and idx.dim() == 1 and idx.is_contiguous()
        if rows:
            if len(idx) != B:
                raise MimrlError(f"a batch of {len(idx)} rows for an engine of batch size {B}")
            for d, s in zip(dsts, srcs):
                b = s.base
                if b.dtype != torch.float32 or not b.is_contiguous() or b.dim() < 1 or b.shape[0] < 1 or b.numel() // b.shape[0] != d.numel() // B:
                    raise MimrlError(f"Rows over a {tuple(b.shape)} {b.dtype} tensor do not fit an input of shape {tuple(d.shape)}: contiguous "
                                     f"float32 rows of the same length are needed")
                if b.device != idx.device or b.shape[0] != srcs[0].base.shape[0]:
                    raise MimrlError("the Rows of a batch must index datasets of one length on the device of their row numbers")
        if rows and self.GATHER_ROWS and idx.is_cuda and self.device.index in (None, idx.device.index):
            key = tuple(s.base.data_ptr() for s in srcs) + tuple(d.data_ptr() for d in dsts)
            cache = self.__dict__.setdefault("_gather_args", {})
            if key not in cache:
                cache[key] = ((C.c_void_p * 4)(*key[:4]), (C.c_void_p * 4)(*key[4:]),
                              (C.c_int64 * 4)(*(4 * (d.numel() // B) for d in dsts)))
            src, dst, row_bytes = cache[key]
            check(self.lib.mimrl_op_gather_rows(C.c_void_p(stream.cuda_stream), 4, src, dst, row_bytes, int(srcs[0].base.shape[0]),
                                                _ptr(idx), B, int(self.GATHER_MAX_WORKGROUPS)))
            self._gather_keep = (idx, srcs)
            return
        if rows and idx.device.type == "cpu":
            if not hasattr(self, "_host_stage"):
                self._host_stage = tuple(torch.empty(d.shape, dtype=d.dtype, pin_memory=True) for d in (self.text, self.audio, self.video, self.labels))
                self._host_stage_ev = torch.cuda.Event()
                self._host_stage_ev.record(stream)
            self._host_stage_ev.synchronize()
            for st, s, d in zip(self._host_stage, srcs, dsts):
                torch.index_select(s.base.reshape(s.base.shape[0], -1), 0, idx, out=st.view(B, -1))
                d.copy_(st, non_blocking=True)
            self._host_stage_ev.record(stream)
            return
        for d, s in zip(dsts, srcs):
            s = s.materialize() if isinstance(s, Rows) else torch.as_tensor(s)
            d.copy_(s.reshape(d.shape), non_blocking=True)

    def set_banks(self, C_all, F_all, T_all, A_all, V_all):
        n = 0 if C_all is None else len(C_all)
        if n:
            if n > self.cfg.bank_capacity:
                raise MimrlError(f"bank of {n} rows exceeds capacity {self.cfg.bank_capacity}")
            for k, src in zip("CFTAV", (C_all, F_all, T_all, A_all, V_all)):
                src = torch.as_tensor(src)
                self.bank[k][:n].copy_(src.reshape(n, -1), non_blocking=True)
        self.bank_rows = n
        self.bank_c_host = None if not n else np.ascontiguousarray(torch.as_tensor(C_all).detach().cpu().numpy().reshape(-1), dtype=np.float32)
        check(self.lib.mimrl_set_bank_rows(self.handle, n))

    def set_bank_rows(self, n: int):
        self.bank_rows = int(n)
        check(self.lib.mimrl_set_bank_rows(self.handle, int(n)))

    def optimizer_state(self) -> Dict[str, torch.Tensor]:
        return {"main_m": self.main["m"].clone(), "main_v": self.main["v"].clone(), "crit_m": self.crit["m"].clone(),
                "crit_v": self.crit["v"].clone(), "counters": self.counters.clone(), "lr_main": self.lr_main.clone(),
                "lr_critic": self.lr_critic.clone()}

    def layout_fingerprint(self) -> str:
        import hashlib
        h = hashlib.sha256(f"abi{int(self.lib.mimrl_abi_version())}".encode())
        for name, group, off, shape in self.entries:
            h.update(f"|{name}:{group}:{off}:{tuple(int(x) for x in shape)}".encode())
        return h.hexdigest()[:32]

    def named_moments(self) -> Dict[str, Dict[str, Dict[str, torch.Tensor]]]:
        out = {"main": {"m": {}, "v": {}}, "critic": {"m": {}, "v": {}}}
        for name, group, off, shape in self.entries:
            bucket, key = (self.crit, "critic") if group == 1 else (self.main, "main")
            n = int(np.prod(shape))
            for k in "mv":
                out[key][k][name] = bucket[k][off:off + n].view(*shape).clone()
        return out

    def load_named_moments(self, group: str, m: Dict[str, torch.Tensor], v: Dict[str, torch.Tensor]):
        for name, g, off, shape in self.entries:
            if (g == 1) != (group == "critic"):
                continue
            bucket = self.crit if g == 1 else self.main
            n = int(np.prod(shape))
            for k, src in (("m", m), ("v", v)):
                if name not in src:
                    raise KeyError(f"optimizer state of {name!r} missing from the checkpoint")
                bucket[k][off:off + n].copy_(torch.as_tensor(src[name]).to(torch.float32).reshape(-1))

    def load_optimizer_state(self, st: Dict[str, torch.Tensor]):
        for k, dst in (("main_m", self.main["m"]), ("main_v", self.main["v"]), ("crit_m", self.crit["m"]), ("crit_v", self.crit["v"]),
                       ("counters", self.counters), ("lr_main", self.lr_main), ("lr_critic", self.lr_critic)):
            if k in st and st[k] is not None:
                dst.copy_(torch.as_tensor(st[k]).to(dst.dtype).reshape(dst.shape))

    def set_anchors(self, stage: int, anchors, exact_ties: bool = False, bank_c=None):
        an = np.asarray(anchors, dtype=np.int32).reshape(6, self.m_anchor)
        self.anchors[stage - 1].copy_(torch.from_numpy(an), non_blocking=True)
        mask = 0
        if exact_ties:
            zc = self.bank_c_host if bank_c is None else np.asarray(bank_c, np.float32).reshape(-1)
            if zc is None:
                raise MimrlError("exact_ties needs the label bank on the host (set_banks first)")
            for e in (1, 3):
                idx = _lib.knn_r1_host(zc[:self.bank_rows], an[e], self.cfg.k_neighbor)
                if idx is not None:
                    self.knn_override[stage - 1, e].copy_(torch.from_numpy(idx.reshape(-1)), non_blocking=True)
                    mask |= 1 << e
        if mask != self._ovr_mask[stage - 1]:
            check(self.lib.mimrl_set_knn_override_mask(self.handle, stage, mask))
            self._ovr_mask[stage - 1] = mask

    def set_lr(self, lr_main: float, lr_critic: float):
        self.lr_main.fill_(float(lr_main))
        self.lr_critic.fill_(float(lr_critic))

    def stage1_step(self):
        self._coherent()
        check(self.lib.mimrl_stage1_step(self.handle))
        self._stepped()

    def stage2_step(self):
        self._coherent()
        check(self.lib.mimrl_stage2_step(self.handle))
        self._stepped()

    def set_stage2_prefetch(self, on):
        check(self.lib.mimrl_set_stage2_prefetch(self.handle, int(on)))

    def stage2_forward_tail(self):
        self._coherent()
        check(self.lib.mimrl_stage2_forward_tail(self.handle))

    def set_grad_scale(self, scale: float):
        check(self.lib.mimrl_set_grad_scale(self.handle, float(scale)))

    def set_comm(self, unique_id: bytes, world: int, rank: int):
        self._coherent()
        if unique_id is None:
            check(self.lib.mimrl_set_comm(self.handle, None, 1, 0))
            self.comm_world = 0
            return
        if int(world) > 1 and self.task_loss not in _ROW_MEAN_LOSSES:
            raise NotImplementedError("a batch-coupled task loss (RMSE, SIMSE, CCC, Focal) is the loss of the whole batch, not of one rank's "
                                      "shard: single rank only")
        buf = (C.c_char * 128).from_buffer_copy(bytes(unique_id))
        check(self.lib.mimrl_set_comm(self.handle, C.cast(buf, C.c_void_p), int(world), int(rank)))
        self.comm_world = int(world)
        self.set_grad_scale(1.0 / world)

    def set_task_loss(self, kind: int):
        self._coherent()
        if getattr(self, "comm_world", 0) > 1 and kind not in _ROW_MEAN_LOSSES:
            raise NotImplementedError("a batch-coupled task loss (RMSE, SIMSE, CCC, Focal) needs the whole batch on one rank")
        setter = self.lib.mimrl_set_class_loss if int(kind) >= _lib.CLASS_LOSSES["CE"] else self.lib.mimrl_set_task_loss
        check(setter(self.handle, int(kind)))
        self.task_loss = int(kind)

    def set_comm_critic_bf16(self, on: bool):
        self._coherent()
        check(self.lib.mimrl_set_comm_critic_bf16(self.handle, int(bool(on))))

    @staticmethod
    def comm_unique_id() -> bytes:
        buf = (C.c_char * 128)()
        check(_lib.load().mimrl_comm_unique_id(C.cast(buf, C.c_void_p)))
        return bytes(buf)

    def step(self):
        self._coherent()
        check(self.lib.mimrl_two_stage_step(self.handle))
        self._stepped()

    def stage_grads(self, stage: int):
        self._coherent()
        check(self.lib.mimrl_stage_grads(self.handle, stage))

    def stage_grads_part(self, stage: int, part: int):
        self._coherent()
        check(self.lib.mimrl_stage_grads_part(self.handle, stage, part))

    def late_grad_ranges(self):
        off = int(self.lib.mimrl_main_late_offset(self.handle))
        n = self.main["g"].numel()
        return [(off, n)] if off < n else []

    def stage_apply(self, stage: int):
        self._coherent()
        check(self.lib.mimrl_stage_apply(self.handle, stage))
        self._stepped()

    def bucket_grad(self, stage: int) -> torch.Tensor:
        return self.crit["g"] if stage == 1 else self.main["g"]

    def has_update(self, stage: int) -> bool:
        return stage == 2 or self.bank_rows > 0

    def forward(self, train: bool = False, with_losses: bool = False):
        self._coherent()
        check(self.lib.mimrl_forward(self.handle, int(train), int(with_losses)))

    def estimate(self, stage: int):
        self._coherent()
        check(self.lib.mimrl_estimate(self.handle, stage))

    def probe_cube(self, x, dout=None):
        x = torch.as_tensor(x, dtype=torch.float32, device=self.device).contiguous()
        c = self.cfg
        nb = c.n_blocks
        out = torch.empty(c.batch, c.d_outs[nb - 1][0], c.d_outs[nb - 1][1], c.d_outs[nb - 1][2], dtype=torch.float32, device=self.device)
        if dout is None:
            check(self.lib.mimrl_probe_cube(self.handle, _ptr(x), _ptr(out), None, None))
            return out
        dout = torch.as_tensor(dout, dtype=torch.float32, device=self.device).contiguous().reshape(out.shape)
        dx = torch.empty_like(x)
        check(self.lib.mimrl_probe_cube(self.handle, _ptr(x), _ptr(out), _ptr(dout), _ptr(dx)))
        return out, dx

    def probe_mi(self, stage: int, feats):
        self.feats.copy_(torch.as_tensor(feats, dtype=torch.float32).reshape(self.feats.shape))
        B = self.cfg.batch
        mi = torch.empty(2, 5, dtype=torch.float32, device=self.device)
        scores = torch.empty(5, B, B, dtype=torch.float32, device=self.device) if self.cfg.critic_type == 1 else None
        dtin = torch.empty(5, 2, B, 128, dtype=torch.float32, device=self.device) if stage == 2 else None
        check(self.lib.mimrl_probe_mi(self.handle, stage, _ptr(mi), _ptr(scores), _ptr(dtin)))
        return {"mi": mi[0], "mi_loss": mi[1], "scores": scores, "dtin": dtin}

    def probe_cmi(self, stage: int, cmi_in):
        n = self.m_anchor * self.cfg.k_neighbor
        x = torch.as_tensor(cmi_in, dtype=torch.float32, device=self.device).contiguous().reshape(6, 2 * n, 384)
        logits = torch.empty(6, 2 * n, 2, dtype=torch.float32, device=self.device)
        vals = torch.empty(2, 6, dtype=torch.float32, device=self.device)
        dcin = torch.empty(6, 2 * n, 384, dtype=torch.float32, device=self.device) if stage == 2 else None
        check(self.lib.mimrl_probe_cmi(self.handle, stage, _ptr(x), _ptr(logits), _ptr(vals), _ptr(dcin)))
        return {"logits": logits, "bce": vals[0], "cmi": vals[1], "dcin": dcin}

    def probe_encoders(self, dcube=None, dmean=None):
        c = self.cfg
        x = torch.empty(c.batch, c.time_len, 3, 128, dtype=torch.float32, device=self.device)
        if dcube is None:
            check(self.lib.mimrl_probe_encoders(self.handle, _ptr(x), None, None))
            return x
        dcube = torch.as_tensor(dcube, dtype=torch.float32, device=self.device).contiguous().reshape(x.shape)
        dm = None if dmean is None else torch.as_tensor(dmean, dtype=torch.float32, device=self.device).contiguous().reshape(3, c.batch, 128)
        check(self.lib.mimrl_probe_encoders(self.handle, _ptr(x), _ptr(dcube), _ptr(dm)))
        self._keep = (dcube, dm)
        return x

    def probe_knn(self, stage: int) -> torch.Tensor:
        out = torch.empty(6, self.m_anchor, self.cfg.k_neighbor, dtype=torch.int32, device=self.device)
        check(self.lib.mimrl_probe_knn(self.handle, stage, _ptr(out)))
        return out

    STAMP_IDS = ("gru_fwd_l0", "gru_fwd_l1", "gru_bwd_l1", "gru_bwd_l0")

    def kernel_stamps(self, slots: int = 1 << 14):
        if getattr(self, "_stamps", None) is None or self._stamps.shape[0] != slots:
            self._stamps = torch.empty(slots, 4, 2, dtype=torch.int64, device=self.device)
            check(self.lib.mimrl_set_kernel_stamps(self.handle, _ptr(self._stamps), slots))
        self._stamps.fill_(-1)

    def read_kernel_stamps(self) -> Dict[str, "np.ndarray"]:
        r = self._stamps.cpu().numpy().view(np.uint64)
        out = {}
        for i, name in enumerate(self.STAMP_IDS):
            t0, t1 = r[:, i, 0], ~r[:, i, 1]
            ok = (r[:, i, 0] != np.uint64(0xFFFFFFFFFFFFFFFF)) & (r[:, i, 1] != np.uint64(0xFFFFFFFFFFFFFFFF))
            out[name] = (t1[ok].astype(np.float64) - t0[ok].astype(np.float64)) / 100.0
        return out

    def profile(self, on: bool):
        check(self.lib.mimrl_profile_enable(self.handle, int(on)))

    def profile_read(self):
        n = len(_lib.PHASES)
        ms, cnt = (C.c_float * n)(), (C.c_int32 * n)()
        check(self.lib.mimrl_profile_read(self.handle, ms, cnt))
        return {p: (float(ms[i]), int(cnt[i])) for i, p in enumerate(_lib.PHASES)}

    def profile_read_gemm(self):
        out = (C.c_double * 4)()
        check(self.lib.mimrl_profile_read_gemm(self.handle, out))
        return {"flops": out[0], "bytes": out[1], "ms": out[2], "launches": int(out[3])}

    def _ensure_sets(self):
        if hasattr(self, "_sets"):
            return
        self._sets = [(self.text, self.audio, self.video, self.labels),
                      tuple(torch.empty_like(t) for t in (self.text, self.audio, self.video, self.labels))]
        self._active = 0
        self._upload_legacy = os.environ.get("MIMRL_UPLOAD_LEGACY") is not None
        self._copy_stream = torch.cuda.Stream(self.device, priority=0 if self._upload_legacy else -1)
        self._staged_ev = torch.cuda.Event()
        self._free_ev = [torch.cuda.Event(), torch.cuda.Event()]
        for ev in self._free_ev:
            ev.record(self.stream)

    def stage_batch(self, text, audio, video, labels):
        self._ensure_sets()
        idle = 1 - self._active
        if not self._upload_legacy:
            self._free_ev[idle].synchronize()
        with torch.cuda.stream(self._copy_stream):
            if self._upload_legacy:
                self._copy_stream.wait_event(self._free_ev[idle])
            if any(isinstance(s, Rows) for s in (text, audio, video, labels)):
                self._put_rows(self._sets[idle], (text, audio, video, labels), self._copy_stream)
            else:
                for dst, src in zip(self._sets[idle], (text, audio, video, labels)):
                    dst.copy_(torch.as_tensor(src).reshape(dst.shape), non_blocking=True)
            self._staged_ev.record(self._copy_stream)

    def commit_batch(self):
        old = self._active
        new = 1 - old
        self._free_ev[old].record(self.stream)
        self.stream.wait_event(self._staged_ev)
        t, a, v, y = self._sets[new]
        check(self.lib.mimrl_set_inputs(self.handle, new, _ptr(t), _ptr(a), _ptr(v), _ptr(y)))
        self.text, self.audio, self.video, self.labels = t, a, v, y
        self._active = new

    def stage1_pass(self, batches, on_step=None):
        self._ensure_sets()
        it = iter(batches)
        cur = next(it, None)
        if cur is None:
            return 0
        def put(slot, b):
            if any(isinstance(s, Rows) for s in b):
                return self._put_rows(self._sets[slot], tuple(b), self.stream)
            for dst, src in zip(self._sets[slot], b):
                dst.copy_(torch.as_tensor(src).reshape(dst.shape), non_blocking=True)
        def bind(slot):
            t, a, v, y = self._sets[slot]
            check(self.lib.mimrl_set_inputs(self.handle, slot, _ptr(t), _ptr(a), _ptr(v), _ptr(y)))
            self.text, self.audio, self.video, self.labels = t, a, v, y
            self._active = slot
        self._coherent()
        with torch.cuda.stream(self.stream):
            bind(1 - self._active); bind(1 - self._active)
            put(self._active, cur)
            check(self.lib.mimrl_stage1_pipe_prime(self.handle))
            n = 0
            while cur is not None:
                nxt = next(it, None)
                if nxt is not None:
                    put(1 - self._active, nxt)
                check(self.lib.mimrl_stage1_pipe(self.handle, 1 if nxt is not None else 0))
                self._stepped()
                n += 1
                if on_step is not None:
                    on_step(self)
                if nxt is not None:
                    bind(1 - self._active)
                cur = nxt
            for ev in self._free_ev:
                ev.record(self.stream)
        return n

    def read_scalars(self) -> np.ndarray:
        return self.scalars.detach().cpu().numpy()

    def workspace_bytes(self) -> int:
        return int(self.lib.mimrl_workspace_bytes(self.handle))
```

Baseline: 1252.

## Fold previous block's D-axis backward into the L-axis backward kernel

Adds an optional D-axis tail to the short L-axis backward kernel. When the next-processed block has a fused D axis, its LayerNorm backward, du GEMM and dx GEMM run in the same launch, reading the freshly computed dx tile from LDS instead of going through global memory and a separate daxis kernel. The shared daxis code is split into reusable device helpers. This saves a launch and a round trip, but the fused kernel now carries more registers and shares LDS through aliasing. It is enabled by default through a new toggle and grabs three extra gradient buffers from the pool.

```diff
diff --git a/include/mimrl.h b/include/mimrl.h
--- a/include/mimrl.h
+++ b/include/mimrl.h
@@ -111,6 +111,7 @@
 int mimrl_forward(mimrl_handle* h, int train_mode, int with_losses);
 int mimrl_estimate(mimrl_handle* h, int stage);
 int mimrl_set_stage2_prefetch(mimrl_handle* h, int on);
+int mimrl_set_cube_bwd_fold(mimrl_handle* h, int on);
 int mimrl_stage2_forward_tail(mimrl_handle* h);
 int mimrl_set_grad_scale(mimrl_handle* h, float scale);
 int mimrl_params_changed(mimrl_handle* h);
diff --git a/mimrl_amd/_lib.py b/mimrl_amd/_lib.py
--- a/mimrl_amd/_lib.py
+++ b/mimrl_amd/_lib.py
@@ -128,7 +128,7 @@
     lib.mimrl_bind.argtypes = [_FP, C.POINTER(Buffers)]
     lib.mimrl_profile_read.argtypes = [_FP, C.POINTER(C.c_float), C.POINTER(C.c_int32)]
     lib.mimrl_profile_read_gemm.argtypes = [_FP, C.POINTER(C.c_double)]
-    for fn in ("mimrl_set_bank_rows", "mimrl_stage_grads", "mimrl_stage_grads_part", "mimrl_stage_apply", "mimrl_estimate", "mimrl_profile_enable", "mimrl_set_stage2_prefetch"):
+    for fn in ("mimrl_set_bank_rows", "mimrl_stage_grads", "mimrl_stage_grads_part", "mimrl_stage_apply", "mimrl_estimate", "mimrl_profile_enable", "mimrl_set_stage2_prefetch", "mimrl_set_cube_bwd_fold"):
         getattr(lib, fn).argtypes = [_FP, C.c_int]
     lib.mimrl_set_grad_scale.argtypes = [_FP, C.c_float]
     lib.mimrl_stage_grads_part.argtypes = [_FP, C.c_int, C.c_int]
@@ -168,7 +168,7 @@
     "mimrl_op_cmi_loss", "mimrl_op_sample_anchors", "mimrl_knn_r1_host", "mimrl_set_knn_override_mask", "mimrl_op_mlp_stack_forward", "mimrl_op_mlp_stack_backward", "mimrl_op_adam",
     "mimrl_probe_cube", "mimrl_probe_mi", "mimrl_probe_cmi", "mimrl_probe_knn", "mimrl_probe_encoders", "mimrl_set_kernel_stamps", "mimrl_comm_unique_id", "mimrl_set_comm", "mimrl_main_late_offset", "mimrl_set_comm_critic_bf16",
     "mimrl_stage1_pipe_prime", "mimrl_stage1_pipe", "mimrl_set_task_loss", "mimrl_op_task_loss", "mimrl_set_class_loss", "mimrl_op_class_loss",
-    "mimrl_op_mi_infonce_rows", "mimrl_op_lstm_forward", "mimrl_op_lstm_backward", "mimrl_op_recur_btv", "mimrl_op_gather_rows",
+    "mimrl_op_mi_infonce_rows", "mimrl_op_lstm_forward", "mimrl_op_lstm_backward", "mimrl_op_recur_btv", "mimrl_op_gather_rows", "mimrl_set_cube_bwd_fold",
 ]
 
 TASK_LOSSES = {"MAE": 0, "MSE": 1, "RMSE": 2, "SIMSE": 3, "CCC": 4}
diff --git a/mimrl_amd/csrc/cube_bwd_fused.h b/mimrl_amd/csrc/cube_bwd_fused.h
--- a/mimrl_amd/csrc/cube_bwd_fused.h
+++ b/mimrl_amd/csrc/cube_bwd_fused.h
@@ -11,6 +11,13 @@
   float *dy, *du, *dx;
   float *db2, *db1;
   int B, il, hl, ol, C, act;
+  struct DTail {
+    const float *y = nullptr, *mean = nullptr, *rstd = nullptr, *gamma = nullptr, *u = nullptr;
+    const __bf16 *w2t = nullptr, *w1t = nullptr, *wrt = nullptr;
+    float *dy = nullptr, *du = nullptr, *dx = nullptr;
+    long R = 0;
+    int ik = 0;
+  } t;
 };
 bool laxis_bwd_supported(int il, int hl, int ol, int C);
 int laxis_bwd_fused(hipStream_t s, const LAxisBwdArgs& a);
diff --git a/mimrl_amd/csrc/cube_bwd_fused.hip b/mimrl_amd/csrc/cube_bwd_fused.hip
--- a/mimrl_amd/csrc/cube_bwd_fused.hip
+++ b/mimrl_amd/csrc/cube_bwd_fused.hip
@@ -14,14 +14,156 @@
 
 constexpr int CT = 128;
 constexpr int KP = 64 + 8;
-
-
-template <bool LONG = false>
-__global__ __launch_bounds__(256, LONG ? 2 : 1) void laxis_bwd_kernel(LAxisBwdArgs a) {
-  __shared__ __attribute__((aligned(16))) __bf16 sdyu[2][CT][KP];
+constexpr int DR = 32;
+constexpr int DP = 128 + 8;
+constexpr int CTD = 132;
+
+__device__ __forceinline__ void daxis_req_frags(const __bf16* wt, int n, int lh, bf16x8 (&bw)[8]) {
+#pragma unroll
+  for (int ks = 0; ks < 8; ++ks) bw[ks] = *reinterpret_cast<const bf16x8*>(wt + n * 128 + ks * 16 + 8 * lh);
+}
+
+template <typename RowC>
+__device__ __forceinline__ void daxis_req_u(const float* u, RowC rowc, int n, int lh, float (&uu)[16]) {
+#pragma unroll
+  for (int r = 0; r < 16; ++r) uu[r] = u[rowc((r & 3) + 8 * (r >> 2) + 4 * lh) * 128 + n];
+}
+
+__device__ __forceinline__ void daxis_req_gamma(const float* gamma, int part, float4 (&gm4)[4]) {
+#pragma unroll
+  for (int q = 0; q < 4; ++q) gm4[q] = *reinterpret_cast<const float4*>(gamma + part * 16 + q * 4);
+}
+
+__device__ __forceinline__ void daxis_ln_bwd(const float4 (&gz4)[4], const float4 (&yv4)[4], const float4 (&gm4)[4], float mu, float rs,
+                                             int row, int part, bool ok, float* dyp, __bf16 (*sdy)[DP], bool pg, LdsAcc (*spg)[128],
+                                             int lane) {
+#pragma clang fp contract(off)
+  float g[16], xh[16], dyk[16], gam[16];
+  float s1 = 0.f, s2 = 0.f;
+#pragma unroll
+  for (int q = 0; q < 4; ++q) {
+    const float4 gz = gz4[q];
+    const float4 yv = yv4[q];
+    const float gg[4] = {gz.x, gz.y, gz.z, gz.w}, yy[4] = {yv.x, yv.y, yv.z, yv.w};
+    gam[q * 4 + 0] = gm4[q].x; gam[q * 4 + 1] = gm4[q].y; gam[q * 4 + 2] = gm4[q].z; gam[q * 4 + 3] = gm4[q].w;
+#pragma unroll
+    for (int j = 0; j < 4; ++j) {
+      g[q * 4 + j] = gg[j];
+      xh[q * 4 + j] = (yy[j] - mu) * rs;
+      const float dxh = gg[j] * gam[q * 4 + j];
+      if (q < 2) { s1 = __builtin_fmaf(gg[j], gam[q * 4 + j], s1); s2 = __builtin_fmaf(xh[q * 4 + j], dxh, s2); }
+      else { s1 += dxh; s2 += dxh * xh[q * 4 + j]; }
+    }
+  }
+  s1 = group_sum<8>(s1); s2 = group_sum<8>(s2);
+  s1 *= (1.f / 128.f); s2 *= (1.f / 128.f);
+#pragma unroll
+  for (int q = 0; q < 4; ++q) {
+    float v[4];
+#pragma unroll
+    for (int j = 0; j < 4; ++j) v[j] = rs * __builtin_fmaf(-xh[q * 4 + j], s2, __builtin_fmaf(g[q * 4 + j], gam[q * 4 + j], -s1));
+    if (ok) *reinterpret_cast<float4*>(dyp + q * 4) = make_float4(v[0], v[1], v[2], v[3]);
+    bf16x4 p; p[0] = to_bf16(v[0]); p[1] = to_bf16(v[1]); p[2] = to_bf16(v[2]); p[3] = to_bf16(v[3]);
+    *reinterpret_cast<bf16x4*>(&sdy[row][part * 16 + q * 4]) = p;
+    if (pg) {
+#pragma unroll
+      for (int j = 0; j < 4; ++j) { const float gz = ok ? g[q * 4 + j] : 0.f; xh[q * 4 + j] *= gz; g[q * 4 + j] = gz; v[j] = ok ? v[j] : 0.f; }
+      dyk[q * 4 + 0] = v[0]; dyk[q * 4 + 1] = v[1]; dyk[q * 4 + 2] = v[2]; dyk[q * 4 + 3] = v[3];
+    }
+  }
+  if (pg) {
+    __syncthreads();
+#pragma unroll
+    for (int j = 0; j < 16; ++j) {
+      float sa = xh[j], sb = g[j], sc = dyk[j];
+#pragma unroll
+      for (int o = 8; o < 64; o <<= 1) { sa += __shfl_xor(sa, o, 64); sb += __shfl_xor(sb, o, 64); sc += __shfl_xor(sc, o, 64); }
+      if (lane < 8) { spg[0][part * 16 + j].add(sa); spg[1][part * 16 + j].add(sb); spg[2][part * 16 + j].add(sc); }
+    }
+  }
+}
+
+template <typename RowOf>
+__device__ __forceinline__ void daxis_du(const __bf16 (*sdy)[DP], __bf16 (*sdu)[DP], const bf16x8 (&bw2)[8], const float (&uu)[16], float* du,
+                                         int act, RowOf rowof, int n, int lr, int lh, bool pg, float* db1) {
+  f32x16 acc;
+#pragma unroll
+  for (int r = 0; r < 16; ++r) acc[r] = 0.f;
+#pragma unroll
+  for (int ks = 0; ks < 8; ++ks) {
+    const bf16x8 af = *reinterpret_cast<const bf16x8*>(&sdy[lr][ks * 16 + 8 * lh]);
+    acc = __builtin_amdgcn_mfma_f32_32x32x16_bf16(af, bw2[ks], acc, 0, 0, 0);
+  }
+  float csum = 0.f;
+  act_dispatch(act, [&](auto AT) __attribute__((always_inline)) {
+#pragma unroll
+  for (int r = 0; r < 16; ++r) {
+    const int m = (r & 3) + 8 * (r >> 2) + 4 * lh;
+    const long row = rowof(m);
+    float v = 0.f;
+    if (row >= 0) {
+      v = acc[r] * act_grad_c<decltype(AT)::value>(act, uu[r]);
+      du[row * 128 + n] = v;
+    }
+    sdu[m][n] = to_bf16(v);
+    csum += v;
+  }
+  });
+  if (pg) {
+    csum += __shfl_xor(csum, 32, 64);
+    if (lh == 0) acc_add(&db1[n], csum);
+  }
+}
+
+template <typename RowOf>
+__device__ __forceinline__ void daxis_dx(const __bf16 (*sdy)[DP], const __bf16 (*sdu)[DP], const bf16x8 (&bw1)[8], const bf16x8 (&bwr)[8],
+                                         float* dx, RowOf rowof, int n, int lr, int lh) {
+  f32x16 acc;
+#pragma unroll
+  for (int r = 0; r < 16; ++r) acc[r] = 0.f;
+#pragma unroll
+  for (int ks = 0; ks < 8; ++ks) {
+    const bf16x8 a1 = *reinterpret_cast<const bf16x8*>(&sdu[lr][ks * 16 + 8 * lh]);
+    acc = __builtin_amdgcn_mfma_f32_32x32x16_bf16(a1, bw1[ks], acc, 0, 0, 0);
+    const bf16x8 a2 = *reinterpret_cast<const bf16x8*>(&sdy[lr][ks * 16 + 8 * lh]);
+    acc = __builtin_amdgcn_mfma_f32_32x32x16_bf16(a2, bwr[ks], acc, 0, 0, 0);
+  }
+#pragma unroll
+  for (int r = 0; r < 16; ++r) {
+    const long row = rowof((r & 3) + 8 * (r >> 2) + 4 * lh);
+    if (row >= 0) dx[row * 128 + n] = acc[r];
+  }
+}
+
+
+template <bool LONG = false, bool DTAIL = false>
+__global__ __launch_bounds__(256, LONG || DTAIL ? 2 : 1) void laxis_bwd_kernel(LAxisBwdArgs a) {
+  static_assert(!(LONG && DTAIL), "the D-axis tail belongs to the short kernel");
+  constexpr int DYU_BYTES = 2 * CT * KP * 2, WTS_BYTES = 3 * 64 * KP * 2;
+  __shared__ __attribute__((aligned(16))) char smem[DYU_BYTES + WTS_BYTES];
+  __bf16 (*sdyu)[CT][KP] = reinterpret_cast<__bf16 (*)[CT][KP]>(smem);
   auto& sdy = sdyu[0];
   auto& sdu = sdyu[1];
-  __shared__ __attribute__((aligned(16))) __bf16 wts[3][64][KP];
+  __bf16 (*wts)[64][KP] = reinterpret_cast<__bf16 (*)[64][KP]>(smem + DYU_BYTES);
+  static_assert(64 * CTD * 4 + 2 * DR * DP * 2 <= DYU_BYTES + WTS_BYTES && 2 * DR * DP * 2 <= 64 * CTD * 4, "the tail's staging fits the operand images");
+  float* tile = reinterpret_cast<float*>(smem);
+  __bf16 (*tdy)[DR][DP] = reinterpret_cast<__bf16 (*)[DR][DP]>(smem + 64 * CTD * 4);
+  __bf16 (*tdu)[DR][DP] = reinterpret_cast<__bf16 (*)[DR][DP]>(smem);
+  bf16x8 tw2[8], tw1[8], twr[8];
+  float4 tgm[4], tyv[2][4];
+  float tuu[2][16], tmu[2], trs[2];
+  const int trow = threadIdx.x >> 3, tpart = threadIdx.x & 7;
+  const int tk = blockIdx.x;
+  auto trowc = [&](int t, int m) { return ((long)blockIdx.y * a.il + min(t * DR + m, a.il - 1)) * a.t.ik + tk; };
+  auto treq_y = [&](int t) __attribute__((always_inline)) {
+    const long rc = trowc(t, trow);
+    tmu[t] = a.t.mean[rc]; trs[t] = a.t.rstd[rc];
+#pragma unroll
+    for (int q = 0; q < 4; ++q) tyv[t][q] = *reinterpret_cast<const float4*>(a.t.y + rc * 128 + tpart * 16 + q * 4);
+  };
+  auto treq_u = [&](int t) __attribute__((always_inline)) {
+    daxis_req_u(a.t.u, [&](int m) { return trowc(t, m); }, (threadIdx.x >> 6) * 32 + (threadIdx.x & 31), (threadIdx.x & 63) >> 5, tuu[t]);
+  };
   float (*red)[2][CT] = reinterpret_cast<float (*)[2][CT]>(&sdu[0][0]);
   __shared__ float acc_l[3][64];
   __shared__ LdsAcc acc_h[64];
@@ -45,7 +187,7 @@
   }
   {
     uint4* z = reinterpret_cast<uint4*>(&wts[0][0][0]);
-    for (int i = tid; i < 3 * 64 * KP * 2 / 16; i += 256) z[i] = make_uint4(0u, 0u, 0u, 0u);
+    for (int i = tid; i < WTS_BYTES / 16; i += 256) z[i] = make_uint4(0u, 0u, 0u, 0u);
     if (tid < 64) { acc_l[0][tid] = 0.f; acc_l[1][tid] = 0.f; acc_l[2][tid] = 0.f; acc_h[tid].zero(); sgam[tid] = a.gamma[tid < ol ? tid : ol - 1]; }
   }
   __syncthreads();
@@ -152,6 +294,12 @@
       }
     });
   }
+  if constexpr (DTAIL) {
+    treq_y(0);
+    treq_y(1);
+    daxis_req_gamma(a.t.gamma, tpart, tgm);
+    daxis_req_frags(a.t.w2t, nt * 32 + lr, lh, tw2);
+  }
   __syncthreads();
   BPHASE(pb, 5);
   if constexpr (LONG) {
@@ -228,12 +376,51 @@
           if (i < il) a.dx[((long)b * il + i) * C + cc] = mt == 0 ? acc0[r] : acc1[r];
         }
     }
+    if constexpr (DTAIL) {
+      __syncthreads();
+#pragma unroll
+      for (int mt = 0; mt < 2; ++mt)
+#pragma unroll
+        for (int r = 0; r < 16; ++r) tile[(mt * 32 + (r & 3) + 8 * (r >> 2) + 4 * lh) * CTD + nt * 32 + lr] = mt == 0 ? acc0[r] : acc1[r];
+      treq_u(0);
+      treq_u(1);
+    }
   }
   __syncthreads();
   BPHASE(pb, 6);
   if (a.db2 && tid < ol) acc_add(&a.db2[tid], acc_l[2][tid]);
   if (a.db1 && tid >= 64 && tid - 64 < hl) acc_add(&a.db1[tid - 64], acc_h[tid - 64].get());
   BPHASE(pb, 7);
+  if constexpr (DTAIL) {
+    BPHASE(32, 8);
+    const int n = nt * 32 + lr;
+    const int ntile = il > DR ? 2 : 1;
+#pragma unroll
+    for (int t = 0; t < 2; ++t)
+      if (t < ntile) {
+        float4 gz4[4];
+#pragma unroll
+        for (int q = 0; q < 4; ++q) gz4[q] = *reinterpret_cast<const float4*>(&tile[(t * DR + trow) * CTD + tpart * 16 + q * 4]);
+        daxis_ln_bwd(gz4, tyv[t], tgm, tmu[t], trs[t], trow, tpart, t * DR + trow < il, a.t.dy + trowc(t, trow) * 128 + tpart * 16, tdy[t], false,
+                     nullptr, lane);
+      }
+    daxis_req_frags(a.t.w1t, n, lh, tw1);
+    daxis_req_frags(a.t.wrt, n, lh, twr);
+    __syncthreads();
+    BPHASE(32, 9);
+#pragma unroll
+    for (int t = 0; t < 2; ++t)
+      if (t < ntile)
+        daxis_du(tdy[t], tdu[t], tw2, tuu[t], a.t.du, a.act, [&](int m) { return t * DR + m < il ? ((long)b * il + t * DR + m) * a.t.ik + tk : -1L; },
+                 n, lr, lh, false, nullptr);
+    __syncthreads();
+    BPHASE(32, 10);
+#pragma unroll
+    for (int t = 0; t < 2; ++t)
+      if (t < ntile)
+        daxis_dx(tdy[t], tdu[t], tw1, twr, a.t.dx, [&](int m) { return t * DR + m < il ? ((long)b * il + t * DR + m) * a.t.ik + tk : -1L; }, n, lr, lh);
+    BPHASE(32, 15);
+  }
 }
 
 }
@@ -249,16 +436,20 @@
 int laxis_bwd_fused(hipStream_t s, const LAxisBwdArgs& a) {
   if (!laxis_bwd_supported(a.il, a.hl, a.ol, a.C)) return set_error(MIMRL_ERR_ARG, "laxis_bwd_fused: unsupported shape");
   if (!a.wr) return set_error(MIMRL_ERR_ARG, "laxis_bwd_fused: needs the residual projection");
-  if (a.il > 64) hipLaunchKernelGGL(laxis_bwd_kernel<true>, dim3(a.C / CT, a.B), dim3(256), 0, s, a);
+  if (a.t.dx) {
+    const LAxisBwdArgs::DTail& t = a.t;
+    if (a.il > 64 || t.ik < 1 || a.C != t.ik * CT || t.R != (long)a.B * a.il * t.ik)
+      return set_error(MIMRL_ERR_ARG, "laxis_bwd_fused: the D-axis tail needs il <= 64 and [B*il*ik, 128] rows");
+    if (!t.y || !t.mean || !t.rstd || !t.gamma || !t.u || !t.w2t || !t.w1t || !t.wrt || !t.dy || !t.du)
+      return set_error(MIMRL_ERR_ARG, "laxis_bwd_fused: null argument in the D-axis tail");
+    hipLaunchKernelGGL((laxis_bwd_kernel<false, true>), dim3(a.C / CT, a.B), dim3(256), 0, s, a);
+  } else if (a.il > 64) hipLaunchKernelGGL(laxis_bwd_kernel<true>, dim3(a.C / CT, a.B), dim3(256), 0, s, a);
   else hipLaunchKernelGGL(laxis_bwd_kernel<false>, dim3(a.C / CT, a.B), dim3(256), 0, s, a);
   LAUNCH_CHECK();
   return MIMRL_OK;
 }
 
 namespace {
-
-constexpr int DR = 32;
-constexpr int DP = 128 + 8;
 
 __global__ __launch_bounds__(256) void daxis_bwd_kernel(DAxisBwdArgs a) {
   __shared__ __attribute__((aligned(16))) __bf16 sdy[DR][DP];
@@ -275,108 +466,26 @@
   const bool ok1 = r1 < a.R;
   const long rc1 = ok1 ? r1 : a.R - 1;
   const float mu1 = a.mean[rc1], rs1 = a.rstd[rc1];
-  float4 gz4[4], yv4[4];
+  float4 gz4[4], yv4[4], gm4[4];
 #pragma unroll
   for (int q = 0; q < 4; ++q) {
     gz4[q] = *reinterpret_cast<const float4*>(a.dz + rc1 * 128 + part1 * 16 + q * 4);
     yv4[q] = *reinterpret_cast<const float4*>(a.y + rc1 * 128 + part1 * 16 + q * 4);
   }
+  daxis_req_gamma(a.gamma, part1, gm4);
   const int n = wave * 32 + lr;
   bf16x8 bw2[8], bw1[8], bwr[8];
-#pragma unroll
-  for (int ks = 0; ks < 8; ++ks) {
-    bw2[ks] = *reinterpret_cast<const bf16x8*>(a.w2t + n * 128 + ks * 16 + 8 * lh);
-    bw1[ks] = *reinterpret_cast<const bf16x8*>(a.w1t + n * 128 + ks * 16 + 8 * lh);
-    bwr[ks] = *reinterpret_cast<const bf16x8*>(a.wrt + n * 128 + ks * 16 + 8 * lh);
-  }
+  daxis_req_frags(a.w2t, n, lh, bw2);
+  daxis_req_frags(a.w1t, n, lh, bw1);
+  daxis_req_frags(a.wrt, n, lh, bwr);
   float uu[16];
-#pragma unroll
-  for (int r = 0; r < 16; ++r) {
-    const long row = min(r0 + (r & 3) + 8 * (r >> 2) + 4 * lh, a.R - 1);
-    uu[r] = a.u[row * 128 + n];
-  }
+  daxis_req_u(a.u, [&](int m) { return min(r0 + m, a.R - 1); }, n, lh, uu);
+  auto rowof = [&](int m) { const long row = r0 + m; return row < a.R ? row : -1L; };
   BPHASE(pb, 1);
-  {
-    const int row = row1, part = part1;
-    const long r = r1;
-    const bool ok = ok1;
-    float g[16], xh[16], dyk[16];
-    float s1 = 0.f, s2 = 0.f;
-    const float mu = mu1, rs = rs1;
-#pragma unroll
-    for (int q = 0; q < 4; ++q) {
-      const float4 gz = gz4[q];
-      const float4 yv = yv4[q];
-      const float gg[4] = {gz.x, gz.y, gz.z, gz.w}, yy[4] = {yv.x, yv.y, yv.z, yv.w};
-#pragma unroll
-      for (int j = 0; j < 4; ++j) {
-        g[q * 4 + j] = gg[j];
-        xh[q * 4 + j] = (yy[j] - mu) * rs;
-        const float dxh = gg[j] * a.gamma[part * 16 + q * 4 + j];
-        s1 += dxh; s2 += dxh * xh[q * 4 + j];
-      }
-    }
-    s1 = group_sum<8>(s1); s2 = group_sum<8>(s2);
-    s1 *= (1.f / 128.f); s2 *= (1.f / 128.f);
-#pragma unroll
-    for (int q = 0; q < 4; ++q) {
-      float v[4];
-#pragma unroll
-      for (int j = 0; j < 4; ++j) {
-        const int c = part * 16 + q * 4 + j;
-        v[j] = rs * (g[q * 4 + j] * a.gamma[c] - s1 - xh[q * 4 + j] * s2);
-      }
-      if (ok) *reinterpret_cast<float4*>(a.dy + r * 128 + part * 16 + q * 4) = make_float4(v[0], v[1], v[2], v[3]);
-      bf16x4 p; p[0] = to_bf16(v[0]); p[1] = to_bf16(v[1]); p[2] = to_bf16(v[2]); p[3] = to_bf16(v[3]);
-      *reinterpret_cast<bf16x4*>(&sdy[row][part * 16 + q * 4]) = p;
-      if (pg) {
-#pragma unroll
-        for (int j = 0; j < 4; ++j) { const float gz = ok ? g[q * 4 + j] : 0.f; xh[q * 4 + j] *= gz; g[q * 4 + j] = gz; v[j] = ok ? v[j] : 0.f; }
-        dyk[q * 4 + 0] = v[0]; dyk[q * 4 + 1] = v[1]; dyk[q * 4 + 2] = v[2]; dyk[q * 4 + 3] = v[3];
-      }
-    }
-    if (pg) {
-      __syncthreads();
-#pragma unroll
-      for (int j = 0; j < 16; ++j) {
-        float sa = xh[j], sb = g[j], sc = dyk[j];
-#pragma unroll
-        for (int o = 8; o < 64; o <<= 1) { sa += __shfl_xor(sa, o, 64); sb += __shfl_xor(sb, o, 64); sc += __shfl_xor(sc, o, 64); }
-        if (lane < 8) { spg[0][part * 16 + j].add(sa); spg[1][part * 16 + j].add(sb); spg[2][part * 16 + j].add(sc); }
-      }
-    }
-  }
+  daxis_ln_bwd(gz4, yv4, gm4, mu1, rs1, row1, part1, ok1, a.dy + rc1 * 128 + part1 * 16, sdy, pg, spg, lane);
   __syncthreads();
   BPHASE(pb, 2);
-  {
-    f32x16 acc;
-#pragma unroll
-    for (int r = 0; r < 16; ++r) acc[r] = 0.f;
-#pragma unroll
-    for (int ks = 0; ks < 8; ++ks) {
-      const bf16x8 af = *reinterpret_cast<const bf16x8*>(&sdy[lr][ks * 16 + 8 * lh]);
-      acc = __builtin_amdgcn_mfma_f32_32x32x16_bf16(af, bw2[ks], acc, 0, 0, 0);
-    }
-    float csum = 0.f;
-    act_dispatch(a.act, [&](auto AT) __attribute__((always_inline)) {
-#pragma unroll
-    for (int r = 0; r < 16; ++r) {
-      const int m = (r & 3) + 8 * (r >> 2) + 4 * lh;
-      const long row = r0 + m;
-      float v = 0.f;
-      if (row < a.R) {
-        v = acc[r] * act_grad_c<decltype(AT)::value>(a.act, uu[r]);
-        a.du[row * 128 + n] = v;
-      }
-      sdu[m][n] = to_bf16(v);
-      csum += v;
-    }
-    });
-    if (pg) {
-      csum += __shfl_xor(csum, 32, 64);
-      if (lh == 0) acc_add(&a.db1[n], csum);
-    }
-  }
+  daxis_du(sdy, sdu, bw2, uu, a.du, a.act, rowof, n, lr, lh, pg, a.db1);
   __syncthreads();
   BPHASE(pb, 3);
   if (pg && tid < 128) {
@@ -384,23 +493,7 @@
     acc_add(&a.dbeta[tid], spg[1][tid].get());
     acc_add(&a.db2[tid], spg[2][tid].get());
   }
-  {
-    f32x16 acc;
-#pragma unroll
-    for (int r = 0; r < 16; ++r) acc[r] = 0.f;
-#pragma unroll
-    for (int ks = 0; ks < 8; ++ks) {
-      const bf16x8 a1 = *reinterpret_cast<const bf16x8*>(&sdu[lr][ks * 16 + 8 * lh]);
-      acc = __builtin_amdgcn_mfma_f32_32x32x16_bf16(a1, bw1[ks], acc, 0, 0, 0);
-      const bf16x8 a2 = *reinterpret_cast<const bf16x8*>(&sdy[lr][ks * 16 + 8 * lh]);
-      acc = __builtin_amdgcn_mfma_f32_32x32x16_bf16(a2, bwr[ks], acc, 0, 0, 0);
-    }
-#pragma unroll
-    for (int r = 0; r < 16; ++r) {
-      const long row = r0 + (r & 3) + 8 * (r >> 2) + 4 * lh;
-      if (row < a.R) a.dx[row * 128 + n] = acc[r];
-    }
-  }
+  daxis_dx(sdy, sdu, bw1, bwr, a.dx, rowof, n, lr, lh);
   BPHASE(pb, 4);
 }
 
diff --git a/mimrl_amd/csrc/engine.h b/mimrl_amd/csrc/engine.h
--- a/mimrl_amd/csrc/engine.h
+++ b/mimrl_amd/csrc/engine.h
@@ -245,6 +245,7 @@
   std::vector<hipEvent_t> ev_pool;
   size_t ev_next = 0;
   bool multi_stream = true;
+  bool cube_bwd_fold = true;
   bool fused_cube_bwd = true;
   bool fused_mlp = true;
   bool fused_cube = true;
diff --git a/mimrl_amd/csrc/engine_abi.hip b/mimrl_amd/csrc/engine_abi.hip
--- a/mimrl_amd/csrc/engine_abi.hip
+++ b/mimrl_amd/csrc/engine_abi.hip
@@ -499,6 +499,15 @@
   return MIMRL_OK;
 }
 
+int mimrl_set_cube_bwd_fold(mimrl_handle* h, int on) {
+  if (!h) return set_error(MIMRL_ERR_ARG, "null handle");
+  if ((on != 0) == h->cube_bwd_fold) return MIMRL_OK;
+  HIPX(hipStreamSynchronize(h->user_stream));
+  h->drop_graphs();
+  h->cube_bwd_fold = on != 0;
+  return MIMRL_OK;
+}
+
 int64_t mimrl_workspace_bytes(const mimrl_handle* h) { return h ? (int64_t)h->ws_bytes : 0; }
 
 void mimrl_destroy(mimrl_handle* h) {
diff --git a/mimrl_amd/csrc/engine_backward.hip b/mimrl_amd/csrc/engine_backward.hip
--- a/mimrl_amd/csrc/engine_backward.hip
+++ b/mimrl_amd/csrc/engine_backward.hip
@@ -8,7 +8,8 @@
     for (int ax = 0; ax < 3; ++ax) dims[i + 1][ax] = cfg.d_outs[i][ax];
   const int per_block = 7 + (cfg.dropout_mlp[0] > 0.f) + (cfg.dropout_mlp[2] > 0.f);
   const bool defer = multi_stream && !cfg.ln_first && per_block * cfg.n_blocks + 1 <= NGBUF;
-  const int npool = defer ? NGBUF : 4;
+  const int npool = defer ? NGBUF : (cube_bwd_fold ? 7 : 4);
+  int fold_dy = -1, fold_du = -1, fold_dx = -1;
   int used[NGBUF] = {0};
   used[cur_in] = 1;
   int cur = cur_in;
@@ -64,14 +65,19 @@
     if (d_fused[i]) {
       const AxisW& a = w.ax[2];
       const long R2 = (long)B * ol * ok;
-      GRAB(i_dy); GRAB(i_du); GRAB(i_dx);
-      DAxisBwdArgs fa;
-      fa.dz = gbuf[cur]; fa.y = b.d.y; fa.mean = b.d.mean; fa.rstd = b.d.rstd; fa.gamma = P(a.ln_g); fa.u = b.d.u;
-      fa.w2t = wtT[i][0]; fa.w1t = wtT[i][1]; fa.wrt = wtT[i][2];
-      fa.dy = gbuf[i_dy]; fa.du = gbuf[i_du]; fa.dx = gbuf[i_dx];
-      fa.R = R2; fa.act = cfg.activation;
-      fa.dgamma = fa.dbeta = fa.db2 = fa.db1 = nullptr;
-      MX(daxis_bwd_fused(stream, fa));
+      int i_dy = fold_dy, i_du = fold_du, i_dx = fold_dx;
+      if (i_dx < 0) {
+        GRAB(q_dy); GRAB(q_du); GRAB(q_dx);
+        i_dy = q_dy; i_du = q_du; i_dx = q_dx;
+        DAxisBwdArgs fa;
+        fa.dz = gbuf[cur]; fa.y = b.d.y; fa.mean = b.d.mean; fa.rstd = b.d.rstd; fa.gamma = P(a.ln_g); fa.u = b.d.u;
+        fa.w2t = wtT[i][0]; fa.w1t = wtT[i][1]; fa.wrt = wtT[i][2];
+        fa.dy = gbuf[i_dy]; fa.du = gbuf[i_du]; fa.dx = gbuf[i_dx];
+        fa.R = R2; fa.act = cfg.activation;
+        fa.dgamma = fa.dbeta = fa.db2 = fa.db1 = nullptr;
+        MX(daxis_bwd_fused(stream, fa));
+      }
+      fold_dy = fold_du = fold_dx = -1;
       MX(W_fork(1, 3));
       MX(W_dpg(2, b.d.y, b.d.mean, b.d.rstd, gbuf[cur], gbuf[i_dy], gbuf[i_du], Gm(a.ln_g), Gm(a.ln_b),
                a.fc2.b >= 0 ? Gm(a.fc2.b) : nullptr, a.fc1.b >= 0 ? Gm(a.fc1.b) : nullptr, R2));
@@ -177,6 +183,17 @@
       const long C = (long)ik * id;
       GRAB(i_dy); GRAB(i_du); GRAB(i_dx);
       LAxisBwdArgs fa;
+      const bool fold = cube_bwd_fold && i > 0 && il <= 64 && id == 128 && d_fused[i - 1] && pk <= 0.f && pd <= 0.f;
+      if (fold) {
+        const AxisW& pa = blk[i - 1].ax[2];
+        const BlockBuf& pb = bb[i - 1];
+        GRAB(t_dy); GRAB(t_du); GRAB(t_dx);
+        fold_dy = t_dy; fold_du = t_du; fold_dx = t_dx;
+        fa.t.y = pb.d.y; fa.t.mean = pb.d.mean; fa.t.rstd = pb.d.rstd; fa.t.gamma = P(pa.ln_g); fa.t.u = pb.d.u;
+        fa.t.w2t = wtT[i - 1][0]; fa.t.w1t = wtT[i - 1][1]; fa.t.wrt = wtT[i - 1][2];
+        fa.t.dy = gbuf[t_dy]; fa.t.du = gbuf[t_du]; fa.t.dx = gbuf[t_dx];
+        fa.t.R = (long)B * il * ik; fa.t.ik = ik;
+      }
       fa.dz = gbuf[cur]; fa.y = b.l.y; fa.mean = b.l.mean; fa.rstd = b.l.rstd; fa.gamma = P(a.ln_g); fa.u = b.l.u;
       fa.w2 = P(a.fc2.w); fa.w1 = P(a.fc1.w); fa.wr = P(a.res);
       fa.dy = gbuf[i_dy]; fa.du = gbuf[i_du]; fa.dx = gbuf[i_dx];
diff --git a/mimrl_amd/engine.py b/mimrl_amd/engine.py
--- a/mimrl_amd/engine.py
+++ b/mimrl_amd/engine.py
@@ -276,6 +276,9 @@
     def set_stage2_prefetch(self, on):
         check(self.lib.mimrl_set_stage2_prefetch(self.handle, int(on)))
 
+    def set_cube_bwd_fold(self, on):
+        check(self.lib.mimrl_set_cube_bwd_fold(self.handle, int(bool(on))))
+
     def stage2_forward_tail(self):
         self._coherent()
         check(self.lib.mimrl_stage2_forward_tail(self.handle))
```

After: 1256 (median of 6 runs). No clear change (+0.3%).
